# Nightmare-n/GD-MAE

Measured on AMD Instinct MI355X. Metric: MAE pre-train frames/sec (Waymo-shape, 180k pts, 75% mask), higher is better.
Workload: dtype bf16

## Files before the change

### gd-mae_amd/csrc/conv_block.hip

```cpp
#include "../../include/gdmae_hip.h"
#include "common.h"
#include "dw_grouped.h"
#include "gemm.h"
#include <stdlib.h>

bool gd_spconv_supported(int cin, int cout);
int gd_spconv(hipStream_t st, const void* X, int x_f32, const int* nbr, const void* Wp, long long n, int cin, int cout, void* Y, int slot,
              float* part, const float* ride_part = nullptr, int ride_S = 0, int ride_cout = 0, int ride_cin = 0,
              float* ride_dW = nullptr);
int gd_spconv_rows(int cin, int cout, int x_f32);
int gd_bn_fold_from_partials(hipStream_t st, const float* part, int nblk, int C, double count, const float* gamma,
                             const float* beta, double eps, double momentum, float* running_mean, float* running_var,
                             long long* num_batches, double* stats, float* ab, float* mv);

namespace {

__device__ inline unsigned short cb_f2bf(float f) { return gd_to_bf16(f); }

__global__ __launch_bounds__(256) void k_gather_rows_f32_bf16(const float* __restrict__ src, const int* __restrict__ idx,
                                                              long long n_slots, int C, unsigned short* __restrict__ out) {
  const int cv = C >> 3;
  const long long total = n_slots * cv;
  for (long long i = blockIdx.x * (long long)blockDim.x + threadIdx.x; i < total; i += (long long)gridDim.x * blockDim.x) {
    const long long s = i / cv;
    const int c = (int)(i % cv) << 3;
    const int j = idx[s];
    uint4 q = make_uint4(0, 0, 0, 0);
    if (j >= 0) {
      const float4 a = *reinterpret_cast<const float4*>(src + (long long)j * C + c);
      const float4 b = *reinterpret_cast<const float4*>(src + (long long)j * C + c + 4);
      q.x = cb_f2bf(a.x) | ((unsigned)cb_f2bf(a.y) << 16);
      q.y = cb_f2bf(a.z) | ((unsigned)cb_f2bf(a.w) << 16);
      q.z = cb_f2bf(b.x) | ((unsigned)cb_f2bf(b.y) << 16);
      q.w = cb_f2bf(b.z) | ((unsigned)cb_f2bf(b.w) << 16);
    }
    *reinterpret_cast<uint4*>(out + s * C + c) = q;
  }
}

template <typename T>
__global__ __launch_bounds__(256) void k_permute_w(const T* __restrict__ W, int cout, int cin, T* __restrict__ Wt) {
  const int total = cout * 9 * cin;
  for (int e = blockIdx.x * blockDim.x + threadIdx.x; e < total; e += gridDim.x * blockDim.x) {
    const int i = e % cin, ko = e / cin, o = ko % cout, k = ko / cout;
    Wt[e] = W[((long long)o * 9 + k) * cin + i];
  }
}

struct Scratch {
  char *gemm_ws, *cs_ws, *st, *rs_ws, *c01, *dy, *gcols, *wt, *sk_ws, *dw_part;
  size_t bytes;
};
int conv_dw_pick(long long n_out, int tiles, long long* n_pad) {
  static const int wgs = getenv("GDMAE_SPCONV_DW_WGS") ? atoi(getenv("GDMAE_SPCONV_DW_WGS")) : 640;
  return gd_dw_pick(n_out, tiles, wgs, n_pad);
}
Scratch layout(void* base, long long n_in, long long n_out, int cin, int cout, int es, bool implicit) {
  Scratch s;
  size_t off = 0;
  auto take = [&](size_t b) { char* p = (char*)base + off; off += gd_align(b); return p; };
  s.gemm_ws = take(implicit ? 0 : GD_LT_WORKSPACE);
  s.cs_ws = take(gdmae_colstats_workspace_bytes(cout));
  s.st = take((size_t)3 * cout * sizeof(double));
  s.rs_ws = take(gdmae_rows_bwd_stats_workspace_bytes(cout));
  s.c01 = take((size_t)2 * cout * sizeof(float));
  long long n_pad = n_out;
  const int S_dw = implicit ? conv_dw_pick(n_out, 9 * (cout / 128) * (cin / 128), &n_pad) : 0;
  s.dy = take((size_t)n_pad * cout * es);
  s.gcols = take(implicit ? 0 : (size_t)n_in * 9 * cout * es);
  s.wt = take(implicit ? 0 : (size_t)9 * cout * cin * es);
  s.sk_ws = take(implicit ? 0 : gdmae_gemm_tn_splitk_workspace_bytes(n_out, cout, 9 * cin));
  s.dw_part = nullptr;
  if (implicit) {
    s.dw_part = take((size_t)S_dw * 9 * cout * cin * sizeof(float));
  }
  s.bytes = off;
  return s;
}
bool use_implicit(const gdmae_conv_block_args* a) {
  static const int off = getenv("GDMAE_SPCONV") ? atoi(getenv("GDMAE_SPCONV")) == 0 : 0;
  return !off && a->bf16 && a->packed_fwd != nullptr && a->packed_bwd != nullptr && gd_spconv_supported(a->cin, a->cout) &&
         gd_spconv_supported(a->cout, a->cin);
}

__global__ __launch_bounds__(256) void k_spconv_dw_reduce(const float* __restrict__ part, int S, int cout, int cin, float* __restrict__ dW) {
  const long long per_tap = (long long)S * cout * cin, mn4 = (long long)cout * cin / 4;
  for (long long e = blockIdx.x * (long long)blockDim.x + threadIdx.x; e < 9 * mn4; e += (long long)gridDim.x * blockDim.x) {
    const int k = (int)(e / mn4);
    const long long r = e % mn4;
    const float4* p = reinterpret_cast<const float4*>(part + k * per_tap) + r;
    float4 acc = make_float4(0.f, 0.f, 0.f, 0.f);
    int s = 0;
    for (; s + 8 <= S; s += 8) {
      float4 v[8];
#pragma unroll
      for (int j = 0; j < 8; ++j) v[j] = p[(long long)(s + j) * mn4];
#pragma unroll
      for (int j = 0; j < 8; ++j) { acc.x += v[j].x; acc.y += v[j].y; acc.z += v[j].z; acc.w += v[j].w; }
    }
    for (; s < S; ++s) {
      const float4 v = p[(long long)s * mn4];
      acc.x += v.x; acc.y += v.y; acc.z += v.z; acc.w += v.w;
    }
    const long long o = (r * 4) / cin, i = (r * 4) % cin;
    float4* d = reinterpret_cast<float4*>(dW + (o * 9 + k) * cin + i);
    float4 w = *d;
    w.x += acc.x; w.y += acc.y; w.z += acc.z; w.w += acc.w;
    *d = w;
  }
}

#define CB_TRY(x)             \
  do {                        \
    int rc_ = (x);            \
    if (rc_ != 0) return rc_; \
  } while (0)

}

extern "C" size_t gdmae_conv_block_scratch_bytes(long long n_in, long long n_out, int cin, int cout, int bf16) {
  size_t b = layout(nullptr, n_in, n_out, cin, cout, bf16 ? 2 : 4, false).bytes;
  if (bf16 && gd_spconv_supported(cin, cout) && gd_spconv_supported(cout, cin)) {
    const size_t bi = layout(nullptr, n_in, n_out, cin, cout, 2, true).bytes;
    b = bi > b ? bi : b;
  }
  return b;
}

extern "C" int gdmae_conv_block_fwd(const gdmae_conv_block_args* a, void* stream) {
  GD_REQUIRE(a->cin % 8 == 0 && a->cout % 8 == 0 && a->cout <= 256, "conv block: channels must be multiples of 8, cout <= 256");
  if (a->n_out <= 0) return 0;
  hipStream_t st = (hipStream_t)stream;
  const int es = a->bf16 ? 2 : 4;
  const bool implicit = use_implicit(a);
  Scratch s = layout(a->scratch, a->n_in, a->n_out, a->cin, a->cout, es, implicit);
  const long long slots = a->n_out * 9;
  bool stats_fused = false;
  if (implicit) {
    const int rpw = gd_spconv_rows(a->cin, a->cout, a->x_f32);
    const long long nblk = rpw > 0 ? (a->n_out + rpw - 1) / rpw : 0;
    static const bool fuse_ok = !(getenv("GDMAE_SPCONV_STATS") && atoi(getenv("GDMAE_SPCONV_STATS")) == 0);
    stats_fused = fuse_ok && nblk >= 1 && nblk <= 1024;
    CB_TRY(gd_spconv(st, a->x, a->x_f32, a->nbr, a->packed_fwd, a->n_out, a->cin, a->cout, a->y, GD_T_SPCONV_FWD,
                     stats_fused ? (float*)s.cs_ws : nullptr));
    if (stats_fused)
      CB_TRY(gd_bn_fold_from_partials(st, (const float*)s.cs_ws, (int)nblk, a->cout, (double)a->n_out, a->gamma, a->beta, a->eps, a->momentum,
                                      a->running_mean, a->running_var, a->num_batches, a->stats, a->ab, a->mv));
  } else if (a->bf16 && a->x_f32) {
    long long g = (slots * (a->cin / 8) + 255) / 256;
    if (g > 16384) g = 16384;
    hipLaunchKernelGGL(k_gather_rows_f32_bf16, dim3((int)g), dim3(256), 0, st, (const float*)a->x, a->nbr, slots, a->cin,
                       (unsigned short*)a->cols);
    GD_LAUNCH_CHECK();
  } else {
    CB_TRY(gdmae_gather_rows(a->x, a->nbr, slots, a->cin * es, a->cols, stream));
  }
  if (!implicit)
    CB_TRY(gdmae_gemm(a->cols, a->W, a->y, a->n_out, a->cout, 9ll * a->cin, 0, 1, a->bf16, 0, nullptr, s.gemm_ws, stream));
  if (!stats_fused)
    CB_TRY(gdmae_bn_fold(a->y, a->n_out, a->cout, a->bf16, (double)a->n_out, a->gamma, a->beta, a->eps, a->momentum, a->running_mean,
                         a->running_var, a->num_batches, a->stats, a->ab, a->mv, s.cs_ws, stream));
  CB_TRY(gdmae_rows_affine_relu_scatter(a->y, a->bf16, nullptr, a->n_out, a->cout, a->ab, a->ab + a->cout, a->out,
                                        a->out_f32 ? 0 : a->bf16, a->cout, 0, stream));
  return 0;
}

extern "C" int gdmae_conv_block_bwd(const gdmae_conv_block_args* a, void* stream) {
  GD_REQUIRE(a->cin % 8 == 0 && a->cout % 8 == 0 && a->cout <= 256, "conv block: channels must be multiples of 8, cout <= 256");
  if (a->n_out <= 0) return 0;
  hipStream_t st = (hipStream_t)stream;
  const int es = a->bf16 ? 2 : 4;
  const bool implicit = use_implicit(a);
  Scratch s = layout(a->scratch, a->n_in, a->n_out, a->cin, a->cout, es, implicit);
  const int C = a->cout;
  CB_TRY(gdmae_rows_bwd_stats(a->y, a->bf16, nullptr, a->n_out, C, a->ab, a->ab + C, a->g, a->g_f32 ? 0 : a->bf16, C, 0, nullptr,
                              s.rs_ws, stream));
  CB_TRY(gdmae_bn_bwd_coeffs_rows((const float*)s.rs_ws, gdmae_rows_bwd_stats_rows(a->n_out), 3, a->stats, a->ab, a->gamma, C,
                                  (double)a->n_out, nullptr, a->dgamma, a->dbeta, 1, (float*)s.c01, stream));
  CB_TRY(gdmae_rows_bwd(a->y, a->bf16, nullptr, a->n_out, C, a->ab, a->ab + C, (const float*)s.c01, (const float*)s.c01 + C, a->g,
                        a->g_f32 ? 0 : a->bf16, C, 0, s.dy, a->bf16, stream));
  if (implicit) {
    GdDwGroup Gp;
    Gp.n_jobs = 9;
    long long n_pad = 0;
    const int S = conv_dw_pick(a->n_out, 9 * (C / 128) * (a->cin / 128), &n_pad);
    for (int k = 0; k < 9; ++k) {
      Gp.job[k] = GdDwJob{s.dy, a->x, C, a->cin, (float*)s.dw_part + (size_t)k * S * C * a->cin, nullptr, 0, a->nbr + k, 9, a->x_f32};
    }
    {
      GdTimed timed(GD_T_SPCONV_BWD, st, (double)a->n_out * (2.0 * C + 9.0 * a->cin * (a->x_f32 ? 4 : 2) + 36.0) + 36.0 * S * C * a->cin,
                    2.0 * a->n_out * 9.0 * C * a->cin);
      CB_TRY(gd_dw_grouped_s(st, Gp, n_pad, a->n_out, S));
    }
    GD_REQUIRE(Gp.S == S, "conv block: slice count");
    static const bool rides = !(getenv("GDMAE_DW_REDUCE_RIDES") && atoi(getenv("GDMAE_DW_REDUCE_RIDES")) == 0);
    bool reduced = false;
    if (a->dx && rides) {
      const int rc = gd_spconv(st, s.dy, 0, a->nbr_t, a->packed_bwd, a->n_in, C, a->cin, a->dx, GD_T_SPCONV_BWD, nullptr, (const float*)s.dw_part, S,
                               C, a->cin, a->dW);
      if (rc != -2) {
        CB_TRY(rc);
        reduced = true;
      }
    }
    if (!reduced) {
      hipLaunchKernelGGL(k_spconv_dw_reduce, dim3(gd_div_up(9ll * C * a->cin / 4, 256)), dim3(256), 0, st, (const float*)s.dw_part, S, C, a->cin,
                         a->dW);
      GD_LAUNCH_CHECK();
      if (a->dx) CB_TRY(gd_spconv(st, s.dy, 0, a->nbr_t, a->packed_bwd, a->n_in, C, a->cin, a->dx, GD_T_SPCONV_BWD, nullptr));
    }
    return 0;
  }
  CB_TRY(gdmae_gemm_tn_splitk(s.dy, a->cols, a->dW, a->n_out, C, 9 * a->cin, a->bf16, 1, s.sk_ws, stream));
  if (a->dx) {
    CB_TRY(gdmae_gather_rows(s.dy, a->nbr_t, a->n_in * 9, C * es, s.gcols, stream));
    const int total = C * 9 * a->cin;
    if (a->bf16) hipLaunchKernelGGL((k_permute_w<unsigned short>), dim3((total + 255) / 256), dim3(256), 0, st, (const unsigned short*)a->W, C, a->cin, (unsigned short*)s.wt);
    else hipLaunchKernelGGL((k_permute_w<float>), dim3((total + 255) / 256), dim3(256), 0, st, (const float*)a->W, C, a->cin, (float*)s.wt);
    GD_LAUNCH_CHECK();
    CB_TRY(gdmae_gemm(s.gcols, s.wt, a->dx, a->n_in, a->cin, 9ll * C, 0, 0, a->bf16, 0, nullptr, s.gemm_ws, stream));
  }
  return 0;
}
```

### gd-mae_amd/csrc/partition.hip

```cpp
#include "common.h"

struct Dims {
  int B, Y, X;
};

struct VisLoad {
  const float* mask;
  const int* counts;
  __device__ int operator()(long long p) const { return (p < counts[1] && mask[p] == 0.f) ? 1 : 0; }
};
struct VisStore {
  const int* counts;
  const int* pillar_cell;
  int* tok_pillar;
  int* tok_cell;
  int* map;
  __device__ void operator()(long long p, int ex, int v) const {
    if (v) {
      tok_pillar[ex] = (int)p;
      int c = pillar_cell[p];
      tok_cell[ex] = c;
      map[c] = ex;
    }
  }
};

extern "C" int gdmae_visible_tokens(const float* mask, const int* pillar_cell, const int* vox_counts, long long m_cap,
                                    long long n_cells, int* tok_pillar, int* tok_cell, int* map, int* n_tok,
                                    void* scan_ws, void* stream) {
  hipStream_t st = (hipStream_t)stream;
  GD_CHECK(hipMemsetAsync(map, 0xFF, sizeof(int) * n_cells, st));
  return gd_device_scan<int>(m_cap, VisLoad{mask, vox_counts}, VisStore{vox_counts, pillar_cell, tok_pillar, tok_cell, map},
                             n_tok, (int*)scan_ws, st);
}

__global__ __launch_bounds__(256) void k_mark_down(const int* __restrict__ n_in, const int* __restrict__ tok_cell,
                                                   Dims di, Dims dn, int* __restrict__ flag) {
  const int M = *n_in;
  for (int t = blockIdx.x * blockDim.x + threadIdx.x; t < M; t += gridDim.x * blockDim.x) {
    int c = tok_cell[t];
    int x = c % di.X;
    int r = c / di.X;
    int y = r % di.Y;
    int b = r / di.Y;
#pragma unroll
    for (int ky = 0; ky < 3; ++ky) {
      int ty = y + 1 - ky;
      if (ty < 0 || (ty & 1)) continue;
      int oy = ty >> 1;
      if (oy >= dn.Y) continue;
#pragma unroll
      for (int kx = 0; kx < 3; ++kx) {
        int tx = x + 1 - kx;
        if (tx < 0 || (tx & 1)) continue;
        int ox = tx >> 1;
        if (ox >= dn.X) continue;
        flag[(b * dn.Y + oy) * dn.X + ox] = 1;
      }
    }
  }
}

struct FlagLoad {
  const int* flag;
  __device__ int operator()(long long c) const { return flag[c]; }
};
struct FlagStore {
  int* tok_cell;
  int* map;
  __device__ void operator()(long long c, int ex, int v) const {
    if (v) {
      tok_cell[ex] = (int)c;
      map[c] = ex;
    } else {
      map[c] = -1;
    }
  }
};

extern "C" int gdmae_downsample_tokens(const int* n_in, const int* tok_cell_in, long long cap_in, int B, int Yi, int Xi,
                                       int* tok_cell_out, int* map_out, int* n_out, int* flag_ws, void* scan_ws,
                                       void* stream) {
  hipStream_t st = (hipStream_t)stream;
  Dims di{B, Yi, Xi};
  Dims dn{B, (Yi + 2 - 3) / 2 + 1, (Xi + 2 - 3) / 2 + 1};
  const long long cells = (long long)B * dn.Y * dn.X;
  GD_CHECK(hipMemsetAsync(flag_ws, 0, sizeof(int) * cells, st));
  int grid = gd_div_up(cap_in > 0 ? cap_in : 1, 256);
  if (grid > 2048) grid = 2048;
  hipLaunchKernelGGL(k_mark_down, dim3(grid), dim3(256), 0, st, n_in, tok_cell_in, di, dn, flag_ws);
  GD_LAUNCH_CHECK();
  return gd_device_scan<int>(cells, FlagLoad{flag_ws}, FlagStore{tok_cell_out, map_out}, n_out, (int*)scan_ws, st);
}

__global__ __launch_bounds__(256) void k_rulebook(const int* __restrict__ n_tok, const int* __restrict__ tok_cell, Dims dt,
                                                  Dims dm, const int* __restrict__ map, int mode, int* __restrict__ nbr) {
  const long long total = (long long)(*n_tok) * 9;
  for (long long i = blockIdx.x * (long long)blockDim.x + threadIdx.x; i < total; i += (long long)gridDim.x * blockDim.x) {
    const int t = (int)(i / 9), k = (int)(i % 9);
    const int ky = k / 3, kx = k % 3;
    int c = tok_cell[t];
    int x = c % dt.X;
    int r = c / dt.X;
    int y = r % dt.Y;
    int b = r / dt.Y;
    int my, mx;
    bool ok = true;
    if (mode == 0) {
      my = y + ky - 1;
      mx = x + kx - 1;
    } else if (mode == 1) {
      my = 2 * y - 1 + ky;
      mx = 2 * x - 1 + kx;
    } else {
      int ty = y + 1 - ky, tx = x + 1 - kx;
      ok = !(ty & 1) && !(tx & 1) && ty >= 0 && tx >= 0;
      my = ty >> 1;
      mx = tx >> 1;
    }
    ok = ok && my >= 0 && my < dm.Y && mx >= 0 && mx < dm.X;
    nbr[i] = ok ? map[(b * dm.Y + my) * dm.X + mx] : -1;
  }
}

extern "C" int gdmae_rulebook(const int* n_tok, const int* tok_cell, long long cap, int B, int Yt, int Xt, int Ym,
                              int Xm, const int* map, int mode, int* nbr, void* stream) {
  GD_REQUIRE(mode >= 0 && mode <= 2, "rulebook mode");
  int grid = gd_div_up((cap > 0 ? cap : 1) * 9, 256);
  if (grid > 4096) grid = 4096;
  hipLaunchKernelGGL(k_rulebook, dim3(grid), dim3(256), 0, (hipStream_t)stream, n_tok, tok_cell, Dims{B, Yt, Xt},
                     Dims{B, Ym, Xm}, map, mode, nbr);
  GD_LAUNCH_CHECK();
  return 0;
}

struct WinParams {
  int B, Y, X;
  int wx, wy;
  int sx, sy;
  int nwx, nwy, nwz;
  int nlev;
  int lo[3], hi[3], T[3];
};

__device__ inline int win_token(const WinParams& P, const int* map, int w, int lane, int& ref_id) {
  const int wyi = w % P.nwy;
  const int r = w / P.nwy;
  const int wxi = r % P.nwx;
  const int b = r / P.nwx;
  ref_id = b * (P.nwx * P.nwy * P.nwz) + wxi * (P.nwy * P.nwz) + wyi * P.nwz;
  if (lane >= P.wx * P.wy) return -1;
  const int ly = lane / P.wx, lx = lane % P.wx;
  const int x = wxi * P.wx - P.sx + lx;
  const int y = wyi * P.wy - P.sy + ly;
  if (x < 0 || x >= P.X || y < 0 || y >= P.Y) return -1;
  return map[(b * P.Y + y) * P.X + x];
}

__global__ __launch_bounds__(256) void k_win_count(WinParams P, const int* __restrict__ map, int n_win,
                                                   int* __restrict__ win_cnt) {
  const int lane = threadIdx.x & (GD_WAVE - 1);
  const int wib = threadIdx.x / GD_WAVE;
  for (int w = blockIdx.x * 4 + wib; w < n_win; w += gridDim.x * 4) {
    int ref;
    int t = win_token(P, map, w, lane, ref);
    unsigned long long m = __ballot(t >= 0);
    if (lane == 0) win_cnt[w] = __popcll(m);
  }
}

__device__ inline int win_level(const WinParams& P, int cnt) {
  for (int l = 0; l < P.nlev; ++l)
    if (cnt >= P.lo[l] && cnt < P.hi[l]) return l;
  return -1;
}

struct WinLoad {
  WinParams P;
  const int* win_cnt;
  __device__ U128 operator()(long long w) const {
    int c = win_cnt[w];
    if (c <= 0) return U128{0ull, 0ull};
    int l = win_level(P, c);
    if (l < 0) return U128{0ull, 0ull};
    return U128{1ull << (21 * l), (unsigned long long)c << (21 * l)};
  }
};
struct WinStore {
  int* win_dense;
  int* win_tokpre;
  __device__ void operator()(long long w, U128 ex, U128 v) const {
    if (v.a) {
      int l = (v.a >> 21) ? ((v.a >> 42) ? 2 : 1) : 0;
      win_dense[w] = (int)((ex.a >> (21 * l)) & 0x1FFFFFull);
      win_tokpre[w] = (int)((ex.b >> (21 * l)) & 0x1FFFFFull);
    }
  }
};

__global__ void k_win_totals(const U128* total, int* counts) {
  if (threadIdx.x == 0 && blockIdx.x == 0) {
    int nw = 0, nt = 0;
    for (int l = 0; l < 3; ++l) {
      int a = (int)((total->a >> (21 * l)) & 0x1FFFFFull);
      int b = (int)((total->b >> (21 * l)) & 0x1FFFFFull);
      counts[l] = a;
      counts[3 + l] = b;
      nw += a;
      nt += b;
    }
    counts[6] = nw;
    counts[7] = nt;
  }
}

__global__ __launch_bounds__(256) void k_win_fill(WinParams P, const int* __restrict__ map, int n_win,
                                                  const int* __restrict__ win_cnt, const int* __restrict__ win_dense,
                                                  const int* __restrict__ win_tokpre, const int* __restrict__ counts,
                                                  int* __restrict__ tok_win, int* __restrict__ tok_level,
                                                  int* __restrict__ tok_slot, int* __restrict__ tok_pos,
                                                  int* __restrict__ csr_tok, int* __restrict__ win_start,
                                                  int* __restrict__ win_len) {
  const int lane = threadIdx.x & (GD_WAVE - 1);
  const int wib = threadIdx.x / GD_WAVE;
  for (int w = blockIdx.x * 4 + wib; w < n_win; w += gridDim.x * 4) {
    const int cnt = win_cnt[w];
    if (cnt <= 0) continue;
    const int l = win_level(P, cnt);
    if (l < 0) continue;
    int ref;
    const int t = win_token(P, map, w, lane, ref);
    const unsigned long long m = __ballot(t >= 0);
    int wbase = 0, tbase = 0;
    for (int q = 0; q < l; ++q) {
      wbase += counts[q];
      tbase += counts[3 + q];
    }
    const int d = win_dense[w];
    const int start = tbase + win_tokpre[w];
    if (lane == 0) {
      win_start[wbase + d] = start;
      win_len[wbase + d] = cnt;
    }
    if (t >= 0) {
      const int r = __popcll(m & ((1ull << lane) - 1ull));
      csr_tok[start + r] = t;
      tok_win[t] = ref;
      tok_level[t] = l;
      tok_slot[t] = d * P.T[l] + r;
      tok_pos[t] = lane;
    }
  }
}

extern "C" size_t gdmae_window_workspace_bytes(int B, int Y, int X, int wx, int wy) {
  long long nwx = (X + wx - 1) / wx + 1, nwy = (Y + wy - 1) / wy + 1;
  long long n = B * nwx * nwy;
  return gd_align(sizeof(int) * n) * 3 + gd_align(sizeof(U128) * (gd_scan_ws_elems(n) + 2)) + 4096;
}

extern "C" int gdmae_window_partition(const int* map, int B, int Y, int X, int wx, int wy, int shifted, int nlev,
                                      const int* drop_lo, const int* drop_hi, const int* max_tokens, int* tok_win,
                                      int* tok_level, int* tok_slot, int* tok_pos, int* csr_tok, int* win_start,
                                      int* win_len, int* counts, void* workspace, size_t workspace_bytes, void* stream) {
  hipStream_t st = (hipStream_t)stream;
  GD_REQUIRE(wx * wy <= GD_WAVE && wx > 0 && wy > 0, "window must fit one wavefront (wx*wy <= 64)");
  GD_REQUIRE(nlev >= 1 && nlev <= 3, "1..3 drop levels");
  WinParams P;
  P.B = B;
  P.Y = Y;
  P.X = X;
  P.wx = wx;
  P.wy = wy;
  P.sx = shifted ? wx / 2 : wx;
  P.sy = shifted ? wy / 2 : wy;
  P.nwx = (X + wx - 1) / wx + 1;
  P.nwy = (Y + wy - 1) / wy + 1;
  P.nwz = 2;
  P.nlev = nlev;
  for (int l = 0; l < 3; ++l) {
    P.lo[l] = l < nlev ? drop_lo[l] : 0;
    P.hi[l] = l < nlev ? drop_hi[l] : 0;
    P.T[l] = l < nlev ? max_tokens[l] : 0;
  }
  const long long n_win = (long long)B * P.nwx * P.nwy;
  GD_REQUIRE(n_win < (1 << 21), "window grid too large for the packed scan");
  GD_REQUIRE(workspace_bytes >= gdmae_window_workspace_bytes(B, Y, X, wx, wy), "window workspace too small");
  GdArena A(workspace, workspace_bytes);
  int* win_cnt = A.take<int>(n_win);
  int* win_dense = A.take<int>(n_win);
  int* win_tokpre = A.take<int>(n_win);
  U128* scan_ws = A.take<U128>(gd_scan_ws_elems(n_win) + 2);
  U128* total = scan_ws + gd_scan_ws_elems(n_win);
  int grid = gd_div_up(n_win, 4);
  if (grid > 8192) grid = 8192;
  hipLaunchKernelGGL(k_win_count, dim3(grid), dim3(256), 0, st, P, map, (int)n_win, win_cnt);
  GD_LAUNCH_CHECK();
  int rc = gd_device_scan<U128>(n_win, WinLoad{P, win_cnt}, WinStore{win_dense, win_tokpre}, total, scan_ws, st);
  if (rc) return rc;
  hipLaunchKernelGGL(k_win_totals, dim3(1), dim3(64), 0, st, total, counts);
  GD_LAUNCH_CHECK();
  hipLaunchKernelGGL(k_win_fill, dim3(grid), dim3(256), 0, st, P, map, (int)n_win, win_cnt, win_dense, win_tokpre,
                     counts, tok_win, tok_level, tok_slot, tok_pos, csr_tok, win_start, win_len);
  GD_LAUNCH_CHECK();
  return 0;
}



struct VisCellLoad {
  const float* mask;
  const int* cell2pillar;
  __device__ int operator()(long long c) const {
    const int p = cell2pillar[c];
    const float m = mask[p < 0 ? 0 : p];
    return (int)(p >= 0) & (int)(m == 0.f);
  }
};
struct VisCellStore {
  const int* cell2pillar;
  int* tok_pillar;
  int* tok_cell;
  int* map;
  __device__ void operator()(long long c, int ex, int v) const {
    map[c] = v ? ex : -1;
    if (v) {
      tok_pillar[ex] = cell2pillar[c];
      tok_cell[ex] = (int)c;
    }
  }
};
size_t gd_plan_scan_state_bytes(long long n) { return gd_scan_lb_state_bytes<int>(n); }
size_t gd_plan_win_state_bytes(long long n) { return gd_scan_lb_state_bytes<U128>(n); }

int gd_plan_visible_tokens(const float* mask, const int* cell2pillar, long long n_cells, int* tok_pillar, int* tok_cell, int* map,
                           int* n_tok, void* lb_state, hipStream_t st) {
  return gd_device_scan_lb<int>(n_cells, VisCellLoad{mask, cell2pillar}, VisCellStore{cell2pillar, tok_pillar, tok_cell, map}, GdNoTotal{},
                                n_tok, lb_state, st);
}

struct DownLoad {
  const int* map_in;
  Dims di, dn;
  __device__ int operator()(long long c) const {
    const int ci = (int)c;
    const int ox = ci % dn.X;
    const int r = ci / dn.X;
    const int oy = r % dn.Y, b = r / dn.Y;
    const int* m = map_in + (long long)b * di.Y * di.X;
    int any = 0;
#pragma unroll
    for (int ky = 0; ky < 3; ++ky) {
      const int iy = 2 * oy - 1 + ky;
      const int cy = iy < 0 ? 0 : (iy >= di.Y ? di.Y - 1 : iy);
#pragma unroll
      for (int kx = 0; kx < 3; ++kx) {
        const int ix = 2 * ox - 1 + kx;
        const int cx = ix < 0 ? 0 : (ix >= di.X ? di.X - 1 : ix);
        const int v = m[(long long)cy * di.X + cx];
        any |= (int)(v >= 0 && iy == cy && ix == cx);
      }
    }
    return any;
  }
};
int gd_plan_downsample(const int* map_in, int B, int Yi, int Xi, int* tok_cell_out, int* map_out, int* n_out, void* lb_state,
                       hipStream_t st) {
  Dims di{B, Yi, Xi};
  Dims dn{B, (Yi + 2 - 3) / 2 + 1, (Xi + 2 - 3) / 2 + 1};
  const long long cells = (long long)B * dn.Y * dn.X;
  return gd_device_scan_lb<int>(cells, DownLoad{map_in, di, dn}, FlagStore{tok_cell_out, map_out}, GdNoTotal{}, n_out, lb_state, st);
}

struct PlanJob {
  const int* n_tok;
  const int* tok_cell;
  Dims dt, dm;
  const int* map;
  int mode, s;
  int* nbr;
  int* nbr_rev;
};
constexpr int kPlanMaxJobs = 16;
struct PlanJobs {
  PlanJob j[kPlanMaxJobs];
  int count;
};
__global__ __launch_bounds__(256) void k_plan_jobs(PlanJobs J) {
  const PlanJob& q = J.j[blockIdx.y];
  const int n = *q.n_tok;
  if (q.mode == 3) {
    const int ss = q.s * q.s;
    const long long total = (long long)n * ss;
    for (long long i = blockIdx.x * (long long)blockDim.x + threadIdx.x; i < total; i += (long long)gridDim.x * blockDim.x) {
      const int t = (int)(i / ss), e = (int)(i % ss);
      const int c = q.tok_cell[t];
      const int x = c % q.dt.X, r = c / q.dt.X, y = r % q.dt.Y, b = r / q.dt.Y;
      q.nbr[i] = (b * (q.dt.Y * q.s) + y * q.s + e / q.s) * (q.dt.X * q.s) + x * q.s + e % q.s;
    }
    return;
  }
  const long long total = (long long)n * 9;
  for (long long i = blockIdx.x * (long long)blockDim.x + threadIdx.x; i < total; i += (long long)gridDim.x * blockDim.x) {
    const int t = (int)(i / 9), k = (int)(i % 9);
    const int ky = k / 3, kx = k % 3;
    const int c = q.tok_cell[t];
    const int x = c % q.dt.X, r = c / q.dt.X, y = r % q.dt.Y, b = r / q.dt.Y;
    int my, mx;
    bool ok = true;
    if (q.mode == 0) {
      my = y + ky - 1;
      mx = x + kx - 1;
    } else if (q.mode == 1) {
      my = 2 * y - 1 + ky;
      mx = 2 * x - 1 + kx;
    } else {
      const int ty = y + 1 - ky, tx = x + 1 - kx;
      ok = !(ty & 1) && !(tx & 1) && ty >= 0 && tx >= 0;
      my = ty >> 1;
      mx = tx >> 1;
    }
    ok = ok && my >= 0 && my < q.dm.Y && mx >= 0 && mx < q.dm.X;
    const int v = ok ? q.map[(b * q.dm.Y + my) * q.dm.X + mx] : -1;
    q.nbr[i] = v;
    if (q.nbr_rev) q.nbr_rev[(long long)t * 9 + (8 - k)] = v;
  }
}
int gd_plan_jobs(const PlanJobs& J, long long cap_max, hipStream_t st) {
  if (J.count <= 0) return 0;
  int grid = gd_div_up((cap_max > 0 ? cap_max : 1) * 9, 256);
  if (grid > 2048) grid = 2048;
  hipLaunchKernelGGL(k_plan_jobs, dim3(grid, J.count), dim3(256), 0, st, J);
  GD_LAUNCH_CHECK();
  return 0;
}

constexpr int GD_WIN_JOBS = 8;
struct WinSet {
  WinParams P[GD_WIN_JOBS];
  const int* map[GD_WIN_JOBS];
  int n_win[GD_WIN_JOBS];
  int* win_cnt[GD_WIN_JOBS];
  int* win_dense[GD_WIN_JOBS];
  int* win_tokpre[GD_WIN_JOBS];
  int* counts[GD_WIN_JOBS];
  int *tok_win[GD_WIN_JOBS], *tok_level[GD_WIN_JOBS], *tok_slot[GD_WIN_JOBS], *tok_pos[GD_WIN_JOBS], *csr_tok[GD_WIN_JOBS],
      *win_start[GD_WIN_JOBS], *win_len[GD_WIN_JOBS];
};
__global__ __launch_bounds__(256) void k_win_count2(WinSet Q) {
  const int lane = threadIdx.x & (GD_WAVE - 1);
  const int wib = threadIdx.x / GD_WAVE;
  const int sh = blockIdx.y;
  const int n_win = Q.n_win[sh];
  const int* __restrict__ map = Q.map[sh];
  for (int w = blockIdx.x * 4 + wib; w < n_win; w += gridDim.x * 4) {
    int ref;
    const int t = win_token(Q.P[sh], map, w, lane, ref);
    const unsigned long long m = __ballot(t >= 0);
    if (lane == 0) Q.win_cnt[sh][w] = __popcll(m);
  }
}
struct WinTotal {
  int* counts;
  __device__ void operator()(U128 total) const {
    int nw = 0, nt = 0;
    for (int l = 0; l < 3; ++l) {
      const int a = (int)((total.a >> (21 * l)) & 0x1FFFFFull);
      const int b = (int)((total.b >> (21 * l)) & 0x1FFFFFull);
      counts[l] = a;
      counts[3 + l] = b;
      nw += a;
      nt += b;
    }
    counts[6] = nw;
    counts[7] = nt;
  }
};
__global__ __launch_bounds__(256) void k_win_fill2(WinSet Q) {
  const int lane = threadIdx.x & (GD_WAVE - 1);
  const int wib = threadIdx.x / GD_WAVE;
  const int sh = blockIdx.y;
  const int n_win = Q.n_win[sh];
  const int* __restrict__ map = Q.map[sh];
  const WinParams& P = Q.P[sh];
  const int* counts = Q.counts[sh];
  for (int w = blockIdx.x * 4 + wib; w < n_win; w += gridDim.x * 4) {
    const int cnt = Q.win_cnt[sh][w];
    if (cnt <= 0) continue;
    const int l = win_level(P, cnt);
    if (l < 0) continue;
    int ref;
    const int t = win_token(P, map, w, lane, ref);
    const unsigned long long m = __ballot(t >= 0);
    int wbase = 0, tbase = 0;
    for (int q = 0; q < l; ++q) {
      wbase += counts[q];
      tbase += counts[3 + q];
    }
    const int d = Q.win_dense[sh][w];
    const int start = tbase + Q.win_tokpre[sh][w];
    if (lane == 0) {
      Q.win_start[sh][wbase + d] = start;
      Q.win_len[sh][wbase + d] = cnt;
    }
    if (t >= 0) {
      const int r = __popcll(m & ((1ull << lane) - 1ull));
      Q.csr_tok[sh][start + r] = t;
      Q.tok_win[sh][t] = ref;
      Q.tok_level[sh][t] = l;
      Q.tok_slot[sh][t] = d * P.T[l] + r;
      Q.tok_pos[sh][t] = lane;
    }
  }
}
size_t gd_plan_windows_ws_bytes(int B, int Y, int X, int wx, int wy) {
  const long long n = (long long)B * ((X + wx - 1) / wx + 1) * ((Y + wy - 1) / wy + 1);
  return 2 * 3 * gd_align(sizeof(int) * n);
}
long long gd_plan_n_windows(int B, int Y, int X, int wx, int wy) { return (long long)B * ((X + wx - 1) / wx + 1) * ((Y + wy - 1) / wy + 1); }
struct GdWinStage {
  const int* map;
  int B, Y, X, wx, wy, nlev;
  const int *drop_lo, *drop_hi, *max_tokens;
  int* out[2][7];
  int* counts[2];
  void* workspace;
  void* lb_state;
};
int gd_plan_windows_all(const GdWinStage* stages, int n_stages, hipStream_t st) {
  GD_REQUIRE(n_stages >= 1 && 2 * n_stages <= GD_WIN_JOBS, "window partitions: at most four stages per launch");
  WinSet Q;
  GdScanBatch<U128, WinLoad, WinStore, WinTotal, GD_WIN_JOBS> Sc;
  long long n_max = 1;
  for (int i = 0; i < n_stages; ++i) {
    const GdWinStage& g = stages[i];
    GD_REQUIRE(g.wx * g.wy <= GD_WAVE && g.wx > 0 && g.wy > 0, "window must fit one wavefront (wx*wy <= 64)");
    GD_REQUIRE(g.nlev >= 1 && g.nlev <= 3, "1..3 drop levels");
    const long long n_win = gd_plan_n_windows(g.B, g.Y, g.X, g.wx, g.wy);
    GD_REQUIRE(n_win < (1 << 21), "window grid too large for the packed scan");
    n_max = n_win > n_max ? n_win : n_max;
    GdArena A(g.workspace, gd_plan_windows_ws_bytes(g.B, g.Y, g.X, g.wx, g.wy));
    for (int sh = 0; sh < 2; ++sh) {
      const int j = 2 * i + sh;
      WinParams& P = Q.P[j];
      P.B = g.B; P.Y = g.Y; P.X = g.X; P.wx = g.wx; P.wy = g.wy;
      P.sx = sh ? g.wx / 2 : g.wx;
      P.sy = sh ? g.wy / 2 : g.wy;
      P.nwx = (g.X + g.wx - 1) / g.wx + 1;
      P.nwy = (g.Y + g.wy - 1) / g.wy + 1;
      P.nwz = 2;
      P.nlev = g.nlev;
      for (int l = 0; l < 3; ++l) {
        P.lo[l] = l < g.nlev ? g.drop_lo[l] : 0;
        P.hi[l] = l < g.nlev ? g.drop_hi[l] : 0;
        P.T[l] = l < g.nlev ? g.max_tokens[l] : 0;
      }
      Q.map[j] = g.map;
      Q.n_win[j] = (int)n_win;
      Q.win_cnt[j] = A.take<int>(n_win);
      Q.win_dense[j] = A.take<int>(n_win);
      Q.win_tokpre[j] = A.take<int>(n_win);
      Q.counts[j] = g.counts[sh];
      Q.tok_win[j] = g.out[sh][0]; Q.tok_level[j] = g.out[sh][1]; Q.tok_slot[j] = g.out[sh][2]; Q.tok_pos[j] = g.out[sh][3];
      Q.csr_tok[j] = g.out[sh][4]; Q.win_start[j] = g.out[sh][5]; Q.win_len[j] = g.out[sh][6];
      Sc.n[j] = n_win;
      Sc.load[j] = WinLoad{P, Q.win_cnt[j]};
      Sc.store[j] = WinStore{Q.win_dense[j], Q.win_tokpre[j]};
      Sc.on_total[j] = WinTotal{g.counts[sh]};
      Sc.S[j] = gd_scan_lb_state<U128>(n_win, (char*)g.lb_state + sh * gd_plan_win_state_bytes(n_win));
    }
  }
  for (int j = 2 * n_stages; j < GD_WIN_JOBS; ++j) {
    Q.P[j] = Q.P[0]; Q.map[j] = Q.map[0]; Q.n_win[j] = 0;
    Q.win_cnt[j] = Q.win_cnt[0]; Q.win_dense[j] = Q.win_dense[0]; Q.win_tokpre[j] = Q.win_tokpre[0]; Q.counts[j] = Q.counts[0];
    Q.tok_win[j] = Q.tok_win[0]; Q.tok_level[j] = Q.tok_level[0]; Q.tok_slot[j] = Q.tok_slot[0]; Q.tok_pos[j] = Q.tok_pos[0];
    Q.csr_tok[j] = Q.csr_tok[0]; Q.win_start[j] = Q.win_start[0]; Q.win_len[j] = Q.win_len[0];
    Sc.n[j] = 0; Sc.load[j] = Sc.load[0]; Sc.store[j] = Sc.store[0]; Sc.on_total[j] = Sc.on_total[0]; Sc.S[j] = Sc.S[0];
  }
  int grid = gd_div_up(n_max, 4);
  if (grid > 4096) grid = 4096;
  hipLaunchKernelGGL(k_win_count2, dim3(grid, 2 * n_stages), dim3(256), 0, st, Q);
  GD_LAUNCH_CHECK();
  int rc = gd_device_scan_lb_batch(Sc, 2 * n_stages, st);
  if (rc) return rc;
  hipLaunchKernelGGL(k_win_fill2, dim3(grid, 2 * n_stages), dim3(256), 0, st, Q);
  GD_LAUNCH_CHECK();
  return 0;
}
```

### gd-mae_amd/csrc/plan.hip

```cpp
#include "../../include/gdmae_hip.h"
#include "common.h"
#include <string.h>

int gd_voxelize_impl(const float* points, long long n_points, int n_cols, const float* lo, const float* vs, const int* grid_xyz,
                     int batch_size, float* points_out, long long* point_coords, long long* inverse, int* inverse32,
                     long long* voxel_coords, int* pillar_cell, int* pillar_pt_off, int* pillar_pts, int* point_rank,
                     int* sample_pillar_off, float* pillar_mean, int* cell2pillar_out, int* counts, void* workspace, size_t workspace_bytes,
                     void* lb_state, float* points_pm, int* row_pillar, hipStream_t st);
size_t gd_voxelize_lb_state_bytes(long long n_points, long long cells);
size_t gd_plan_scan_state_bytes(long long n);
size_t gd_plan_win_state_bytes(long long n);
int gd_plan_visible_tokens(const float* mask, const int* cell2pillar, long long n_cells, int* tok_pillar, int* tok_cell, int* map,
                           int* n_tok, void* lb_state, hipStream_t st);
int gd_plan_downsample(const int* map_in, int B, int Yi, int Xi, int* tok_cell_out, int* map_out, int* n_out, void* lb_state,
                       hipStream_t st);
struct Dims {
  int B, Y, X;
};
struct PlanJob {
  const int* n_tok;
  const int* tok_cell;
  Dims dt, dm;
  const int* map;
  int mode, s;
  int* nbr;
  int* nbr_rev;
};
constexpr int kPlanMaxJobs = 16;
struct PlanJobs {
  PlanJob j[kPlanMaxJobs];
  int count;
};
int gd_plan_jobs(const PlanJobs& J, long long cap_max, hipStream_t st);
size_t gd_plan_windows_ws_bytes(int B, int Y, int X, int wx, int wy);
long long gd_plan_n_windows(int B, int Y, int X, int wx, int wy);
struct GdWinStage {
  const int* map;
  int B, Y, X, wx, wy, nlev;
  const int *drop_lo, *drop_hi, *max_tokens;
  int* out[2][7];
  int* counts[2];
  void* workspace;
  void* lb_state;
};
int gd_plan_windows_all(const GdWinStage* stages, int n_stages, hipStream_t st);
size_t gd_decoder_tiles_lb_state_bytes(long long nt);
int gd_decoder_tiles_lb(const int* const* maps, const int* strides, int k, int B, int H, int W, int* tile_slot, int* tile_list, int* n_act,
                        int* flag, void* lb_state, hipStream_t st);
int gd_decoder_site_rulebook(const int* site, const int* n_dev, int sites_per_tok, long long cap_sites, const int* tile_slot, int H, int W,
                             int* nbr, hipStream_t st);

namespace {

struct StageGeo {
  int Y, X;
  long long cap;
  long long cap_in;
  int up_s;
  long long n_win;
};

struct Layout {
  gdmae_plan_buffer* table;
  int max_entries, n;
  size_t off;
  bool ok;
  long long add(const char* name, size_t bytes) {
    const size_t o = off;
    if (table) {
      if (n >= max_entries) {
        ok = false;
        return -1;
      }
      strncpy(table[n].name, name, sizeof(table[n].name) - 1);
      table[n].name[sizeof(table[n].name) - 1] = 0;
      table[n].offset = (long long)o;
      table[n].bytes = (long long)bytes;
    }
    ++n;
    off += gd_align(bytes);
    return (long long)o;
  }
};

struct Offsets {
  long long lb_state, counts, points, point_coords, inverse, inverse32, voxel_coords, pillar_cell, pt_off, pillar_pts, point_rank,
      sample_off, pillar_mean, cell2pillar, points_pm, row_pillar, vox_ws, mask, len_keep, tok_pillar;
  long long vis_tok_cell, vis_map;
  struct {
    long long tok_cell, map, nbr_subm, nbr_subm_t, nbr_down, nbr_down_t, up_sites, win_ws;
    long long w[2][7];
  } s[GDMAE_PLAN_MAX_STAGES];
  long long dec_slot, dec_list, dec_flag, dec_nbr[3];
  size_t lb_bytes, vox_ws_bytes;
  int n_counts;
  bool dec;
  StageGeo geo[GDMAE_PLAN_MAX_STAGES];
  long long cap_pts, m_cap, cells;
};

int check(const gdmae_plan_params* p) {
  GD_REQUIRE(p != nullptr, "geometry plan: null parameters");
  GD_REQUIRE(p->n_points >= 0 && p->n_points < (1ll << 31) && p->n_cols >= 4 && p->n_cols <= 65 && p->batch_size >= 1,
             "geometry plan: bad point buffer");
  GD_REQUIRE(p->grid[0] >= 1 && p->grid[1] >= 1 && p->grid[2] == 1, "geometry plan: single-layer pillar grids (spt_backbone_mae.py:94)");
  GD_REQUIRE(p->n_stages >= 1 && p->n_stages <= GDMAE_PLAN_MAX_STAGES, "geometry plan: 1..4 stages");
  for (int i = 0; i < p->n_stages; ++i) {
    GD_REQUIRE(p->stride[i] == 1 || p->stride[i] == 2, "geometry plan: conv_down stride 1 or 2 (k3 s2 p1)");
    GD_REQUIRE(i == 0 || p->stride[i] == 2, "geometry plan: only the first stage may keep the resolution");
    GD_REQUIRE(p->win_x[i] >= 1 && p->win_y[i] >= 1 && p->win_x[i] * p->win_y[i] <= 64, "geometry plan: window must fit one wavefront");
    GD_REQUIRE(p->n_levels[i] >= 1 && p->n_levels[i] <= 3, "geometry plan: 1..3 drop levels");
  }
  GD_REQUIRE(p->n_dec >= 0 && p->n_dec <= 3, "geometry plan: at most 3 decoder source stages");
  for (int g = 0; g < p->n_dec; ++g) GD_REQUIRE(p->dec_sources[g] >= 0 && p->dec_sources[g] < p->n_stages, "geometry plan: decoder source");
  return 0;
}

int layout(const gdmae_plan_params* p, gdmae_plan_buffer* table, int max_entries, Offsets& O, size_t* total, int* n_entries) {
  if (int rc = check(p)) return rc;
  Layout L{table, max_entries, 0, 0, true};
  const int B = p->batch_size, gx = p->grid[0], gy = p->grid[1], F = p->n_cols - 1;
  const long long n0 = p->cap_points > p->n_points ? p->cap_points : p->n_points;
  O.cells = (long long)B * gx * gy;
  GD_REQUIRE(O.cells < (1ll << 31), "geometry plan: B*Y*X must fit int32");
  O.cap_pts = n0 > 0 ? n0 : 1;
  O.m_cap = n0 < O.cells ? n0 : O.cells;
  if (O.m_cap < 1) O.m_cap = 1;
  const long long cap = O.cap_pts;
  int Y = gy, X = gx;
  long long c = O.m_cap;
  for (int i = 0; i < p->n_stages; ++i) {
    StageGeo& g = O.geo[i];
    g.cap_in = c;
    if (p->stride[i] == 2) {
      Y = (Y - 1) / 2 + 1;
      X = (X - 1) / 2 + 1;
      c = 4 * c < (long long)B * Y * X ? 4 * c : (long long)B * Y * X;
    }
    g.Y = Y; g.X = X; g.cap = c;
    const int us = gy / Y;
    g.up_s = (us >= 1 && us * Y == gy && us * X == gx) ? us : 0;
    g.n_win = gd_plan_n_windows(B, Y, X, p->win_x[i], p->win_y[i]);
    GD_REQUIRE(g.n_win < (1 << 21), "geometry plan: window grid too large for the packed scan");
    GD_REQUIRE(g.cap < (1 << 21), "geometry plan: stage token capacity must stay below 2^21 (21-bit fields of the packed window scan)");
  }
  O.dec = p->n_dec > 0;
  for (int g = 0; g < p->n_dec; ++g) {
    const int us = O.geo[p->dec_sources[g]].up_s;
    O.dec = O.dec && (us == 1 || us == 2 || us == 4 || us == 8);
  }
  const long long nt = (long long)B * ((gy + 7) / 8) * ((gx + 7) / 8);
  size_t lb = gd_voxelize_lb_state_bytes(n0, O.cells) + gd_plan_scan_state_bytes(O.cells);
  for (int i = 0; i < p->n_stages; ++i) {
    if (p->stride[i] == 2) lb += gd_plan_scan_state_bytes((long long)B * O.geo[i].Y * O.geo[i].X);
    lb += 2 * gd_plan_win_state_bytes(O.geo[i].n_win);
  }
  if (O.dec) lb += gd_decoder_tiles_lb_state_bytes(nt);
  O.lb_bytes = lb;
  O.lb_state = L.add("lb_state", lb);
  O.n_counts = 2 + p->n_stages + 16 * p->n_stages + 1 + 1;
  O.counts = L.add("counts", sizeof(int) * O.n_counts);
  O.points = L.add("points", sizeof(float) * cap * p->n_cols);
  O.point_coords = L.add("point_coords", sizeof(long long) * cap * 4);
  O.inverse = L.add("inverse", sizeof(long long) * cap);
  O.inverse32 = L.add("inverse32", sizeof(int) * cap);
  O.voxel_coords = L.add("voxel_coords", sizeof(long long) * cap * 4);
  O.pillar_cell = L.add("pillar_cell", sizeof(int) * cap);
  O.pt_off = L.add("pt_off", sizeof(int) * (cap + 1));
  O.pillar_pts = L.add("pillar_pts", sizeof(int) * cap);
  O.point_rank = L.add("point_rank", sizeof(int) * cap);
  O.sample_off = L.add("sample_off", sizeof(int) * (B + 1));
  O.pillar_mean = L.add("pillar_mean", sizeof(float) * cap * F);
  O.cell2pillar = L.add("cell2pillar", sizeof(int) * O.cells);
  O.points_pm = L.add("points_pm", sizeof(float) * cap * p->n_cols);
  O.row_pillar = L.add("row_pillar", sizeof(int) * cap);
  O.vox_ws_bytes = gdmae_voxelize_workspace_bytes(n0, B, gx, gy, 1);
  O.vox_ws = L.add("vox_ws", O.vox_ws_bytes);
  O.mask = L.add("mask", sizeof(float) * O.m_cap);
  O.len_keep = L.add("len_keep", sizeof(int) * B);
  O.tok_pillar = L.add("tok_pillar", sizeof(int) * O.m_cap);
  O.vis_tok_cell = O.vis_map = -1;
  if (p->stride[0] == 2) {
    O.vis_tok_cell = L.add("vis.tok_cell", sizeof(int) * O.m_cap);
    O.vis_map = L.add("vis.map", sizeof(int) * O.cells);
  }
  char nm[40];
  static const char* const kWin[7] = {"tok_win", "tok_level", "tok_slot", "tok_pos", "csr_tok", "win_start", "win_len"};
  for (int i = 0; i < p->n_stages; ++i) {
    const StageGeo& g = O.geo[i];
    auto name = [&](const char* s) { snprintf(nm, sizeof(nm), "s%d.%s", i, s); return (const char*)nm; };
    O.s[i].tok_cell = L.add(name("tok_cell"), sizeof(int) * g.cap);
    O.s[i].map = L.add(name("map"), sizeof(int) * (long long)B * g.Y * g.X);
    O.s[i].nbr_subm = L.add(name("nbr_subm"), sizeof(int) * g.cap * 9);
    O.s[i].nbr_subm_t = L.add(name("nbr_subm_t"), sizeof(int) * g.cap * 9);
    O.s[i].nbr_down = O.s[i].nbr_down_t = O.s[i].up_sites = -1;
    if (p->stride[i] == 2) {
      O.s[i].nbr_down = L.add(name("nbr_down"), sizeof(int) * g.cap * 9);
      O.s[i].nbr_down_t = L.add(name("nbr_down_t"), sizeof(int) * g.cap_in * 9);
    }
    if (g.up_s > 1) O.s[i].up_sites = L.add(name("up_sites"), sizeof(int) * g.cap * g.up_s * g.up_s);
    O.s[i].win_ws = L.add(name("win_ws"), gd_plan_windows_ws_bytes(B, g.Y, g.X, p->win_x[i], p->win_y[i]));
    const long long wcap = g.n_win < g.cap ? g.n_win : g.cap;
    for (int sh = 0; sh < 2; ++sh)
      for (int k = 0; k < 7; ++k) {
        snprintf(nm, sizeof(nm), "s%d.w%d.%s", i, sh, kWin[k]);
        O.s[i].w[sh][k] = L.add(nm, sizeof(int) * (k < 5 ? g.cap : wcap));
      }
  }
  O.dec_slot = O.dec_list = O.dec_flag = -1;
  if (O.dec) {
    O.dec_slot = L.add("dec.tile_slot", sizeof(int) * nt);
    O.dec_list = L.add("dec.tile_list", sizeof(int) * nt);
    O.dec_flag = L.add("dec.flag", sizeof(int) * nt);
    for (int g = 0; g < p->n_dec; ++g) {
      const StageGeo& sg = O.geo[p->dec_sources[g]];
      snprintf(nm, sizeof(nm), "dec.nbr%d", g);
      O.dec_nbr[g] = L.add(nm, sizeof(int) * sg.cap * sg.up_s * sg.up_s * 9);
    }
  }
  GD_REQUIRE(L.ok, "geometry plan: buffer table too small");
  if (total) *total = L.off;
  if (n_entries) *n_entries = L.n;
  return 0;
}

}

extern "C" int gdmae_geometry_plan_layout(const gdmae_plan_params* p, gdmae_plan_buffer* table, int max_entries, int* n_entries,
                                          size_t* total_bytes) {
  Offsets O;
  return layout(p, table, max_entries, O, total_bytes, n_entries);
}

extern "C" int gdmae_geometry_plan(const gdmae_plan_params* p, const float* points, const float* noise, void* arena, size_t arena_bytes,
                                   void* stream) {
  Offsets O;
  size_t total = 0;
  if (int rc = layout(p, nullptr, 0, O, &total, nullptr)) return rc;
  GD_REQUIRE(arena != nullptr && arena_bytes >= total, "geometry plan: arena too small (gdmae_geometry_plan_layout)");
  GD_REQUIRE(!p->masked || noise != nullptr, "geometry plan: masking needs one noise value per pillar (capacity min(points, cells))");
  hipStream_t st = (hipStream_t)stream;
  char* A = (char*)arena;
  auto I = [&](long long off) { return off < 0 ? (int*)nullptr : (int*)(A + off); };
  const int B = p->batch_size, gx = p->grid[0], gy = p->grid[1], ns = p->n_stages;
  int* counts = I(O.counts);
  int* n_tok = counts + 2;
  int* win_counts = counts + 2 + ns;
  int* n_act = counts + 2 + ns + 16 * ns;
  int* n_vis = n_act + 1;
  GD_CHECK(hipMemsetAsync(A + O.lb_state, 0, (size_t)(O.counts - O.lb_state) + gd_align(sizeof(int) * O.n_counts), st));
  char* lb = A + O.lb_state;
  {
    int rc = gd_voxelize_impl(points, p->n_points, p->n_cols, p->lo, p->vs, p->grid, B, (float*)(A + O.points), (long long*)(A + O.point_coords),
                              (long long*)(A + O.inverse), I(O.inverse32), (long long*)(A + O.voxel_coords), I(O.pillar_cell), I(O.pt_off),
                              I(O.pillar_pts), I(O.point_rank), I(O.sample_off), (float*)(A + O.pillar_mean), I(O.cell2pillar), counts,
                              A + O.vox_ws, O.vox_ws_bytes, lb, p->want_pm ? (float*)(A + O.points_pm) : nullptr,
                              p->want_pm ? I(O.row_pillar) : nullptr, st);
    if (rc) return rc;
    lb += gd_voxelize_lb_state_bytes(p->n_points, O.cells);
  }
  float* mask = (float*)(A + O.mask);
  if (p->masked) {
    int rc = gdmae_random_mask(noise, I(O.sample_off), B, p->keep_frac, mask, I(O.len_keep), stream);
    if (rc) return rc;
  } else {
    GD_CHECK(hipMemsetAsync(mask, 0, sizeof(float) * O.m_cap, st));
  }
  const bool first_strided = p->stride[0] == 2;
  int* cur_cell = first_strided ? I(O.vis_tok_cell) : I(O.s[0].tok_cell);
  int* cur_map = first_strided ? I(O.vis_map) : I(O.s[0].map);
  int* cur_n = first_strided ? n_vis : n_tok;
  {
    int rc = gd_plan_visible_tokens(mask, I(O.cell2pillar), O.cells, I(O.tok_pillar), cur_cell, cur_map, cur_n, lb, st);
    if (rc) return rc;
    lb += gd_plan_scan_state_bytes(O.cells);
  }
  int Yp = gy, Xp = gx;
  PlanJobs J;
  J.count = 0;
  long long cap_max = 1;
  GdWinStage W[4];
  GD_REQUIRE(ns <= 4, "geometry plan: at most four stages");
  for (int i = 0; i < ns; ++i) {
    const StageGeo& g = O.geo[i];
    GD_REQUIRE(J.count + 4 <= kPlanMaxJobs, "geometry plan: job table full");
    if (g.cap > cap_max) cap_max = g.cap;
    if (p->stride[i] == 2) {
      int rc = gd_plan_downsample(cur_map, B, Yp, Xp, I(O.s[i].tok_cell), I(O.s[i].map), n_tok + i, lb, st);
      if (rc) return rc;
      lb += gd_plan_scan_state_bytes((long long)B * g.Y * g.X);
      J.j[J.count++] = PlanJob{n_tok + i, I(O.s[i].tok_cell), Dims{B, g.Y, g.X}, Dims{B, Yp, Xp}, cur_map, 1, 0, I(O.s[i].nbr_down), nullptr};
      J.j[J.count++] = PlanJob{cur_n, cur_cell, Dims{B, Yp, Xp}, Dims{B, g.Y, g.X}, I(O.s[i].map), 2, 0, I(O.s[i].nbr_down_t), nullptr};
      if (g.cap_in > cap_max) cap_max = g.cap_in;
      cur_cell = I(O.s[i].tok_cell);
      cur_map = I(O.s[i].map);
      cur_n = n_tok + i;
      Yp = g.Y;
      Xp = g.X;
    }
    J.j[J.count++] = PlanJob{cur_n, cur_cell, Dims{B, g.Y, g.X}, Dims{B, g.Y, g.X}, cur_map, 0, 0, I(O.s[i].nbr_subm), I(O.s[i].nbr_subm_t)};
    if (g.up_s > 1) {
      J.j[J.count++] = PlanJob{cur_n, cur_cell, Dims{B, g.Y, g.X}, Dims{B, g.Y, g.X}, nullptr, 3, g.up_s, I(O.s[i].up_sites), nullptr};
      if (g.cap * g.up_s * g.up_s / 9 + 1 > cap_max) cap_max = g.cap * g.up_s * g.up_s / 9 + 1;
    }
    GdWinStage& w = W[i];
    w.map = cur_map;
    w.B = B; w.Y = g.Y; w.X = g.X; w.wx = p->win_x[i]; w.wy = p->win_y[i]; w.nlev = p->n_levels[i];
    w.drop_lo = p->drop_lo[i]; w.drop_hi = p->drop_hi[i]; w.max_tokens = p->max_tokens[i];
    w.counts[0] = win_counts + 16 * i;
    w.counts[1] = win_counts + 16 * i + 8;
    for (int sh = 0; sh < 2; ++sh)
      for (int k = 0; k < 7; ++k) w.out[sh][k] = I(O.s[i].w[sh][k]);
    w.workspace = A + O.s[i].win_ws;
    w.lb_state = lb;
    lb += 2 * gd_plan_win_state_bytes(g.n_win);
  }
  {
    int rc = gd_plan_jobs(J, cap_max, st);
    if (rc) return rc;
    rc = gd_plan_windows_all(W, ns, st);
    if (rc) return rc;
  }
  if (O.dec) {
    const int* maps[3];
    int ups[3];
    for (int g = 0; g < p->n_dec; ++g) {
      maps[g] = I(O.s[p->dec_sources[g]].map);
      ups[g] = O.geo[p->dec_sources[g]].up_s;
    }
    int rc = gd_decoder_tiles_lb(maps, ups, p->n_dec, B, gy, gx, I(O.dec_slot), I(O.dec_list), n_act, I(O.dec_flag), lb, st);
    if (rc) return rc;
    for (int g = 0; g < p->n_dec; ++g) {
      const int si = p->dec_sources[g];
      const StageGeo& sg = O.geo[si];
      const int* sites = sg.up_s > 1 ? I(O.s[si].up_sites) : I(O.s[si].tok_cell);
      rc = gd_decoder_site_rulebook(sites, n_tok + si, sg.up_s * sg.up_s, sg.cap * sg.up_s * sg.up_s, I(O.dec_slot), gy, gx, I(O.dec_nbr[g]), st);
      if (rc) return rc;
    }
  }
  return 0;
}
```

### gd-mae_amd/csrc/spconv.hip

```cpp
#include "../../include/gdmae_hip.h"
#include "common.h"
#include "dw_grouped.h"
#include <stdlib.h>

typedef float f32x16 __attribute__((ext_vector_type(16)));
typedef __bf16 bf16x8 __attribute__((ext_vector_type(8)));

namespace {

union SpFrag {
  uint4 q;
  bf16x8 v;
};
__device__ inline unsigned short sp_f2bf(float f) { return gd_to_bf16(f); }
__device__ inline unsigned sp_pack2(float lo, float hi) { return gd_pack_bf16(lo, hi); }

struct SpArgs {
  const void* X;
  const int* nbr;
  const uint4* Wp;
  unsigned short* Y;
  long long n;
  float* part;
  const float* ride_part;
  float* ride_dW;
  int ride_S, ride_cout, ride_cin;
  unsigned ride_blocks;
  const float* bias;
};

__device__ __forceinline__ void sp_ride_dw_reduce(const SpArgs& A) {
  const int S = A.ride_S, cout = A.ride_cout, cin = A.ride_cin;
  const long long per_tap = (long long)S * cout * cin, mn4 = (long long)cout * cin / 4;
  for (long long e = blockIdx.x * (long long)blockDim.x + threadIdx.x; e < 9 * mn4; e += (long long)A.ride_blocks * blockDim.x) {
    const int k = (int)(e / mn4);
    const long long r = e % mn4;
    const float4* p = reinterpret_cast<const float4*>(A.ride_part + k * per_tap) + r;
    float4 acc = make_float4(0.f, 0.f, 0.f, 0.f);
    int s = 0;
    for (; s + 8 <= S; s += 8) {
      float4 v[8];
#pragma unroll
      for (int j = 0; j < 8; ++j) v[j] = p[(long long)(s + j) * mn4];
#pragma unroll
      for (int j = 0; j < 8; ++j) { acc.x += v[j].x; acc.y += v[j].y; acc.z += v[j].z; acc.w += v[j].w; }
    }
    for (; s < S; ++s) {
      const float4 v = p[(long long)s * mn4];
      acc.x += v.x; acc.y += v.y; acc.z += v.z; acc.w += v.w;
    }
    const long long o = (r * 4) / cin, i = (r * 4) % cin;
    float4* d = reinterpret_cast<float4*>(A.ride_dW + (o * 9 + k) * cin + i);
    float4 w = *d;
    w.x += acc.x; w.y += acc.y; w.z += acc.z; w.w += acc.w;
    *d = w;
  }
}

constexpr int kWaves = 8;

#ifndef SP_ROWS256
#define SP_ROWS256 64
#endif
template <int CIN, int COUT, bool SRC_F32>
struct SpRows {
#ifndef SP_ROWS128
#define SP_ROWS128 128
#endif
  static constexpr int value = COUT >= 256 ? ((SRC_F32 && CIN >= 256) ? 32 : SP_ROWS256) : ((CIN == 128 && !SRC_F32) ? SP_ROWS128 : 64);
};

template <int CIN, int COUT, bool SRC_F32, bool EPI = false>
__global__ __launch_bounds__(512, 2) void k_spconv(SpArgs A) {
  constexpr int ROWS = SpRows<CIN, COUT, SRC_F32>::value;
  constexpr int KS = CIN / 16;
  constexpr int MB = COUT / 32;
  constexpr int MPW = MB >= kWaves ? MB / kWaves : 1;
  constexpr int WPB = MB >= kWaves ? 1 : kWaves / MB;
  constexpr int NPW = (ROWS / 32) / WPB;
  static_assert(NPW >= 1 && NPW * WPB * 32 == ROWS, "row blocks");
  constexpr int XP = CIN * 2 + 16;
  constexpr int SP = COUT * 2 + 16;
  constexpr int CPR = CIN / 8;
  constexpr int RPP = 512 / CPR;
  constexpr int P = ROWS / RPP;
  static_assert(P >= 1 && ROWS % RPP == 0, "unsupported shape");
  extern __shared__ __align__(16) unsigned char lds[];
  if (blockIdx.x < A.ride_blocks) return sp_ride_dw_reduce(A);
  const unsigned blk = blockIdx.x - A.ride_blocks;
  const int tid = threadIdx.x, lane = tid & 63, wv = tid >> 6;
  const long long row0 = (long long)blk * ROWS;
  const int mb0 = wv / WPB;
  const int nb0 = (wv % WPB) * NPW;
  const uint4* __restrict__ wp = A.Wp + (size_t)mb0 * 64 + lane;

  constexpr int RING = (KS == 16 && (ROWS == 64 || SRC_F32)) ? ((SRC_F32 && ROWS == 64) ? 4 : 8) : ((KS == 8 && ROWS == 128) ? 4 : KS);
  SpFrag wr[RING][MPW];
#pragma unroll
  for (int ks = 0; ks < RING; ++ks)
#pragma unroll
    for (int j = 0; j < MPW; ++j) wr[ks][j].q = wp[((size_t)ks * MB + j * kWaves) * 64];

  constexpr int GD = 1;
  constexpr int RQ = SRC_F32 ? 2 : 1;
  const int gc = tid % CPR;
  long long nrow[P];
  unsigned rvalid = 0u;
#pragma unroll
  for (int p = 0; p < P; ++p) {
    const long long g = row0 + p * RPP + tid / CPR;
    rvalid |= g < A.n ? 1u << p : 0u;
    nrow[p] = (g < A.n ? g : A.n - 1) * 9;
  }
  int idx[P];
  uint4 rq[1][P][RQ];
  unsigned keep[1] = {0u};
  auto load_idx = [&](int tap) {
#pragma unroll
    for (int p = 0; p < P; ++p) idx[p] = A.nbr[nrow[p] + tap];
  };
  auto fetch = [&](int slot) {
    unsigned k = 0u;
#pragma unroll
    for (int p = 0; p < P; ++p) {
      asm volatile("" : "+v"(idx[p]));
      const bool ok = idx[p] >= 0 && ((rvalid >> p) & 1u);
      const long long j = ok ? idx[p] : 0;
      k |= ok ? 1u << p : 0u;
      if (SRC_F32) {
        const float* s = (const float*)A.X + j * CIN + gc * 8;
        rq[slot][p][0] = *reinterpret_cast<const uint4*>(s);
        rq[slot][p][RQ - 1] = *reinterpret_cast<const uint4*>(s + 4);
      } else {
        rq[slot][p][0] = *reinterpret_cast<const uint4*>((const unsigned short*)A.X + j * CIN + gc * 8);
      }
    }
    keep[slot] = k;
  };
  auto stage = [&](unsigned char* b, int slot) {
#pragma unroll
    for (int p = 0; p < P; ++p) {
      uint4 q;
      if (SRC_F32) {
        const uint4 a = rq[slot][p][0], c = rq[slot][p][RQ - 1];
        q.x = sp_pack2(__uint_as_float(a.x), __uint_as_float(a.y)); q.y = sp_pack2(__uint_as_float(a.z), __uint_as_float(a.w));
        q.z = sp_pack2(__uint_as_float(c.x), __uint_as_float(c.y)); q.w = sp_pack2(__uint_as_float(c.z), __uint_as_float(c.w));
      } else {
        q = rq[slot][p][0];
      }
      const unsigned m = ((keep[slot] >> p) & 1u) ? 0xFFFFFFFFu : 0u;
      q.x &= m; q.y &= m; q.z &= m; q.w &= m;
      *reinterpret_cast<uint4*>(b + (p * RPP + tid / CPR) * XP + gc * 16) = q;
    }
  };
  load_idx(0);
  fetch(0);
  load_idx(1);
  stage(lds, 0);
  __syncthreads();

  f32x16 acc[MPW][NPW];
#pragma unroll
  for (int j = 0; j < MPW; ++j)
#pragma unroll
    for (int b = 0; b < NPW; ++b)
#pragma unroll
      for (int i = 0; i < 16; ++i) acc[j][b][i] = 0.f;

#pragma unroll
  for (int tap = 0; tap < 9; ++tap) {
    if (tap + GD < 9) {
      fetch(0);
      if (tap + GD + 1 < 9) load_idx(tap + GD + 1);
    }
    __builtin_amdgcn_sched_barrier(0);
    const unsigned char* lb = lds + (tap & 1) * (ROWS * XP) + ((nb0 * 32) + (lane & 31)) * XP + (lane >> 5) * 16;
    SpFrag sf[2][NPW];
#pragma unroll
    for (int b = 0; b < NPW; ++b) sf[0][b].q = *reinterpret_cast<const uint4*>(lb + b * 32 * XP);
#pragma unroll
    for (int ks = 0; ks < KS; ++ks) {
      if (ks + 1 < KS) {
#pragma unroll
        for (int b = 0; b < NPW; ++b) sf[(ks + 1) & 1][b].q = *reinterpret_cast<const uint4*>(lb + b * 32 * XP + (ks + 1) * 32);
      }
#pragma unroll
      for (int j = 0; j < MPW; ++j)
#pragma unroll
        for (int b = 0; b < NPW; ++b) acc[j][b] = __builtin_amdgcn_mfma_f32_32x32x16_bf16(wr[ks % RING][j].v, sf[ks & 1][b].v, acc[j][b], 0, 0, 0);
      if (tap * KS + ks + RING < 9 * KS) {
#pragma unroll
        for (int j = 0; j < MPW; ++j) wr[ks % RING][j].q = wp[(((size_t)tap * KS + ks + RING) * MB + j * kWaves) * 64];
      }
      __builtin_amdgcn_sched_barrier(0);
    }
    if (tap < 8) stage(lds + ((tap + 1) & 1) * (ROWS * XP), 0);
    __syncthreads();
  }

#pragma unroll
  for (int j = 0; j < MPW; ++j) {
    const int cb = (mb0 + j * kWaves) * 32 + 4 * (lane >> 5);
#pragma unroll
    for (int b = 0; b < NPW; ++b) {
      const int row = (nb0 + b) * 32 + (lane & 31);
#pragma unroll
      for (int q = 0; q < 4; ++q) {
        uint2 o;
        if constexpr (EPI) {
          const float4 bv = *reinterpret_cast<const float4*>(A.bias + cb + 8 * q);
          o.x = sp_pack2(fmaxf(acc[j][b][4 * q] + bv.x, 0.f), fmaxf(acc[j][b][4 * q + 1] + bv.y, 0.f));
          o.y = sp_pack2(fmaxf(acc[j][b][4 * q + 2] + bv.z, 0.f), fmaxf(acc[j][b][4 * q + 3] + bv.w, 0.f));
        } else {
        o.x = sp_pack2(acc[j][b][4 * q], acc[j][b][4 * q + 1]);
        o.y = sp_pack2(acc[j][b][4 * q + 2], acc[j][b][4 * q + 3]);
        }
        *reinterpret_cast<uint2*>(lds + row * SP + (cb + 8 * q) * 2) = o;
      }
    }
  }
  __syncthreads();
  {
    constexpr int OCPR = COUT / 8;
    constexpr int ORPP = 512 / OCPR;
    const int c = tid % OCPR, r = tid / OCPR;
    float s1[8], s2[8];
#pragma unroll
    for (int k = 0; k < 8; ++k) s1[k] = s2[k] = 0.f;
    const bool stats = A.part != nullptr;
#pragma unroll
    for (int p = 0; p < (ROWS + ORPP - 1) / ORPP; ++p) {
      const int rl = p * ORPP + r;
      if (rl < ROWS && row0 + rl < A.n) {
        const uint4 q = *reinterpret_cast<const uint4*>(lds + rl * SP + c * 16);
        *reinterpret_cast<uint4*>(A.Y + (row0 + rl) * COUT + c * 8) = q;
        if (stats) {
          const unsigned w[4] = {q.x, q.y, q.z, q.w};
#pragma unroll
          for (int k = 0; k < 4; ++k) {
            const float lo = __uint_as_float(w[k] << 16), hi = __uint_as_float(w[k] & 0xFFFF0000u);
            s1[2 * k] += lo; s2[2 * k] = fmaf(lo, lo, s2[2 * k]);
            s1[2 * k + 1] += hi; s2[2 * k + 1] = fmaf(hi, hi, s2[2 * k + 1]);
          }
        }
      }
    }
    if (stats) {
      static_assert(ORPP * 2 * COUT * 4 <= 2 * ROWS * XP || ORPP * 2 * COUT * 4 <= ROWS * SP, "statistics scratch fits the tiles");
      __syncthreads();
      float* red = reinterpret_cast<float*>(lds);
#pragma unroll
      for (int k = 0; k < 8; ++k) {
        red[(r * 2 + 0) * COUT + c * 8 + k] = s1[k];
        red[(r * 2 + 1) * COUT + c * 8 + k] = s2[k];
      }
      __syncthreads();
      for (int e = tid; e < 2 * COUT; e += 512) {
        float a = 0.f;
#pragma unroll
        for (int g = 0; g < ORPP; ++g) a += red[g * 2 * COUT + e];
        A.part[(long long)blk * 2 * COUT + e] = a;
      }
    }
  }
}

template <int CIN, int COUT, bool SRC_F32, bool EPI = false>
int sp_launch(const SpArgs& A, hipStream_t st) {
  constexpr int ROWS = SpRows<CIN, COUT, SRC_F32>::value;
  constexpr int tile = ROWS * (CIN * 2 + 16), stg = ROWS * (COUT * 2 + 16);
  constexpr int lds = 2 * tile > stg ? 2 * tile : stg;
  static bool once = false;
  if (!once) {
    GD_CHECK(hipFuncSetAttribute((const void*)k_spconv<CIN, COUT, SRC_F32, EPI>, hipFuncAttributeMaxDynamicSharedMemorySize, lds));
    once = true;
  }
  hipLaunchKernelGGL((k_spconv<CIN, COUT, SRC_F32, EPI>), dim3((unsigned)gd_div_up(A.n, ROWS) + A.ride_blocks), dim3(512), lds, st, A);
  GD_LAUNCH_CHECK();
  return 0;
}

}

bool gd_spconv_supported(int cin, int cout) { return (cin == 128 || cin == 256) && (cout == 128 || cout == 256); }
size_t gd_spconv_packed_bytes(int cin, int cout) { return (size_t)9 * cin * cout * 2; }

int gd_spconv_rows(int cin, int cout, int x_f32) {
#define SP_CASE(ci, co) \
  if (cin == ci && cout == co) return x_f32 ? SpRows<ci, co, true>::value : SpRows<ci, co, false>::value;
  SP_CASE(128, 128);
  SP_CASE(128, 256);
  SP_CASE(256, 128);
  SP_CASE(256, 256);
#undef SP_CASE
  return 0;
}
int gd_spconv(hipStream_t st, const void* X, int x_f32, const int* nbr, const void* Wp, long long n, int cin, int cout, void* Y, int slot,
              float* part, const float* ride_part, int ride_S, int ride_cout, int ride_cin, float* ride_dW) {
  if (n <= 0) return ride_part ? -2 : 0;
  GD_REQUIRE(gd_spconv_supported(cin, cout), "spconv: channels must be 128 or 256");
  SpArgs A{X, nbr, (const uint4*)Wp, (unsigned short*)Y, n, part, nullptr, nullptr, 0, 0, 0, 0u, nullptr};
  if (ride_part) {
    A.ride_part = ride_part; A.ride_dW = ride_dW; A.ride_S = ride_S; A.ride_cout = ride_cout; A.ride_cin = ride_cin;
    A.ride_blocks = (unsigned)gd_div_up(9ll * ride_cout * ride_cin / 4, 512);
  }
  GdTimed timed(slot, st, (double)n * (9.0 * cin * (x_f32 ? 4 : 2) + 2.0 * cout + 36.0) + 18.0 * cin * cout, 2.0 * n * 9.0 * cin * cout);
#define SP_CASE(ci, co)                                                    \
  if (cin == ci && cout == co) return x_f32 ? sp_launch<ci, co, true>(A, st) : sp_launch<ci, co, false>(A, st);
  SP_CASE(128, 128);
  SP_CASE(128, 256);
  SP_CASE(256, 128);
  SP_CASE(256, 256);
#undef SP_CASE
  return -1;
}

extern "C" size_t gdmae_spconv_packed_bytes(int cin, int cout) { return gd_spconv_packed_bytes(cin, cout); }

extern "C" int gdmae_spconv_pack_jobs(const float* W, int cin, int cout, int transposed, void* packed, long long* jobs) {
  GD_REQUIRE(gd_spconv_supported(cin, cout), "spconv_pack_jobs: channels must be 128 or 256");
  for (int t = 0; t < 9; ++t) {
    long long* J = jobs + 6 * t;
    J[0] = (long long)(W + (size_t)t * cin);
    J[1] = (long long)((char*)packed + (size_t)t * cin * cout * 2);
    J[2] = transposed ? cin : cout;
    J[3] = transposed ? cout : cin;
    J[4] = 9ll * cin;
    J[5] = transposed;
  }
  return 0;
}

extern "C" int gdmae_spconv(const void* X, int x_f32, const int* nbr, const void* packed, long long n, int cin, int cout, void* Y,
                            int timing_slot, void* stream) {
  return gd_spconv((hipStream_t)stream, X, x_f32, nbr, packed, n, cin, cout, Y, timing_slot > 0 ? timing_slot : GD_T_SPCONV_FWD, nullptr, nullptr, 0, 0, 0, nullptr);
}
extern "C" int gdmae_spconv_bias_relu(const void* X, int x_f32, const int* nbr, const void* packed, const float* bias, long long n, int cin,
                                      int cout, void* Y, void* stream) {
  if (n <= 0) return 0;
  GD_REQUIRE(gd_spconv_supported(cin, cout), "spconv_bias_relu: channels must be 128 or 256");
  GD_REQUIRE(bias != nullptr, "spconv_bias_relu: bias");
  hipStream_t st = (hipStream_t)stream;
  SpArgs A{X, nbr, (const uint4*)packed, (unsigned short*)Y, n, nullptr, nullptr, nullptr, 0, 0, 0, 0u, bias};
  GdTimed timed(GD_T_SPCONV_FWD, st, (double)n * (9.0 * cin * (x_f32 ? 4 : 2) + 2.0 * cout + 36.0) + 18.0 * cin * cout, 2.0 * n * 9.0 * cin * cout);
#define SP_CASE(ci, co) \
  if (cin == ci && cout == co) return x_f32 ? sp_launch<ci, co, true, true>(A, st) : sp_launch<ci, co, false, true>(A, st);
  SP_CASE(128, 128);
  SP_CASE(128, 256);
  SP_CASE(256, 128);
  SP_CASE(256, 256);
#undef SP_CASE
  return -1;
}
extern "C" int gdmae_spconv_stat_rows(int cin, int cout, int x_f32) { return gd_spconv_rows(cin, cout, x_f32); }
extern "C" int gdmae_spconv_stats(const void* X, int x_f32, const int* nbr, const void* packed, long long n, int cin, int cout, void* Y,
                                  float* part, void* stream) {
  GD_REQUIRE(part != nullptr, "spconv_stats: partial rows");
  return gd_spconv((hipStream_t)stream, X, x_f32, nbr, packed, n, cin, cout, Y, GD_T_SPCONV_FWD, part, nullptr, 0, 0, 0, nullptr);
}


namespace {
__global__ __launch_bounds__(256) void k_tap_dw_reduce(const float* __restrict__ part, int S, int M, int N, float* __restrict__ out, int ld_out,
                                                       int m_off) {
  const long long per_tap = (long long)S * M * N;
  const long long total = 9ll * N * M;
  for (long long e = blockIdx.x * (long long)blockDim.x + threadIdx.x; e < total; e += (long long)gridDim.x * blockDim.x) {
    const int n = (int)(e % N);
    const long long km = e / N;
    const int m = (int)(km % M), k = (int)(km / M);
    const float* p = part + k * per_tap + (long long)m * N + n;
    const long long st = (long long)M * N;
    float acc = 0.f;
    int s = 0;
    for (; s + 8 <= S; s += 8) {
      float v[8];
#pragma unroll
      for (int j = 0; j < 8; ++j) v[j] = p[(long long)(s + j) * st];
#pragma unroll
      for (int j = 0; j < 8; ++j) acc += v[j];
    }
    for (; s < S; ++s) acc += p[(long long)s * st];
    out[((long long)k * N + n) * ld_out + m_off + m] += acc;
  }
}
int tap_dw_pick(long long n, int tiles, long long* n_pad) {
  static const int wgs = getenv("GDMAE_SPCONV_DW_WGS") ? atoi(getenv("GDMAE_SPCONV_DW_WGS")) : 640;
  return gd_dw_pick(n, tiles, wgs, n_pad);
}
}

extern "C" long long gdmae_tap_dw_rows(long long n, int M, int N) {
  long long n_pad = 0;
  tap_dw_pick(n, 9 * (M / 128) * (N / 128), &n_pad);
  return n_pad;
}
extern "C" size_t gdmae_tap_dw_workspace_bytes(long long n, int M, int N) {
  long long n_pad = 0;
  return gd_align((size_t)tap_dw_pick(n, 9 * (M / 128) * (N / 128), &n_pad) * 9 * M * N * sizeof(float));
}
extern "C" int gdmae_tap_dw(const void* G, long long n, long long n_pad, int M, const void* X, const int* nbr, int N, float* out, int ld_out,
                            int m_off, void* workspace, void* stream) {
  GD_REQUIRE(M % 128 == 0 && N % 128 == 0 && n >= 0, "tap_dw: M, N multiples of 128");
  if (n == 0) return 0;
  hipStream_t st = (hipStream_t)stream;
  GdDwGroup Gp;
  Gp.n_jobs = 9;
  long long want = 0;
  const int S = tap_dw_pick(n, 9 * (M / 128) * (N / 128), &want);
  GD_REQUIRE(n_pad == want, "tap_dw: G must be allocated for gdmae_tap_dw_rows(n, M, N) rows");
  for (int k = 0; k < 9; ++k) Gp.job[k] = GdDwJob{G, X, M, N, (float*)workspace + (size_t)k * S * M * N, nullptr, 0, nbr + k, 9, 0};
  {
    GdTimed timed(GD_T_DEC_CONV_BWD, st, (double)n * (2.0 * M + 9.0 * 2.0 * N + 36.0) + 36.0 * S * M * N, 2.0 * n * 9.0 * M * N);
    int rc = gd_dw_grouped_s(st, Gp, n_pad, n, S);
    if (rc) return rc;
  }
  hipLaunchKernelGGL(k_tap_dw_reduce, dim3(gd_div_up(9ll * M * N, 256)), dim3(256), 0, st, (const float*)workspace, S, M, N, out, ld_out, m_off);
  GD_LAUNCH_CHECK();
  return 0;
}
```

### gd-mae_amd/gdmae_hip/convblock.py

```python
from __future__ import annotations

import ctypes as C

import torch

from . import lib as L
from . import ops, packing


import os

IMPLICIT = os.environ.get("GDMAE_SPCONV", "1") != "0"


class ConvBNReLUFn(torch.autograd.Function):
    @staticmethod
    def forward(ctx, x, info):
        weight, bn, nbr, nbr_t, direct, out_f32 = info
        cout, _, _, cin = weight.shape
        n_in, n_out = x.shape[0], nbr.shape[0]
        dev = x.device
        cdt = torch.bfloat16 if torch.is_autocast_enabled() else torch.float32
        assert x.dtype in (torch.float32, cdt)
        x = x.contiguous()
        wc = ops.shadow(weight, cdt).contiguous()
        a = L.ConvBlockArgs()
        a.n_in, a.n_out, a.cin, a.cout = n_in, n_out, cin, cout
        a.bf16, a.x_f32 = int(cdt == torch.bfloat16), int(x.dtype == torch.float32 and cdt != torch.float32)
        a.eps = float(bn.eps)
        a.x, a.nbr, a.nbr_t, a.W = L.ptr(x), L.ptr(nbr), L.ptr(nbr_t), L.ptr(wc)
        a.gamma, a.beta = L.ptr(bn.weight), L.ptr(bn.bias)
        if bn.training and bn.running_mean is not None:
            a.momentum = float(bn.momentum)
            a.running_mean, a.running_var, a.num_batches = L.ptr(bn.running_mean), L.ptr(bn.running_var), L.ptr(bn.num_batches_tracked)
        packed = None
        if cdt == torch.bfloat16 and IMPLICIT and packing.conv_supported(weight):
            packed = packing.conv_registered(weight)
            a.packed_fwd, a.packed_bwd = L.ptr(packed[0]), L.ptr(packed[1])
        cols = torch.empty(n_out, 9 * cin, dtype=cdt, device=dev) if packed is None else torch.empty(0, dtype=cdt, device=dev)
        y = torch.empty(n_out, cout, dtype=cdt, device=dev)
        out = torch.empty(n_out, cout, dtype=torch.float32 if out_f32 else cdt, device=dev)
        a.out_f32 = int(out_f32 and cdt != torch.float32)
        stats = torch.empty(2 * cout, dtype=torch.float64, device=dev)
        abmv = torch.empty(4 * cout, dtype=torch.float32, device=dev)
        nb = L.load().gdmae_conv_block_scratch_bytes(n_in, n_out, cin, cout, a.bf16)
        scratch = torch.empty(nb, dtype=torch.uint8, device=dev)
        a.cols, a.y, a.out, a.stats, a.ab, a.mv = (L.ptr(cols) if packed is None else None, L.ptr(y), L.ptr(out), L.ptr(stats),
                                                   L.ptr(abmv), L.ptr(abmv[2 * cout:]))
        a.scratch = L.ptr(scratch)
        L.call("gdmae_conv_block_fwd", C.byref(a), L.stream())
        ctx.save_for_backward(x, cols, y, stats, abmv, wc, nbr, nbr_t, bn.weight.detach())
        ctx.meta = (a, nb, direct, x.dtype)
        ctx.packed = packed
        return out

    @staticmethod
    def backward(ctx, g):
        x, cols, y, stats, abmv, wc, nbr, nbr_t, gamma = ctx.saved_tensors
        a0, nb, direct, x_dtype = ctx.meta
        a = L.ConvBlockArgs.from_buffer_copy(a0)
        g = g.contiguous()
        assert g.dtype in (torch.float32, y.dtype)
        a.g, a.g_f32 = L.ptr(g), int(g.dtype == torch.float32 and y.dtype != torch.float32)
        dx = torch.empty(x.shape[0], a.cin, dtype=y.dtype, device=x.device) if ctx.needs_input_grad[0] else None
        a.dx = L.ptr(dx) if dx is not None else None
        a.dW, a.dgamma, a.dbeta = (L.ptr(t) for t in direct)
        scratch = torch.empty(nb, dtype=torch.uint8, device=x.device)
        a.scratch = L.ptr(scratch)
        L.call("gdmae_conv_block_bwd", C.byref(a), L.stream())
        return dx, None


def conv_bn_relu(x, conv, bn, nbr, nbr_t, out_f32=False):
    direct = [ops.direct_grad(p) for p in (conv.weight, bn.weight, bn.bias)]
    if any(t is None for t in direct) or not x.is_cuda:
        return None
    return ConvBNReLUFn.apply(x, (conv.weight, bn, nbr, nbr_t, direct, out_f32))
```

### gd-mae_amd/gdmae_hip/lib.py

```python
from __future__ import annotations

import ctypes as C
import os

import torch

_HERE = os.path.dirname(os.path.abspath(__file__))
LIB_PATH = os.path.abspath(os.path.join(_HERE, "..", "csrc", "libgdmae_hip.so"))
if os.environ.get("GDMAE_LIB"):
    LIB_PATH = os.path.abspath(os.environ["GDMAE_LIB"])


class GdmaeHipError(RuntimeError):
    pass


_P, _I, _L, _F, _D, _Z = C.c_void_p, C.c_int, C.c_longlong, C.c_float, C.c_double, C.c_size_t

SIGNATURES = {
    "gdmae_abi_version": (_I, []),
    "gdmae_target_arch": (C.c_char_p, []),
    "gdmae_last_error": (C.c_char_p, []),
    "gdmae_voxelize_workspace_bytes": (_Z, [_L, _I, _I, _I, _I]),
    "gdmae_voxelize": (_I, [_P, _L, _I, _P, _P, _P, _I, _P, _P, _P, _P, _P, _P, _P, _P, _P, _P, _P, _P, _P, _P, _Z, _P]),
    "gdmae_decorate_points": (_I, [_P, _P, _P, _P, _L, _I, _P, _P, _P, _P]),
    "gdmae_vfe_infer": (_I, [_P, _P, _P, _P, _L, _L, _I, _P, _P, _P, _P, _I, _P, _P, _I, _P, _P]),
    "gdmae_vfe_point_layer_workspace_bytes": (_Z, [_I]),
    "gdmae_pillar_major_rows": (_I, [_P, _I, _P, _P, _P, _L, _P, _P, _P]),
    "gdmae_vfe_point_layer_fwd": (_I, [_P, _P, _P, _P, _I, _L, _I, _P, _P, _P, _I, _P, _P, _D, _D, _P, _P, _P, _P, _P, _P, _P, _I, _P, _P]),
    "gdmae_vfe_point_layer_bwd": (_I, [_P, _P, _P, _P, _I, _L, _I, _P, _P, _P, _I, _P, _P, _P, _P, _I, _P, _P, _P, _I, _P, _P]),
    "gdmae_vfe_max_layer_workspace_bytes": (_Z, []),
    "gdmae_vfe_max_layer_fwd": (_I, [_P, _L, _P, _P, _P, _I, _P, _P, _D, _D, _P, _P, _P, _P, _P, _P, _P, _P, _P, _P]),
    "gdmae_vfe_max_layer_bwd": (_I, [_P, _L, _P, _P, _I, _P, _P, _P, _P, _P, _P, _P, _P, _P, _P, _P, _I, _P, _P]),
    "gdmae_vfe_max_layer_fwd_f16": (_I, [_P, _L, _P, _P, _P, _I, _P, _P, _D, _D, _P, _P, _P, _P, _P, _P, _P, _P, _P, _P]),
    "gdmae_vfe_max_layer_bwd_f16": (_I, [_P, _L, _P, _P, _I, _P, _P, _P, _P, _P, _P, _P, _P, _P, _P, _P, _I, _P, _P]),
    "gdmae_fill_rows": (_I, [_P, _L, _I, _I, _P, _P]),
    "gdmae_weighted_mean_finish": (_I, [_P, _P, _L, _P, _P]),
    "gdmae_decoder_region_workspace_bytes": (_Z, [_I, _I]),
    "gdmae_decoder_region_algebra": (_I, [_P, _P, _P, _P, _P, _P, _P, _D, _I, _I, _P, _P, _I, _P, _P, _P, _P, _P, _P]),
    "gdmae_segment_max": (_I, [_P, _P, _P, _I, _I, _P, _P, _P]),
    "gdmae_segment_max_bwd": (_I, [_P, _P, _P, _L, _I, _P, _P]),
    "gdmae_random_mask": (_I, [_P, _P, _I, _D, _P, _P, _P]),
    "gdmae_visible_tokens": (_I, [_P, _P, _P, _L, _L, _P, _P, _P, _P, _P, _P]),
    "gdmae_downsample_tokens": (_I, [_P, _P, _L, _I, _I, _I, _P, _P, _P, _P, _P, _P]),
    "gdmae_rulebook": (_I, [_P, _P, _L, _I, _I, _I, _I, _I, _P, _I, _P, _P]),
    "gdmae_window_workspace_bytes": (_Z, [_I, _I, _I, _I, _I]),
    "gdmae_window_partition": (_I, [_P, _I, _I, _I, _I, _I, _I, _I, _P, _P, _P, _P, _P, _P, _P, _P, _P, _P, _P, _P, _Z, _P]),
    "gdmae_gather_rows": (_I, [_P, _P, _L, _I, _P, _P]),
    "gdmae_scatter_rows": (_I, [_P, _P, _L, _I, _P, _P]),
    "gdmae_gather_rows_strided": (_I, [_P, _P, _L, _I, _I, _I, _P, _P]),
    "gdmae_scatter_rows_strided": (_I, [_P, _P, _L, _I, _I, _I, _P, _P]),
    "gdmae_colstats_workspace_bytes": (_Z, [_I]),
    "gdmae_colstats": (_I, [_P, _L, _I, _I, _P, _P, _P]),
    "gdmae_rows_affine_relu_scatter": (_I, [_P, _I, _P, _L, _I, _P, _P, _P, _I, _I, _I, _P]),
    "gdmae_rows_affine_relu_sub": (_I, [_P, _I, _P, _L, _I, _P, _P, _P, _P, _I, _I, _I, _P]),
    "gdmae_rows_affine_relu_add": (_I, [_P, _I, _L, _I, _P, _P, _P, _P, _I, _P]),
    "gdmae_rows_bwd_stats_workspace_bytes": (_Z, [_I]),
    "gdmae_rows_bwd_stats": (_I, [_P, _I, _P, _L, _I, _P, _P, _P, _I, _I, _I, _P, _P, _P]),
    "gdmae_bn_fold": (_I, [_P, _L, _I, _I, _D, _P, _P, _D, _D, _P, _P, _P, _P, _P, _P, _P, _P]),
    "gdmae_bn_bwd_coeffs": (_I, [_P, _I, _P, _P, _P, _I, _D, _P, _P, _P, _I, _P, _P]),
    "gdmae_rows_bwd_stats_rows": (_I, [_L]),
    "gdmae_bn_bwd_coeffs_rows": (_I, [_P, _I, _I, _P, _P, _P, _I, _D, _P, _P, _P, _I, _P, _P]),
    "gdmae_border_sums_workspace_bytes": (_Z, [_I, _I]),
    "gdmae_border_sums": (_I, [_P, _I, _P, _P, _P, _P, _I, _I, _I, _I, _I, _P, _P, _P]),
    "gdmae_conv3x3_grad_taps": (_I, [_P, _I, _P, _P, _P, _P, _P, _P, _P, _L, _I, _I, _I, _P, _P]),
    "gdmae_decoder_tiles_workspace_bytes": (_Z, [_I, _I, _I]),
    "gdmae_decoder_tiles": (_I, [_P, _P, _I, _I, _I, _I, _P, _P, _P, _P, _P]),
    "gdmae_conv3x3_tiles_packed_bytes": (_Z, [_I]),
    "gdmae_conv3x3_tiles_pack": (_I, [_P, _I, _I, _P, _I, _P, _P, _P, _P]),
    "gdmae_conv3x3_tiles_workspace_bytes": (_Z, [_I]),
    "gdmae_conv3x3_tiles_fwd": (_I, [_P, _P, _P, _P, _P, _I, _P, _P, _P, _I, _I, _I, _I, _P, _P, _P, _D, _D, _P, _P, _P, _P, _P, _P,
                                     _P, _P]),
    "gdmae_tiles_gather_rows": (_I, [_P, _P, _P, _P, _L, _I, _I, _I, _I, _P, _P]),
    "gdmae_tiles_to_dense": (_I, [_P, _P, _P, _I, _I, _I, _I, _I, _P, _P]),
    "gdmae_tiles_to_dense_affine_relu": (_I, [_P, _P, _P, _I, _I, _I, _I, _P, _P, _P, _P]),
    "gdmae_rows_bwd": (_I, [_P, _I, _P, _L, _I, _P, _P, _P, _P, _P, _I, _I, _I, _P, _I, _P]),
    "gdmae_segment_max_affine": (_I, [_P, _I, _P, _P, _I, _I, _P, _P, _P, _P, _P]),
    "gdmae_segmax_bwd_stats": (_I, [_P, _I, _P, _P, _P, _L, _I, _P, _P, _P, _P, _P]),
    "gdmae_segmax_bn_bwd": (_I, [_P, _I, _P, _P, _P, _P, _L, _I, _P, _P, _P, _P, _I, _P]),
    "gdmae_window_attention_fwd": (_I, [_P, _P, _P, _I, _P, _P, _P, _I, _I, _I, _I, _P, _F, _P]),
    "gdmae_window_attention_bwd": (_I, [_P, _P, _P, _P, _P, _I, _P, _P, _P, _P, _I, _I, _I, _I, _P, _F, _P]),
    "gdmae_window_attention_levels_writes_lse": (_I, [_I, _I, _P, _I, _I]),
    "gdmae_window_attention_levels_fwd": (_I, [_P, _P, _P, _I, _P, _P, _P, _I, _P, _P, _I, _I, _P, _F, _P, _P]),
    "gdmae_window_attention_levels_bwd": (_I, [_P, _P, _P, _P, _P, _I, _P, _P, _P, _P, _I, _P, _P, _I, _I, _P, _F, _P, _P, _P]),
    "gdmae_conv3x3_dense_packed_bytes": (_Z, [_I, _I]),
    "gdmae_conv3x3_dense_pack": (_I, [_P, _I, _I, _I, _I, _P, _P]),
    "gdmae_conv3x3_dense": (_I, [_P, _I, _I, _I, _I, _I, _I, _P, _P, _P, _P]),
    "gdmae_conv3x3_dense_add": (_I, [_P, _I, _I, _I, _I, _I, _I, _P, _P, _P, _P, _P]),
    "gdmae_conv3x3_dense_relu": (_I, [_P, _I, _I, _I, _I, _I, _I, _P, _P, _P, _P, _P]),
    "gdmae_conv3x3_dense_stats_workspace_bytes": (_Z, [_I, _I, _I, _I]),
    "gdmae_conv3x3_dense_stat_rows": (_I, []),
    "gdmae_conv3x3_dense_stats": (_I, [_P, _I, _I, _I, _I, _I, _I, _P, _P, _P, _P, _P, _P]),
    "gdmae_bn_fold_partials": (_I, [_P, _I, _I, _D, _P, _P, _D, _D, _P, _P, _P, _P, _P, _P, _P]),
    "gdmae_conv3x3_dense_f32out": (_I, [_P, _I, _I, _I, _I, _I, _I, _P, _P, _P, _I, _P]),
    "gdmae_conv3x3_dense_dw_workspace_bytes": (_Z, [_I, _I, _I, _I, _I]),
    "gdmae_conv3x3_dense_bwd_weight": (_I, [_P, _P, _I, _I, _I, _I, _I, _I, _I, _I, _P, _P, _P]),
    "gdmae_attention_timing": (_I, [_I]),
    "gdmae_attention_timing_read": (_I, [_I, _P, _P]),
    "gdmae_kernel_timing": (_I, [_I]),
    "gdmae_kernel_timing_slots": (_I, []),
    "gdmae_kernel_timing_name": (C.c_char_p, [_I]),
    "gdmae_kernel_timing_read": (_I, [_I, _P, _P, _P, _P]),
    "gdmae_kernel_timing_read_side": (_I, [_I, _P]),
    "gdmae_add_layernorm_workspace_bytes": (_Z, [_I]),
    "gdmae_add_layernorm_fwd": (_I, [_P, _P, _I, _P, _P, _L, _I, _F, _P, _P, _P, _P]),
    "gdmae_add_layernorm_bwd": (_I, [_P, _P, _I, _P, _P, _P, _P, _I, _L, _I, _P, _P, _P, _P, _P]),
    "gdmae_prep_tokens": (_I, [_P, _P, _P, _L, _I, _P, _P, _I, _P]),
    "gdmae_sum_bf16": (_I, [_P, _I, _L, _P, _P]),
    "gdmae_add3": (_I, [_P, _P, _I, _P, _I, _L, _P, _P]),
    "gdmae_add3_to": (_I, [_P, _P, _I, _P, _I, _L, _P, _I, _P]),
    "gdmae_set_attention_impl": (_I, [_I]),
    "gdmae_sum_partials": (_I, [_P, _L, _F, _P, _I, _P]),
    "gdmae_sum_partials_gated": (_I, [_P, _L, _F, _P, _P, _F, _P]),
    "gdmae_gemm_workspace_bytes": (_Z, []),
    "gdmae_gemm_stats": (_I, [_P]),
    "gdmae_gemm_tuning": (_I, [_I]),
    "gdmae_gemm": (_I, [_P, _P, _P, _L, _L, _L, _I, _I, _I, _I, _P, _P, _P]),
    "gdmae_gemm_tn_splitk_workspace_bytes": (_Z, [_L, _I, _I]),
    "gdmae_gemm_tn_splitk": (_I, [_P, _P, _P, _L, _I, _I, _I, _I, _P, _P]),
    "gdmae_conv_block_scratch_bytes": (_Z, [_L, _L, _I, _I, _I]),
    "gdmae_spconv_packed_bytes": (_Z, [_I, _I]),
    "gdmae_spconv_pack_jobs": (_I, [_P, _I, _I, _I, _P, _P]),
    "gdmae_spconv": (_I, [_P, _I, _P, _P, _L, _I, _I, _P, _I, _P]),
    "gdmae_spconv_bias_relu": (_I, [_P, _I, _P, _P, _P, _L, _I, _I, _P, _P]),
    "gdmae_spconv_stat_rows": (_I, [_I, _I, _I]),
    "gdmae_spconv_stats": (_I, [_P, _I, _P, _P, _L, _I, _I, _P, _P, _P]),
    "gdmae_decoder_dy": (_I, [_P, _P, _I, _P, _P, _P, _P, _I, _I, _I, _P, _P]),
    "gdmae_decoder_site_rulebook": (_I, [_P, _P, _I, _L, _P, _I, _I, _P, _P]),
    "gdmae_tap_dw_rows": (_L, [_L, _I, _I]),
    "gdmae_tap_dw_workspace_bytes": (_Z, [_L, _I, _I]),
    "gdmae_tap_dw": (_I, [_P, _L, _L, _I, _P, _P, _I, _P, _I, _I, _P, _P]),
    "gdmae_decoder_block_dw_workspace_bytes": (_Z, [_L, _I]),
    "gdmae_decoder_block_dw": (_I, [_P, _P, _P, _P, _P, _L, _I, _P, _P, _I, _I, _P, _I, _I, _P, _P]),
    "gdmae_conv_block_fwd": (_I, [_P, _P]),
    "gdmae_conv_block_bwd": (_I, [_P, _P]),
    "gdmae_encoder_layer_bytes": (_I, [_L, _I, _I, _I, _I, _P, _P, _P]),
    "gdmae_dw_gemm_workspace_bytes": (_Z, [_L, _I, _I]),
    "gdmae_dw_gemm": (_I, [_P, _P, _L, _I, _I, _P, _P, _P, _P]),
    "gdmae_layer_packed_bytes": (_Z, [_I, _I]),
    "gdmae_layer_pack_jobs": (_I, [_P, _P, _P, _P, _I, _I, _P, _P]),
    "gdmae_layer_pack_job_count": (_I, [_I, _I]),
    "gdmae_tok_gemm_pack": (_I, [_P, _I, _P]),
    "gdmae_tok_gemm": (_I, [_P, _P, _P, _L, _L, _I, _I, _I, _P, _P, _P, _P, _P, _P, _F, _P, _P, _P, _P, _P, _P, _P]),
    "gdmae_tok_gemm_qkv": (_I, [_P, _P, _P, _P, _P, _L, _I, _P, _P, _P]),
    "gdmae_tok_gemm_ffn": (_I, [_P, _P, _P, _P, _P, _L, _L, _I, _P, _P, _P, _P, _F, _P, _P, _P, _P, _P, _P, _P, _P]),
    "gdmae_tok_gemm_ln_bwd_rows": (_I, [_I]),
    "gdmae_tok_gemm_ln_bwd": (_I, [_P, _P, _L, _L, _I, _I, _P, _P, _P, _P, _P, _P, _P, _P, _P, _P]),
    "gdmae_encoder_layer_fwd": (_I, [_P, _P]),
    "gdmae_encoder_layer_bwd": (_I, [_P, _P]),
    "gdmae_encoder_stage_fwd": (_I, [_P, _I, _P]),
    "gdmae_encoder_stage_bwd": (_I, [_P, _I, _P]),
    "gdmae_deconv_rows_packed_bytes": (_Z, [_I, _I, _I]),
    "gdmae_deconv_rows_pack": (_I, [_P, _I, _I, _I, _P, _P, _P]),
    "gdmae_deconv_rows_fwd": (_I, [_P, _L, _I, _I, _I, _P, _P, _P]),
    "gdmae_deconv_rows_bwd_input": (_I, [_P, _L, _I, _I, _I, _P, _P, _P]),
    "gdmae_deconv_rows_dw_workspace_bytes": (_Z, [_L, _I, _I, _I]),
    "gdmae_deconv_rows_bwd_weight": (_I, [_P, _P, _L, _I, _I, _I, _P, _P, _P]),
    "gdmae_pred_head_packed_bytes": (_Z, []),
    "gdmae_pred_head_pack": (_I, [_P, _P, _I, _I, _P, _P]),
    "gdmae_pred_head_fwd": (_I, [_P, _L, _I, _P, _P, _P, _P, _P]),
    "gdmae_pred_head_bwd_workspace_bytes": (_Z, [_L]),
    "gdmae_pred_head_bwd": (_I, [_P, _I, _P, _P, _P, _P, _L, _I, _P, _P, _P, _P, _P, _P]),
    "gdmae_encoder_set_layer_path": (_I, [_I]),
    "gdmae_encoder_stage_fused": (_I, [_P, _I]),
    "gdmae_group_gt_points": (_I, [_P, _I, _P, _P, _P, _I, _I, _P, _P, _P, _P, _P]),
    "gdmae_chamfer": (_I, [_P, _P, _P, _I, _I, _I, _P, _P, _P]),
    "gdmae_augment_collate_workspace_bytes": (_Z, [_L]),
    "gdmae_augment_collate": (_I, [_P, _L, _I, _P, _I, _P, _P, _P, _P, _P, _P]),
    "gdmae_gt_sample_workspace_bytes": (_Z, [_L]),
    "gdmae_gt_sample_select": (_I, [_P, _P, _P, _P, _I, _I, _P, _P, _P, _I, _I, _P, _P, _P, _P, _P, _P]),
    "gdmae_gt_sample_collate": (_I, [_P, _P, _I, _P, _I, _L, _I, _P, _P, _P, _P, _P, _P, _P, _P, _P, _P]),
    "gdmae_group_workspace_bytes": (_Z, [_L, _L]),
    "gdmae_ingroup_inds": (_I, [_P, _L, _L, _P, _P, _Z, _P]),
    "gdmae_group_inner_inds": (_I, [_P, _L, _L, _I, _P, _P, _Z, _P]),
    "gdmae_center_head_targets_workspace_bytes": (_Z, [_I, _I]),
    "gdmae_center_head_targets": (_I, [_P, _I, _I, _I, _P, _I, _I, _P, _P, _F, _I, _I, _I, _D, _I, _P, _P, _P, _P, _P, _P]),
    "gdmae_center_head_targets_iou": (_I, [_P, _I, _I, _I, _P, _I, _I, _P, _P, _F, _I, _I, _I, _D, _I, _P, _P, _P, _P, _P, _P, _P]),
    "gdmae_focal_loss_rows": (_I, []),
    "gdmae_focal_loss_fwd": (_I, [_P, _I, _P, _P, _I, _I, _I, _I, _P, _P, _P, _P]),
    "gdmae_focal_loss_bwd": (_I, [_P, _I, _P, _P, _I, _I, _I, _I, _P, _P, _P, _I, _P]),
    "gdmae_center_head_decode": (_I, [_P, _P, _P, _P, _P, _P, _P, _P, _I, _I, _I, _I, _P, _P, _F, _P, _F, _I, _P, _P, _P, _P, _P]),
    "gdmae_center_head_detect_workspace_bytes": (_Z, [_I, _I, _I]),
    "gdmae_center_head_detect": (_I, [_P] * 8 + [_I] * 4 + [_P, _P, _F, _P, _F, _I, _I, _P, _P, _P, _P, _P, _I, _I] + [_P] * 6),
    "gdmae_anchor_targets_workspace_bytes": (_Z, [_I, _I, _I]),
    "gdmae_anchor_targets": (_I, [_P, _I, _I, _I, _I, _I, _I, _I, _I, _P, _P, _P, _P, _P, _P, _P, _P, _P, _F, _I, _P, _P, _P, _P, _P, _P, _P]),
    "gdmae_anchor_loss_rows": (_I, []),
    "gdmae_anchor_loss_fwd": (_I, [_P, _I, _I, _I, _I, _I, _I, _I, _P, _P, _P, _P, _P, _P, _P, _P, _P]),
    "gdmae_anchor_loss_bwd": (_I, [_P, _I, _I, _I, _I, _I, _I, _I, _P, _P, _P, _P, _P, _P, _P, _P, _P]),
    "gdmae_anchor_decode": (_I, [_P, _I, _I, _I, _I, _I, _I, _I, _I, _P, _P, _P, _F, _F, _P, _P, _P]),
    "gdmae_anchor_select": (_I, [_P, _I, _I, _I, _I, _F, _P, _P, _P, _P, _P]),
    "gdmae_anchor_head_infer_packed_bytes": (_Z, [_I]),
    "gdmae_anchor_head_infer_pack": (_I, [_P, _P, _P, _P, _P, _P, _I, _I, _I, _I, _P, _P]),
    "gdmae_anchor_head_infer_workspace_bytes": (_Z, [_I, _I, _I, _I]),
    "gdmae_anchor_head_infer": (_I, [_P, _I, _I, _I, _I, _I, _I, _I, _P, _P, _P, _P, _F, _F, _F, _P, _P, _P, _P, _P, _P, _P, _P]),
    "gdmae_boxes_bev_pairs": (_I, [_P, _I, _P, _I, _I, _P, _P]),
    "gdmae_nms_workspace_bytes": (_Z, [_I]),
    "gdmae_nms_bev": (_I, [_P, _I, _F, _I, _P, _P, _P, _P]),
    "gdmae_geometry_plan_layout": (_I, [_P, _P, _I, _P, _P]),
    "gdmae_geometry_plan": (_I, [_P, _P, _P, _P, _Z, _P]),
    "gdmae_grad_sq_norm": (_I, [_P, _L, _P, _P, _P]),
    "gdmae_adam_step": (_I, [_P, _P, _P, _P, _P, _I, _F, _F, _F, _F, _F, _I, _F, _F, _P, _P]),
    "gdmae_adam_step_shadow": (_I, [_P, _P, _P, _P, _P, _I, _F, _F, _F, _F, _F, _I, _F, _F, _P, _P, _P]),
    "gdmae_roi_dfvs_pool_workspace_bytes": (_Z, [_L, _I, _I, _I, _I]),
    "gdmae_roi_dfvs_pool": (_I, [_P, _L, _I, _P, _I, _I, _I, _P, _P, _I, _I, _P, _I, _I, _I, _F, _F, _I, _I, _P, _P, _P, _P, _P, _Z, _P]),
    "gdmae_roi_graph_folded_floats": (_Z, []),
    "gdmae_roi_graph_packed_bytes": (_Z, []),
    "gdmae_roi_graph_workspace_bytes": (_Z, [_L]),
    "gdmae_roi_graph_pack": (_I, [_P, _P, _P]),
    "gdmae_roi_graph_forward": (_I, [_P, _P, _P, _I, _P, _I, _I, _I, _P, _P, _P, _P, _P, _P, _P, _Z, _P]),
}

class LayerArgs(C.Structure):
    _fields_ = ([("n", _L), ("d", _I), ("ff", _I), ("nhead", _I), ("bf16", _I), ("eps", _F), ("tau_min", _F), ("n_levels", _I),
                 ("n_win", _I * 4), ("max_tokens", _I * 4)]
                + [(k, _P) for k in ("tok_pos", "csr_tok", "win_start", "win_len", "pos_table", "Win", "bin", "Wo", "bo", "W1", "b1",
                                     "W2", "b2", "g1", "be1", "g2", "be2", "tau", "x", "y", "dy", "dx", "dWin", "dbin", "dtau", "dWo",
                                     "dbo", "dW1", "db1", "dW2", "db2", "dg1", "dbe1", "dg2", "dbe2", "saved", "scratch", "packed")]
                + [("x_bf16", _I), ("res_out", _P), ("dres", _P), ("dx_bf16", _P), ("path", _I)])


class PlanParams(C.Structure):
    _fields_ = [("n_points", _L), ("n_cols", _I), ("batch_size", _I), ("lo", _F * 3), ("vs", _F * 3), ("grid", _I * 3), ("n_stages", _I),
                ("stride", _I * 4), ("win_x", _I * 4), ("win_y", _I * 4), ("n_levels", _I * 4), ("drop_lo", (_I * 3) * 4),
                ("drop_hi", (_I * 3) * 4), ("max_tokens", (_I * 3) * 4), ("masked", _I), ("keep_frac", _D), ("n_dec", _I),
                ("dec_sources", _I * 4), ("want_pm", _I), ("cap_points", _L)]


class PlanBuffer(C.Structure):
    _fields_ = [("name", C.c_char * 40), ("offset", _L), ("bytes", _L)]


class ConvBlockArgs(C.Structure):
    _fields_ = ([("n_in", _L), ("n_out", _L), ("cin", _I), ("cout", _I), ("bf16", _I), ("x_f32", _I), ("g_f32", _I),
                 ("eps", _F), ("momentum", _F)]
                + [(k, _P) for k in ("x", "nbr", "nbr_t", "W", "gamma", "beta", "running_mean", "running_var", "num_batches", "cols",
                                     "y", "stats", "ab", "mv", "out", "g", "dx", "dW", "dgamma", "dbeta", "scratch", "packed_fwd", "packed_bwd")]
                + [("out_f32", _I)])


_lib = None


def load():
    global _lib
    if _lib is not None:
        return _lib
    if not os.path.exists(LIB_PATH):
        raise GdmaeHipError(f"{LIB_PATH} not found - build it with `python -m gdmae_hip.build` "
                            "(__graft_entry__.build()); there is no CPU fallback for the product path")
    lib = C.CDLL(LIB_PATH)
    for name, (res, args) in SIGNATURES.items():
        fn = getattr(lib, name)
        fn.restype = res
        fn.argtypes = args
    _lib = lib
    return lib


def ptr(t):
    if t is None:
        return None
    assert t.is_cuda and t.is_contiguous(), "HIP entry points need contiguous device tensors"
    return t.data_ptr()


_raw_stream = getattr(torch._C, "_cuda_getCurrentRawStream", None)


def stream():
    if _raw_stream is not None:
        return _raw_stream(torch.cuda.current_device())
    return torch.cuda.current_stream().cuda_stream


def call(name, *args):
    lib = load()
    rc = getattr(lib, name)(*args)
    if rc != 0:
        raise GdmaeHipError(f"{name} failed ({rc}): {lib.gdmae_last_error().decode()}")


def host_f32(vals):
    return (C.c_float * len(vals))(*[float(v) for v in vals])


def host_i32(vals):
    return (C.c_int * len(vals))(*[int(v) for v in vals])


def host_i64(vals):
    return (C.c_longlong * len(vals))(*[int(v) for v in vals])


def ptr_any(t):
    assert t.is_cuda
    return t.data_ptr()


def host_ptrs(tensors):
    return (C.c_void_p * len(tensors))(*[ptr(t) for t in tensors])


def host_ptrs_any(tensors):
    return (C.c_void_p * len(tensors))(*[ptr_any(t) for t in tensors])
```

### gd-mae_amd/gdmae_hip/plan.py

```python
from __future__ import annotations

from dataclasses import dataclass, field
from typing import List, Optional

import torch

from . import lib as L

I32 = torch.int32


def _empty(n, dtype, dev):
    return torch.empty(int(n), dtype=dtype, device=dev)


@dataclass
class VoxelPlan:
    batch_size: int
    grid: tuple
    lo: tuple
    vs: tuple
    n_cols: int
    N: int
    M: int
    points: torch.Tensor
    point_coords: torch.Tensor
    inverse: torch.Tensor
    inverse32: torch.Tensor
    voxel_coords: torch.Tensor
    pillar_cell: torch.Tensor
    pt_off: torch.Tensor
    pillar_pts: torch.Tensor
    point_rank: torch.Tensor
    sample_off: torch.Tensor
    pillar_mean: torch.Tensor
    cell2pillar: torch.Tensor
    counts: torch.Tensor
    points_pm: torch.Tensor = None
    row_pillar: torch.Tensor = None


def _voxelize_launch(points: torch.Tensor, point_cloud_range, voxel_size, grid_size, batch_size: int) -> dict:
    assert points.is_cuda and points.dtype == torch.float32 and points.dim() == 2
    points = points.contiguous()
    dev = points.device
    n0, ncols = points.shape
    gx, gy, gz = (int(g) for g in grid_size)
    cells = batch_size * gx * gy * gz
    lo = tuple(float(v) for v in point_cloud_range[:3])
    vs = tuple(float(v) for v in voxel_size)
    F = ncols - 1
    cap = max(n0, 1)
    r = dict(batch_size=batch_size, grid=(gx, gy, gz), lo=lo, vs=vs, ncols=ncols, n0=n0, src=points,
             pts_out=_empty(cap * ncols, torch.float32, dev), pcoords=_empty(cap * 4, torch.int64, dev),
             inverse=_empty(cap, torch.int64, dev), inverse32=_empty(cap, I32, dev), vcoords=_empty(cap * 4, torch.int64, dev),
             pillar_cell=_empty(cap, I32, dev), pt_off=_empty(cap + 1, I32, dev), pillar_pts=_empty(cap, I32, dev),
             prank=_empty(cap, I32, dev), sample_off=_empty(batch_size + 1, I32, dev), mean=_empty(cap * F, torch.float32, dev),
             cell2pillar=_empty(cells, I32, dev), counts=_empty(2, I32, dev))
    wsb = L.load().gdmae_voxelize_workspace_bytes(n0, batch_size, gx, gy, gz)
    r["ws"] = _empty(wsb, torch.uint8, dev)
    L.call("gdmae_voxelize", L.ptr(points), n0, ncols, L.host_f32(lo), L.host_f32(vs), L.host_i32((gx, gy, gz)),
           batch_size, L.ptr(r["pts_out"]), L.ptr(r["pcoords"]), L.ptr(r["inverse"]), L.ptr(r["inverse32"]), L.ptr(r["vcoords"]),
           L.ptr(r["pillar_cell"]), L.ptr(r["pt_off"]), L.ptr(r["pillar_pts"]), L.ptr(r["prank"]), L.ptr(r["sample_off"]),
           L.ptr(r["mean"]), L.ptr(r["cell2pillar"]), L.ptr(r["counts"]), L.ptr(r["ws"]), wsb, L.stream())
    r["pts_pm"] = _empty(cap * ncols, torch.float32, dev)
    r["row_pillar"] = _empty(cap, I32, dev)
    L.call("gdmae_pillar_major_rows", L.ptr(r["pts_out"]), ncols, L.ptr(r["pillar_pts"]), L.ptr(r["inverse32"]), L.ptr(r["counts"]),
           cap, L.ptr(r["pts_pm"]), L.ptr(r["row_pillar"]), L.stream())
    return r


def _voxelize_finalize(r: dict, N: int, M: int) -> VoxelPlan:
    ncols = r["ncols"]
    F = ncols - 1
    return VoxelPlan(r["batch_size"], r["grid"], r["lo"], r["vs"], ncols, N, M,
                     r["pts_out"][:N * ncols].view(N, ncols), r["pcoords"][:N * 4].view(N, 4), r["inverse"][:N],
                     r["inverse32"][:N], r["vcoords"][:M * 4].view(M, 4), r["pillar_cell"][:M], r["pt_off"][:M + 1],
                     r["pillar_pts"][:N], r["prank"][:N], r["sample_off"], r["mean"][:M * F].view(M, F), r["cell2pillar"],
                     r["counts"], r["pts_pm"][:N * ncols].view(N, ncols), r["row_pillar"][:N])


def voxelize(points: torch.Tensor, point_cloud_range, voxel_size, grid_size, batch_size: int) -> VoxelPlan:
    r = _voxelize_launch(points, point_cloud_range, voxel_size, grid_size, batch_size)
    N, M = (int(v) for v in r["counts"].tolist())
    return _voxelize_finalize(r, N, M)


@dataclass
class WindowPlan:
    tok_win: torch.Tensor
    tok_level: torch.Tensor
    tok_slot: torch.Tensor
    tok_pos: torch.Tensor
    csr_tok: torch.Tensor
    win_start: torch.Tensor
    win_len: torch.Tensor
    n_win: List[int] = field(default_factory=list)
    n_tok: List[int] = field(default_factory=list)
    max_tokens: List[int] = field(default_factory=list)


@dataclass
class StagePlan:
    B: int
    Y: int
    X: int
    n_tok: int
    tok_cell: torch.Tensor
    map: torch.Tensor
    nbr_subm: torch.Tensor
    nbr_down: Optional[torch.Tensor]
    nbr_down_t: Optional[torch.Tensor]
    windows: List[WindowPlan] = field(default_factory=list)

    def indices_byx(self) -> torch.Tensor:
        c = self.tok_cell.long()
        x = c % self.X
        r = c // self.X
        return torch.stack([r // self.Y, r % self.Y, x], dim=-1).int()


@dataclass
class DecoderTiles:
    sources: tuple
    B: int
    H: int
    W: int
    n_act: int
    tile_slot: torch.Tensor
    tile_list: torch.Tensor
    nbr: Optional[list] = None


@dataclass
class EncoderPlan:
    mask: Optional[torch.Tensor]
    tok_pillar: torch.Tensor
    stages: List[StagePlan]
    dec_tiles: Optional[DecoderTiles] = None


def upsample_cells(c: torch.Tensor, Ys: int, Xs: int, s: int) -> torch.Tensor:
    x = c % Xs
    r = torch.div(c, Xs, rounding_mode='floor')
    y = r % Ys
    b = torch.div(r, Ys, rounding_mode='floor')
    d = torch.arange(s, device=c.device, dtype=c.dtype)
    yy = (y * s).view(-1, 1, 1) + d.view(1, s, 1)
    xx = (x * s).view(-1, 1, 1) + d.view(1, 1, s)
    return ((b.view(-1, 1, 1) * (Ys * s) + yy) * (Xs * s) + xx).reshape(c.numel(), s * s)


def _drop_arrays(drop_info):
    d = {int(k): v for k, v in drop_info.items()}
    keys = sorted(d)
    assert keys == list(range(len(keys))) and len(keys) <= 3
    lo = [int(d[k]["drop_range"][0]) for k in keys]
    hi = [int(d[k]["drop_range"][1]) for k in keys]
    T = [int(d[k]["max_tokens"]) for k in keys]
    return lo, hi, T


def _decoder_tiles_launch(maps, ups, B, H, W, dev) -> dict:
    nt = B * ((H + 7) // 8) * ((W + 7) // 8)
    r = dict(tile_slot=_empty(nt, I32, dev), tile_list=_empty(nt, I32, dev), n_act=_empty(1, I32, dev), B=B, H=H, W=W)
    ws = _empty(L.load().gdmae_decoder_tiles_workspace_bytes(B, H, W), torch.uint8, dev)
    L.call("gdmae_decoder_tiles", L.host_ptrs(maps), L.host_i32(ups), len(maps), B, H, W, L.ptr(r["tile_slot"]),
           L.ptr(r["tile_list"]), L.ptr(r["n_act"]), L.ptr(ws), L.stream())
    r["_ws"] = ws
    return r


def decoder_tiles(ep: "EncoderPlan", sources, H: int, W: int) -> DecoderTiles:
    sources = tuple(int(v) for v in sources)
    dt = ep.dec_tiles
    if dt is not None and dt.sources == sources and dt.H == H and dt.W == W:
        return dt
    st = [ep.stages[i] for i in sources]
    B = st[0].B
    ups = [H // sp.Y for sp in st]
    assert all(sp.Y * u == H and sp.X * u == W for sp, u in zip(st, ups))
    r = _decoder_tiles_launch([sp.map for sp in st], ups, B, H, W, st[0].map.device)
    n = int(r["n_act"].item())
    ep.dec_tiles = DecoderTiles(sources, B, H, W, n, r["tile_slot"], r["tile_list"][:n])
    ep.dec_tiles.nbr = _site_rulebooks(ep.dec_tiles, st, ups)
    return ep.dec_tiles


def decoder_site_rulebooks(dt: "DecoderTiles", sites, ups, n_tok=None):
    out = []
    for g, (st, u) in enumerate(zip(sites, ups)):
        n_dev = torch.tensor([st.numel() // (u * u) if n_tok is None else n_tok[g]], dtype=I32, device=st.device)
        nbr = _empty(st.numel() * 9, I32, st.device)
        L.call("gdmae_decoder_site_rulebook", L.ptr(st.contiguous()), L.ptr(n_dev), u * u, st.numel(), L.ptr(dt.tile_slot), dt.H, dt.W,
               L.ptr(nbr), L.stream())
        out.append(nbr.view(-1, 9))
    return out


def _site_rulebooks(dt: "DecoderTiles", stages, ups):
    sites = (sp.tok_cell if u == 1 else (sp._up_sites[1] if getattr(sp, "_up_sites", None) is not None and sp._up_sites[0] == u
                                         else upsample_cells(sp.tok_cell, sp.Y, sp.X, u).reshape(-1).contiguous())
             for sp, u in zip(stages, ups))
    return decoder_site_rulebooks(dt, sites, ups, [sp.n_tok for sp in stages])


def _encoder_launch(vox, m_cap: int, strides, window_shapes, drop_infos, keep_frac, noise, dec_sources=None) -> dict:
    if isinstance(vox, dict):
        dev, grid, B = vox["src"].device, vox["grid"], vox["batch_size"]
        sample_off, pillar_cell, vcounts = vox["sample_off"], vox["pillar_cell"], vox["counts"]
    else:
        dev, grid, B = vox.points.device, vox.grid, vox.batch_size
        sample_off, pillar_cell, vcounts = vox.sample_off, vox.pillar_cell, vox.counts
    gx, gy, gz = grid
    assert gz == 1, "the SST backbone works on single-layer pillar grids (spt_backbone_mae.py:94)"
    lib = L.load()
    st = L.stream()
    M = m_cap
    scan_ws = _empty(8 * (max(B * gx * gy, M) // 4096 + 4), torch.int64, dev)

    if keep_frac is not None:
        if noise is None:
            noise = torch.rand(max(M, 1), device=dev, dtype=torch.float32)
        assert noise.numel() >= 1 and noise.dtype == torch.float32
        mask = _empty(max(M, 1), torch.float32, dev)
        len_keep = _empty(B, I32, dev)
        L.call("gdmae_random_mask", L.ptr(noise.contiguous()), L.ptr(sample_off), B, float(keep_frac), L.ptr(mask),
               L.ptr(len_keep), st)
    else:
        mask = torch.zeros(max(M, 1), dtype=torch.float32, device=dev)

    cap = max(M, 1)
    Y, X = gy, gx
    tok_pillar = _empty(cap, I32, dev)
    tok_cell = _empty(cap, I32, dev)
    smap = _empty(B * Y * X, I32, dev)
    n_tok = _empty(1, I32, dev)
    L.call("gdmae_visible_tokens", L.ptr(mask), L.ptr(pillar_cell), L.ptr(vcounts), M, B * Y * X,
           L.ptr(tok_pillar), L.ptr(tok_cell), L.ptr(smap), L.ptr(n_tok), L.ptr(scan_ws), st)

    raw = []
    for si, stride in enumerate(strides):
        if stride > 1:
            assert stride == 2, "only the k3 s2 p1 strided sparse conv of the shipped configs is implemented"
            Yi, Xi = Y, X
            Y, X = (Yi - 1) // 2 + 1, (Xi - 1) // 2 + 1
            cap_in = cap
            cap = min(4 * cap_in, B * Y * X)
            tok_cell_n = _empty(cap, I32, dev)
            smap_n = _empty(B * Y * X, I32, dev)
            n_tok_n = _empty(1, I32, dev)
            flag = _empty(B * Y * X, I32, dev)
            L.call("gdmae_downsample_tokens", L.ptr(n_tok), L.ptr(tok_cell), cap_in, B, Yi, Xi, L.ptr(tok_cell_n),
                   L.ptr(smap_n), L.ptr(n_tok_n), L.ptr(flag), L.ptr(scan_ws), st)
            nbr_down = _empty(cap * 9, I32, dev)
            L.call("gdmae_rulebook", L.ptr(n_tok_n), L.ptr(tok_cell_n), cap, B, Y, X, Yi, Xi, L.ptr(smap), 1,
                   L.ptr(nbr_down), st)
            nbr_down_t = _empty(cap_in * 9, I32, dev)
            L.call("gdmae_rulebook", L.ptr(n_tok), L.ptr(tok_cell), cap_in, B, Yi, Xi, Y, X, L.ptr(smap_n), 2,
                   L.ptr(nbr_down_t), st)
            tok_cell, smap, n_tok = tok_cell_n, smap_n, n_tok_n
        else:
            nbr_down = nbr_down_t = None
        nbr_subm = _empty(cap * 9, I32, dev)
        L.call("gdmae_rulebook", L.ptr(n_tok), L.ptr(tok_cell), cap, B, Y, X, Y, X, L.ptr(smap), 0, L.ptr(nbr_subm), st)
        wx, wy, wz = (int(v) for v in window_shapes[si])
        assert wz == 1
        dlo, dhi, dT = _drop_arrays(drop_infos[si])
        assert wx * wy <= max(dT), "token drop would not be the identity: unsupported (SURVEY header item 5)"
        wsb = lib.gdmae_window_workspace_bytes(B, Y, X, wx, wy)
        wins = []
        for shifted in (0, 1):
            nwin_cap = B * ((X + wx - 1) // wx + 1) * ((Y + wy - 1) // wy + 1)
            w = dict(tok_win=_empty(cap, I32, dev), tok_level=_empty(cap, I32, dev), tok_slot=_empty(cap, I32, dev),
                     tok_pos=_empty(cap, I32, dev), csr_tok=_empty(cap, I32, dev),
                     win_start=_empty(min(nwin_cap, cap), I32, dev), win_len=_empty(min(nwin_cap, cap), I32, dev),
                     counts=_empty(8, I32, dev), T=dT)
            ws = _empty(wsb, torch.uint8, dev)
            L.call("gdmae_window_partition", L.ptr(smap), B, Y, X, wx, wy, shifted, len(dT), L.host_i32(dlo),
                   L.host_i32(dhi), L.host_i32(dT), L.ptr(w["tok_win"]), L.ptr(w["tok_level"]), L.ptr(w["tok_slot"]),
                   L.ptr(w["tok_pos"]), L.ptr(w["csr_tok"]), L.ptr(w["win_start"]), L.ptr(w["win_len"]),
                   L.ptr(w["counts"]), L.ptr(ws), wsb, st)
            w["_ws"] = ws
            wins.append(w)
        nbr_subm_t = torch.flip(nbr_subm.view(cap, 9), dims=[1]).contiguous().view(-1)
        up_s = gy // Y
        up_sites = upsample_cells(tok_cell, Y, X, up_s) if (up_s > 1 and up_s * Y == gy and up_s * X == gx) else None
        raw.append(dict(B=B, Y=Y, X=X, cap=cap, tok_cell=tok_cell, map=smap, n_tok=n_tok, nbr_subm=nbr_subm,
                        nbr_subm_t=nbr_subm_t, up_s=up_s, up_sites=up_sites, nbr_down=nbr_down, nbr_down_t=nbr_down_t, wins=wins))
    dec = None
    if dec_sources is not None:
        srcs = [raw[int(i)] for i in dec_sources]
        if all(r["up_s"] * r["Y"] == gy and r["up_s"] * r["X"] == gx and r["up_s"] in (1, 2, 4, 8) for r in srcs):
            dec = _decoder_tiles_launch([r["map"] for r in srcs], [r["up_s"] for r in srcs], B, gy, gx, dev)
            dec["sources"] = tuple(int(i) for i in dec_sources)
    counts = torch.cat([r["n_tok"] for r in raw] + [w["counts"] for r in raw for w in r["wins"]]
                       + ([dec["n_act"]] if dec is not None else []))
    return dict(stages=raw, mask=mask, tok_pillar=tok_pillar, masked=keep_frac is not None, counts=counts,
                keep=(noise, scan_ws), dec=dec)


def _encoder_finalize(e: dict, allc, M: int) -> EncoderPlan:
    raw = e["stages"]
    ns = len(raw)
    stages = []
    for si, r in enumerate(raw):
        n = int(allc[si])
        wps = []
        for k, w in enumerate(r["wins"]):
            c = allc[ns + 8 * (2 * si + k): ns + 8 * (2 * si + k) + 8]
            assert c[7] == n, (c, n)
            nw = int(c[6])
            wps.append(WindowPlan(w["tok_win"][:n], w["tok_level"][:n], w["tok_slot"][:n], w["tok_pos"][:n],
                                  w["csr_tok"][:n], w["win_start"][:nw], w["win_len"][:nw],
                                  [int(v) for v in c[0:3]], [int(v) for v in c[3:6]], list(w["T"])))
        n_prev = int(allc[si - 1]) if r["nbr_down"] is not None else 0
        stages.append(StagePlan(r["B"], r["Y"], r["X"], n, r["tok_cell"][:n], r["map"],
                                r["nbr_subm"][:n * 9].view(n, 9),
                                None if r["nbr_down"] is None else r["nbr_down"][:n * 9].view(n, 9),
                                None if r["nbr_down_t"] is None else r["nbr_down_t"][:n_prev * 9].view(n_prev, 9),
                                wps))
        stages[-1]._nbr_subm_t = r["nbr_subm_t"][:n * 9].view(n, 9)
        stages[-1]._up_sites = None if r["up_sites"] is None else (r["up_s"], r["up_sites"][:n].reshape(-1))
    dec = e.get("dec", None)
    dt = None
    if dec is not None:
        n_act = int(allc[ns + 16 * ns])
        dt = DecoderTiles(dec["sources"], dec["B"], dec["H"], dec["W"], n_act, dec["tile_slot"], dec["tile_list"][:n_act])
    return EncoderPlan(e["mask"][:M] if e["masked"] else None, e["tok_pillar"][:stages[0].n_tok], stages, dt)


def encoder_plan(vox: VoxelPlan, strides, window_shapes, drop_infos, keep_frac: Optional[float] = None,
                 noise: Optional[torch.Tensor] = None, dec_sources=None) -> EncoderPlan:
    if noise is not None:
        assert noise.shape == (vox.M,)
    e = _encoder_launch(vox, vox.M, strides, window_shapes, drop_infos, keep_frac, noise, dec_sources)
    return _encoder_finalize(e, e["counts"].tolist(), vox.M)


import collections
import time as _time

EVENT_WAIT_S = 0.0

_PLAN_SHAPES = collections.OrderedDict()
_PLAN_SHAPES_MAX = 32
_PLAN_GRANULE = 16384
_PINNED = {}


def _plan_shape(n0, ncols, B, pcr, voxel_size, grid_size, strides, window_shapes, drop_infos, keep_frac, dec_sources):
    gx, gy, gz = (int(g) for g in grid_size)
    lo = tuple(float(v) for v in pcr[:3])
    vs = tuple(float(v) for v in voxel_size)
    drops = tuple(tuple(map(tuple, _drop_arrays(d))) for d in drop_infos)
    n_exact = n0
    n0 = max(1, (n0 + _PLAN_GRANULE - 1) // _PLAN_GRANULE) * _PLAN_GRANULE
    key = (n0, ncols, B, lo, vs, (gx, gy, gz), tuple(int(s) for s in strides), tuple(tuple(int(v) for v in w) for w in window_shapes),
           drops, None if keep_frac is None else float(keep_frac), None if dec_sources is None else tuple(int(i) for i in dec_sources))
    hit = _PLAN_SHAPES.get(key)
    if hit is not None:
        _PLAN_SHAPES.move_to_end(key)
        return hit
    del n_exact
    import ctypes as C
    ns = len(strides)
    assert gz == 1, "the SST backbone works on single-layer pillar grids (spt_backbone_mae.py:94)"
    assert 1 <= ns <= 4
    P = L.PlanParams()
    P.n_points, P.cap_points, P.n_cols, P.batch_size = n0, n0, ncols, B
    for i in range(3):
        P.lo[i], P.vs[i] = lo[i], vs[i]
        P.grid[i] = (gx, gy, gz)[i]
    P.n_stages = ns
    geo = []
    Y, X = gy, gx
    cap = max(1, min(n0, B * gx * gy))
    m_cap = cap
    for i in range(ns):
        wx, wy, wz = (int(v) for v in window_shapes[i])
        assert wz == 1
        dlo, dhi, dT = drops[i]
        assert wx * wy <= max(dT), "token drop would not be the identity: unsupported (SURVEY header item 5)"
        P.stride[i], P.win_x[i], P.win_y[i], P.n_levels[i] = int(strides[i]), wx, wy, len(dT)
        for l in range(len(dT)):
            P.drop_lo[i][l], P.drop_hi[i][l], P.max_tokens[i][l] = dlo[l], dhi[l], dT[l]
        cap_in = cap
        if int(strides[i]) > 1:
            assert int(strides[i]) == 2, "only the k3 s2 p1 strided sparse conv of the shipped configs is implemented"
            Y, X = (Y - 1) // 2 + 1, (X - 1) // 2 + 1
            cap = min(4 * cap, B * Y * X)
        us = gy // Y
        up_s = us if (us >= 1 and us * Y == gy and us * X == gx) else 0
        geo.append(dict(Y=Y, X=X, cap=cap, cap_in=cap_in, up_s=up_s, strided=int(strides[i]) > 1, T=list(dT)))
    P.masked = int(keep_frac is not None)
    P.keep_frac = float(keep_frac) if keep_frac is not None else 1.0
    P.n_dec = 0 if dec_sources is None else len(dec_sources)
    for g in range(P.n_dec):
        P.dec_sources[g] = int(dec_sources[g])
    P.want_pm = 1
    table = (L.PlanBuffer * 160)()
    n_ent, total = C.c_int(0), C.c_size_t(0)
    L.call("gdmae_geometry_plan_layout", C.byref(P), table, 160, C.byref(n_ent), C.byref(total))
    names = {table[i].name.decode(): (int(table[i].offset), int(table[i].bytes)) for i in range(n_ent.value)}
    hit = _PLAN_SHAPES[key] = (P, names, int(total.value), geo, m_cap, (lo, vs, (gx, gy, gz)))
    while len(_PLAN_SHAPES) > _PLAN_SHAPES_MAX:
        _PLAN_SHAPES.popitem(last=False)
    return hit


class _Arena:

    def __init__(self, raw, names):
        self.raw, self.names = raw, names
        self.base = {torch.int32: raw.view(torch.int32), torch.float32: raw.view(torch.float32), torch.int64: raw.view(torch.int64)}

    def has(self, name):
        return name in self.names

    def view(self, name, dtype, *shape):
        off, _ = self.names[name]
        es = 8 if dtype == torch.int64 else 4
        strides, acc = [], 1
        for d in reversed(shape):
            strides.append(acc)
            acc *= int(d)
        return self.base[dtype].as_strided(tuple(int(d) for d in shape), tuple(reversed(strides)), off // es)


class PlanPrefetch:

    _side = {}
    _arena_bytes = {}

    def __init__(self, points, point_cloud_range, voxel_size, grid_size, batch_size, strides, window_shapes, drop_infos,
                 keep_frac=None, noise=None, ready=None, dec_sources=None):
        import ctypes as C
        assert points.is_cuda and points.dtype == torch.float32 and points.dim() == 2
        points = points.contiguous()
        dev = points.device
        main = torch.cuda.current_stream(dev)
        side = PlanPrefetch._side.setdefault(dev.index, torch.cuda.Stream(device=dev))
        side.wait_stream(main)
        if ready is not None:
            side.wait_event(ready)
        points.record_stream(side)
        if noise is not None:
            noise.record_stream(side)
        n0, ncols = points.shape
        P, names, total, geo, m_cap, _ = self.shape = _plan_shape(n0, ncols, int(batch_size), point_cloud_range, voxel_size, grid_size,
                                                                    strides, window_shapes, drop_infos, keep_frac, dec_sources)
        self.masked, self.dec_sources, self.batch_size, self.ncols = keep_frac is not None, dec_sources, int(batch_size), ncols
        with torch.cuda.stream(side):
            cap = PlanPrefetch._arena_bytes.get(dev.index, 0)
            if total > cap:
                cap = PlanPrefetch._arena_bytes[dev.index] = -(-total // (64 << 20)) * (64 << 20)
            raw = torch.empty(cap, dtype=torch.uint8, device=dev)
            if self.masked and noise is None:
                noise = torch.rand(m_cap, device=dev, dtype=torch.float32)
            if noise is not None:
                assert noise.dtype == torch.float32 and noise.numel() >= 1
                noise = noise.contiguous()
            Pc = L.PlanParams.from_buffer_copy(P)
            Pc.n_points = n0
            L.call("gdmae_geometry_plan", C.byref(Pc), L.ptr(points), None if noise is None else L.ptr(noise), L.ptr(raw), total, L.stream())
            self.arena = _Arena(raw, names)
            nc = names["counts"][1] // 4
            assert nc <= 256
            free = _PINNED.setdefault(dev.index, [])
            self._pinned = free.pop() if free else torch.empty(256, dtype=torch.int32).pin_memory()
            self.host = self._pinned[:nc]
            self.host.copy_(self.arena.view("counts", torch.int32, nc), non_blocking=True)
            self.event = torch.cuda.Event()
            self.event.record(side)
        self.side, self.keep, self.points = side, noise, points
        self.serial = side == main

    def finish(self):
        assert self.serial or torch.cuda.current_stream() != self.side, "plan tensors must not be consumed on the plan stream"
        global EVENT_WAIT_S
        t_w = _time.perf_counter()
        self.event.synchronize()
        EVENT_WAIT_S += _time.perf_counter() - t_w
        torch.cuda.current_stream().wait_event(self.event)
        c = self.host.tolist()
        self.points_device = self.points.device
        self.host = None
        if self._pinned is not None:
            _PINNED.setdefault(self.points_device.index, []).append(self._pinned)
            self._pinned = None
        P, names, total, geo, m_cap, (lo, vs, grid) = self.shape
        A, V = self.arena, self.arena.view
        i32, f32, i64 = torch.int32, torch.float32, torch.int64
        B, ncols = self.batch_size, self.ncols
        F = ncols - 1
        N, M = int(c[0]), int(c[1])
        gx, gy, gz = grid
        vox = VoxelPlan(B, grid, lo, vs, ncols, N, M, V("points", f32, N, ncols), V("point_coords", i64, N, 4), V("inverse", i64, N),
                        V("inverse32", i32, N), V("voxel_coords", i64, M, 4), V("pillar_cell", i32, M), V("pt_off", i32, M + 1),
                        V("pillar_pts", i32, N), V("point_rank", i32, N), V("sample_off", i32, B + 1), V("pillar_mean", f32, M, F),
                        V("cell2pillar", i32, B * gx * gy * gz), V("counts", i32, 2), V("points_pm", f32, N, ncols), V("row_pillar", i32, N))
        vox._arena = A
        ns = len(geo)
        n_vis = int(c[2 + ns + 16 * ns + 1])
        stages = []
        for i, g in enumerate(geo):
            n = int(c[2 + i])
            pre = f"s{i}."
            wps = []
            for k in range(2):
                wc = c[2 + ns + 16 * i + 8 * k: 2 + ns + 16 * i + 8 * k + 8]
                assert wc[7] == n, (wc, n)
                nw = int(wc[6])
                wpre = f"{pre}w{k}."
                wps.append(WindowPlan(V(wpre + "tok_win", i32, n), V(wpre + "tok_level", i32, n), V(wpre + "tok_slot", i32, n),
                                      V(wpre + "tok_pos", i32, n), V(wpre + "csr_tok", i32, n), V(wpre + "win_start", i32, nw),
                                      V(wpre + "win_len", i32, nw), [int(v) for v in wc[0:3]], [int(v) for v in wc[3:6]], list(g["T"])))
            n_prev = (int(c[2 + i - 1]) if i > 0 else n_vis) if g["strided"] else 0
            sp = StagePlan(B, g["Y"], g["X"], n, V(pre + "tok_cell", i32, n), V(pre + "map", i32, B * g["Y"] * g["X"]),
                           V(pre + "nbr_subm", i32, n, 9), V(pre + "nbr_down", i32, n, 9) if g["strided"] else None,
                           V(pre + "nbr_down_t", i32, n_prev, 9) if g["strided"] else None, wps)
            sp._nbr_subm_t = V(pre + "nbr_subm_t", i32, n, 9)
            sp._up_sites = (g["up_s"], V(pre + "up_sites", i32, n * g["up_s"] * g["up_s"])) if g["up_s"] > 1 else None
            stages.append(sp)
        dt = None
        if A.has("dec.tile_slot"):
            n_act = int(c[2 + ns + 16 * ns])
            nt = B * ((gy + 7) // 8) * ((gx + 7) // 8)
            nbrs = [V(f"dec.nbr{g}", i32, stages[int(si)].n_tok * geo[int(si)]["up_s"] ** 2, 9) for g, si in enumerate(self.dec_sources)]
            dt = DecoderTiles(tuple(int(i) for i in self.dec_sources), B, gy, gx, n_act, V("dec.tile_slot", i32, nt), V("dec.tile_list", i32, n_act),
                              nbrs)
        ep = EncoderPlan(V("mask", f32, M) if self.masked else None, V("tok_pillar", i32, stages[0].n_tok if not geo[0]["strided"] else n_vis),
                         stages, dt)
        self.arena = self.points = self.keep = None
        return vox, ep


def _tensors_of(obj):
    out = []
    if isinstance(obj, torch.Tensor):
        if obj.is_cuda:
            out.append(obj)
    elif isinstance(obj, dict):
        for v in obj.values():
            out += _tensors_of(v)
    elif isinstance(obj, (list, tuple)):
        for v in obj:
            out += _tensors_of(v)
    return out
```

### gd-mae_amd/pcdet/utils/spconv_utils.py

```python
from __future__ import annotations

import math
import os
import types
from typing import Set

import torch
import torch.nn as nn

from gdmae_hip import ops


class SparseConvTensor:
    def __init__(self, features, plan, stage: int):
        self.features = features
        self._plan = plan
        self._stage = stage

    @property
    def stage_plan(self):
        return self._plan.stages[self._stage]

    @property
    def indices(self):
        return self.stage_plan.indices_byx()

    @property
    def spatial_shape(self):
        sp = self.stage_plan
        return [sp.Y, sp.X]

    @property
    def batch_size(self):
        return self.stage_plan.B

    def replace_feature(self, f):
        return SparseConvTensor(f, self._plan, self._stage)

    def dense(self, channels_last: bool = True):
        sp = self.stage_plan
        flat = ops.ScatterToDense.apply(self.features, sp.tok_cell, sp.B * sp.Y * sp.X)
        return flat.view(sp.B, sp.Y, sp.X, -1).permute(0, 3, 1, 2)


class SparseModule(nn.Module):
    pass


class SparseConvolution(SparseModule):
    def __init__(self, in_channels, out_channels, kernel_size, stride=1, padding=0, bias=False, indice_key=None, subm=False):
        super().__init__()
        if bias or kernel_size != 3 or (not subm and (stride != 2 or padding != 1)):
            raise NotImplementedError("hot path uses SubMConv2d(k3) and SparseConv2d(k3, s2, p1) without bias only")
        self.in_channels, self.out_channels, self.subm, self.indice_key = in_channels, out_channels, subm, indice_key
        self.weight = nn.Parameter(torch.empty(out_channels, 3, 3, in_channels))
        nn.init.kaiming_uniform_(self.weight, a=math.sqrt(5))

    def rulebooks(self, x: SparseConvTensor):
        if self.subm:
            sp = x.stage_plan
            if getattr(sp, "_nbr_subm_t", None) is None:
                sp._nbr_subm_t = torch.flip(sp.nbr_subm, dims=[1]).contiguous()
            return sp.nbr_subm, sp._nbr_subm_t, x._stage
        nxt = x._plan.stages[x._stage + 1]
        return nxt.nbr_down, nxt.nbr_down_t, x._stage + 1

    def forward(self, x: SparseConvTensor) -> SparseConvTensor:
        nbr, nbr_t, stage = self.rulebooks(x)
        f = ops.SparseConv3x3.apply(x.features, self.weight, nbr, nbr_t)
        return x.replace_feature(f) if stage == x._stage else SparseConvTensor(f, x._plan, stage)


class SubMConv2d(SparseConvolution):
    def __init__(self, in_channels, out_channels, kernel_size, bias=False, indice_key=None, **kw):
        super().__init__(in_channels, out_channels, kernel_size, 1, kernel_size // 2, bias, indice_key, subm=True)


class SparseConv2d(SparseConvolution):
    def __init__(self, in_channels, out_channels, kernel_size, stride=1, padding=0, bias=False, indice_key=None, **kw):
        super().__init__(in_channels, out_channels, kernel_size, stride, padding, bias, indice_key, subm=False)


class SparseSequential(SparseModule):
    fused_bn_relu = True
    native_block = os.environ.get("GDMAE_CONV_BLOCK", "1") != "0"
    out_fp32 = False

    def __init__(self, *mods):
        super().__init__()
        for i, m in enumerate(mods):
            self.add_module(str(i), m)

    def forward(self, x):
        mods = list(self._modules.values())
        if (self.fused_bn_relu and self.training and len(mods) == 3 and isinstance(mods[1], nn.BatchNorm1d)
                and isinstance(mods[2], nn.ReLU) and mods[1].affine):
            from gdmae_hip import convblock, vfe as gvfe
            conv, bn = mods[0], mods[1]
            if self.native_block and isinstance(conv, SparseConvolution):
                nbr, nbr_t, stage = conv.rulebooks(x)
                f = convblock.conv_bn_relu(x.features, conv, bn, nbr, nbr_t, self.out_fp32)
                if f is not None:
                    return x.replace_feature(f) if stage == x._stage else SparseConvTensor(f, x._plan, stage)
            x = conv(x)
            f, _, _ = gvfe.BNReLURows.apply(x.features, bn.weight, bn.bias, bn.eps, bn)
            return x.replace_feature(f)
        for m in mods:
            x = m(x) if isinstance(m, SparseModule) else x.replace_feature(m(x.features))
        return x


spconv = types.SimpleNamespace(SparseConvTensor=SparseConvTensor, SparseModule=SparseModule, SubMConv2d=SubMConv2d,
                               SparseConv2d=SparseConv2d, SparseSequential=SparseSequential,
                               conv=types.SimpleNamespace(SparseConvolution=SparseConvolution))


def find_all_spconv_keys(model: nn.Module, prefix="") -> Set[str]:
    found: Set[str] = set()
    for name, child in model.named_children():
        p = f"{prefix}.{name}" if prefix else name
        if isinstance(child, SparseConvolution):
            found.add(f"{p}.weight")
        found.update(find_all_spconv_keys(child, prefix=p))
    return found


def replace_feature(out, new_features):
    return out.replace_feature(new_features)


def post_act_block(in_channels, out_channels, kernel_size, indice_key=None, stride=1, padding=0, conv_type='subm',
                   norm_fn=None, dim=2):
    if dim != 2:
        raise NotImplementedError("only 2-D sparse convolutions are on the GD-MAE hot path")
    if conv_type == 'subm':
        conv = SubMConv2d(in_channels, out_channels, kernel_size, bias=False, indice_key=indice_key)
    elif conv_type == 'spconv':
        conv = SparseConv2d(in_channels, out_channels, kernel_size, stride=stride, padding=padding, bias=False,
                            indice_key=indice_key)
    else:
        raise NotImplementedError(conv_type)
    return SparseSequential(conv, norm_fn(out_channels), nn.ReLU())
```

### include/gdmae_hip.h

```cpp
#ifndef GDMAE_HIP_H
#define GDMAE_HIP_H

#include <stddef.h>
#include <stdint.h>

#ifdef __cplusplus
extern "C" {
#endif

int gdmae_abi_version(void);
const char* gdmae_target_arch(void);
const char* gdmae_last_error(void);

size_t gdmae_voxelize_workspace_bytes(long long n_points, int batch_size, int gx, int gy, int gz);
int gdmae_voxelize(const float* points, long long n_points, int n_cols, const float* lo, const float* vs,
                   const int* grid_xyz, int batch_size, float* points_out, long long* point_coords,
                   long long* inverse, int* inverse32, long long* voxel_coords, int* pillar_cell,
                   int* pillar_pt_off, int* pillar_pts, int* point_rank, int* sample_pillar_off,
                   float* pillar_mean, int* cell2pillar, int* counts, void* workspace, size_t workspace_bytes,
                   void* stream);

int gdmae_decorate_points(const float* points, const long long* point_coords, const int* inverse32,
                          const float* pillar_mean, long long N, int n_cols, const float* lo, const float* vs,
                          float* out, void* stream);
int gdmae_pillar_major_rows(const float* points, int n_cols, const int* pillar_pts, const int* inverse32, const int* n_dev,
                            long long capacity, float* points_pm, int* row_pillar, void* stream);
int gdmae_vfe_infer(const float* points_pm, const long long* voxel_coords, const int* row_pillar, const float* pillar_mean,
                    long long N, long long M, int n_cols, const float* lo, const float* vs, const float* W1, const float* b1,
                    int c1, const float* W2, const float* b2, int c2, float* out, void* stream);
size_t gdmae_vfe_point_layer_workspace_bytes(int n_cols);
int gdmae_vfe_point_layer_fwd(const float* points, const long long* point_coords, const int* inverse32,
                              const float* pillar_mean, int coords_per_pillar, long long N, int n_cols, const float* lo,
                              const float* vs,
                              const float* W, int C, const float* gamma, const float* beta, double eps, double momentum,
                              float* running_mean, float* running_var, long long* num_batches, double* stats, float* ab,
                              float* mv, void* out, int out_bf16, void* workspace, void* stream);
int gdmae_vfe_point_layer_bwd(const float* points, const long long* point_coords, const int* inverse32,
                              const float* pillar_mean, int coords_per_pillar, long long N, int n_cols, const float* lo,
                              const float* vs,
                              const float* W, int C, const float* gamma, const double* stats, const float* ab,
                              const void* g, int g_bf16, float* dgamma, float* dbeta, float* dW, int accumulate,
                              void* workspace, void* stream);
size_t gdmae_vfe_max_layer_workspace_bytes(void);
int gdmae_vfe_max_layer_fwd(const void* y1, long long N, const void* W, const int* pillar_pt_off, const int* row_pillar,
                            int M, const float* gamma, const float* beta, double eps, double momentum,
                            float* running_mean, float* running_var, long long* num_batches, double* stats, float* ab,
                            float* mv, float* out, int* arg, void* workspace, void* stream);
int gdmae_vfe_max_layer_bwd(const void* y1, long long N, const void* W, const int* row_pillar, int M, const float* gamma,
                            const double* stats, const float* ab, const float* out, const int* arg, const float* g, void* gm,
                            void* dy1, float* dgamma, float* dbeta, float* dW, int accumulate,
                            void* workspace, void* stream);
int gdmae_vfe_max_layer_fwd_f16(const void* y1, long long N, const float* W, const int* pillar_pt_off, const int* row_pillar,
                                int M, const float* gamma, const float* beta, double eps, double momentum,
                                float* running_mean, float* running_var, long long* num_batches, double* stats, float* ab,
                                float* mv, float* out, int* arg, void* workspace, void* stream);
int gdmae_vfe_max_layer_bwd_f16(const void* y1, long long N, const float* W, const int* row_pillar, int M, const float* gamma,
                                const double* stats, const float* ab, const float* out, const int* arg, const float* g, void* gm,
                                void* dy1, float* dgamma, float* dbeta, float* dW, int accumulate,
                                void* workspace, void* stream);
int gdmae_segment_max(const float* x, const int* pillar_pt_off, const int* pillar_pts, int M, int C, float* out,
                      int* arg, void* stream);
int gdmae_segment_max_bwd(const float* dout, const int* arg, const int* inverse32, long long N, int C, float* dx,
                          void* stream);

int gdmae_random_mask(const float* noise, const int* sample_pillar_off, int batch_size, double keep_frac,
                      float* mask_out, int* len_keep_out, void* stream);

int gdmae_visible_tokens(const float* mask, const int* pillar_cell, const int* vox_counts, long long m_cap,
                         long long n_cells, int* tok_pillar, int* tok_cell, int* map, int* n_tok, void* scan_ws,
                         void* stream);
int gdmae_downsample_tokens(const int* n_in, const int* tok_cell_in, long long cap_in, int B, int Yi, int Xi,
                            int* tok_cell_out, int* map_out, int* n_out, int* flag_ws, void* scan_ws, void* stream);
int gdmae_rulebook(const int* n_tok, const int* tok_cell, long long cap, int B, int Yt, int Xt, int Ym, int Xm,
                   const int* map, int mode, int* nbr, void* stream);

size_t gdmae_window_workspace_bytes(int B, int Y, int X, int wx, int wy);
int gdmae_window_partition(const int* map, int B, int Y, int X, int wx, int wy, int shifted, int nlev,
                           const int* drop_lo, const int* drop_hi, const int* max_tokens, int* tok_win,
                           int* tok_level, int* tok_slot, int* tok_pos, int* csr_tok, int* win_start, int* win_len,
                           int* counts, void* workspace, size_t workspace_bytes, void* stream);

int gdmae_gather_rows(const void* src, const int* idx, long long n_slots, int row_bytes, void* out, void* stream);
int gdmae_scatter_rows(const void* src, const int* idx, long long n_rows, int row_bytes, void* dst, void* stream);

int gdmae_gather_rows_strided(const void* src, const int* idx, long long n_slots, int row_bytes, int table_row_bytes,
                              int table_col_bytes, void* out, void* stream);
int gdmae_scatter_rows_strided(const void* src, const int* idx, long long n_rows, int row_bytes, int table_row_bytes,
                               int table_col_bytes, void* dst, void* stream);
size_t gdmae_colstats_workspace_bytes(int C);
int gdmae_colstats(const void* x, long long R, int C, int is_bf16, double* out, void* workspace, void* stream);

size_t gdmae_decoder_region_workspace_bytes(int C2, int Cin);
int gdmae_decoder_region_algebra(const double* stats2, const float* ab2, const double* st2, const float* k01,
                                 const double* reg, const double* tap_region, const double* cnt, double R, int C2, int Cin,
                                 const float* conv_w, const void* bgz, int cdt_bf16, double* S, double* tot, float* dWk,
                                 void* Wd, void* workspace, void* stream);
int gdmae_fill_rows(const void* v, long long R, int C, int elem_bytes, void* Z, void* stream);
int gdmae_rows_affine_relu_scatter(const void* P, int p_bf16, const int* site, long long n, int C, const float* a,
                                   const float* b, void* Z, int z_bf16, int z_row_elems, int col0, void* stream);
int gdmae_rows_affine_relu_sub(const void* P, int p_bf16, const int* site, long long n, int C, const float* a, const float* b,
                               const void* sub, void* Z, int z_bf16, int z_row_elems, int col0, void* stream);
int gdmae_rows_affine_relu_add(const void* P, int p_bf16, long long n, int C, const float* a, const float* b, const void* R, void* Z,
                               int z_bf16, void* stream);
size_t gdmae_rows_bwd_stats_workspace_bytes(int C);
int gdmae_rows_bwd_stats(const void* P, int p_bf16, const int* site, long long n, int C, const float* a, const float* b,
                         const void* dZ, int z_bf16, int z_row_elems, int col0, double* out, void* workspace, void* stream);
int gdmae_rows_bwd(const void* P, int p_bf16, const int* site, long long n, int C, const float* a, const float* b,
                   const float* c0, const float* c1, const void* dZ, int z_bf16, int z_row_elems, int col0, void* dP,
                   int dp_bf16, void* stream);

int gdmae_bn_fold(const void* x, long long R, int C, int is_bf16, double count, const float* gamma, const float* beta,
                  double eps, double momentum, float* running_mean, float* running_var, long long* num_batches,
                  double* stats, float* ab, float* mv, void* workspace, void* stream);
int gdmae_bn_fold_partials(const float* part, int nblk, int C, double count, const float* gamma, const float* beta, double eps,
                           double momentum, float* running_mean, float* running_var, long long* num_batches, double* stats, float* ab,
                           float* mv, void* stream);
int gdmae_bn_bwd_coeffs(const double* st, int n_st, const double* stats, const float* ab, const float* gamma, int C,
                        double count, const double* tot, float* dgamma, float* dbeta, int accumulate, float* c01,
                        void* stream);
int gdmae_rows_bwd_stats_rows(long long n);
int gdmae_bn_bwd_coeffs_rows(const float* part, int nblk, int n_st, const double* stats, const float* ab, const float* gamma, int C,
                             double count, const double* tot, float* dgamma, float* dbeta, int accumulate, float* c01,
                             void* stream);

int gdmae_conv3x3_grad_taps(const void* Y, int y_bf16, const int* tile_slot, const void* ybg, const float* k0,
                            const float* k1, const float* rows, const int* cell2pillar, const int* site, long long n, int H,
                            int W, int C, void* out, void* stream);

size_t gdmae_border_sums_workspace_bytes(int B, int C);
int gdmae_border_sums(const void* Y, int y_bf16, const int* tile_slot, const void* ybg, const float* rows,
                      const int* pillar_cell, int M, int B, int H, int W, int C, double* out, void* workspace, void* stream);

size_t gdmae_decoder_tiles_workspace_bytes(int B, int H, int W);
int gdmae_decoder_tiles(const int* const* maps, const int* strides, int k, int B, int H, int W, int* tile_slot, int* tile_list,
                        int* n_act, void* workspace, void* stream);
size_t gdmae_conv3x3_tiles_packed_bytes(int k);
int gdmae_conv3x3_tiles_pack(const float* conv_w, int C2, int Cin, const float* const* b, int k, void* Wp, void* bgz, void* ybg,
                             void* stream);
size_t gdmae_conv3x3_tiles_workspace_bytes(int n_act);
int gdmae_conv3x3_tiles_fwd(const void* const* P, const int* const* maps, const float* const* a, const float* const* b,
                            const int* strides, int k, const void* Wp, const void* ybg, const int* tile_list, int n_act, int B,
                            int H, int W, void* Yc, const float* gamma, const float* beta, double eps, double momentum,
                            float* running_mean, float* running_var, long long* num_batches, double* stats, float* ab,
                            float* mv, void* workspace, void* stream);
int gdmae_tiles_gather_rows(const void* Yc, const int* tile_slot, const void* ybg, const int* cell, long long n, int H, int W,
                            int C, int elem_bytes, void* out, void* stream);
int gdmae_tiles_to_dense(const void* Yc, const int* tile_slot, const void* ybg, int B, int H, int W, int C, int elem_bytes,
                         void* out, void* stream);
int gdmae_tiles_to_dense_affine_relu(const void* Yc, const int* tile_slot, const void* ybg, int B, int H, int W, int C, const float* a,
                                     const float* b, float* out, void* stream);

int gdmae_segment_max_affine(const void* x, int x_bf16, const int* pillar_pt_off, const int* pillar_pts, int M, int C,
                             const float* a, const float* b, float* out, int* arg, void* stream);
int gdmae_segmax_bwd_stats(const void* x, int x_bf16, const float* out, const int* arg, const float* dout, long long M,
                           int C, const float* a ,
                           const float* b, double* sums, void* workspace, void* stream);
int gdmae_segmax_bn_bwd(const void* x, int x_bf16, const float* out, const int* arg, const float* dout,
                        const int* inverse32, long long N, int C, const float* a, const float* c0, const float* c1,
                        void* dx, int dx_bf16, void* stream);

int gdmae_set_attention_impl(int impl);
int gdmae_window_attention_fwd(const void* qk, const void* v, void* out, int io_bf16, const int* csr_tok,
                               const int* win_start, const int* win_len, int n_win, int T, int d, int H,
                               const float* tau, float tau_min, void* stream);
int gdmae_window_attention_bwd(const void* qk, const void* v, const void* dout, void* dqk, void* dv, int io_bf16,
                               float* dtau_part, const int* csr_tok, const int* win_start, const int* win_len,
                               int n_win, int T, int d, int H, const float* tau, float tau_min, void* stream);
int gdmae_window_attention_levels_writes_lse(int io_bf16, int n_levels, const int* max_tokens, int d, int H);
int gdmae_window_attention_levels_fwd(const void* qk, const void* v, void* out, int io_bf16, const int* csr_tok,
                                      const int* win_start, const int* win_len, int n_levels, const int* n_win,
                                      const int* max_tokens, int d, int H, const float* tau, float tau_min, float* lse, void* stream);
int gdmae_window_attention_levels_bwd(const void* qk, const void* v, const void* dout, void* dqk, void* dv, int io_bf16,
                                      float* dtau_part, const int* csr_tok, const int* win_start, const int* win_len,
                                      int n_levels, const int* n_win, const int* max_tokens, int d, int H, const float* tau,
                                      float tau_min, const void* out, const float* lse, void* stream);
int gdmae_attention_timing(int on);
int gdmae_attention_timing_read(int which, double* total_ms, long long* calls);
int gdmae_kernel_timing(int on);
int gdmae_kernel_timing_slots(void);
const char* gdmae_kernel_timing_name(int slot);
int gdmae_kernel_timing_read(int slot, double* total_ms, long long* calls, double* bytes, double* flops);
int gdmae_kernel_timing_read_side(int slot, double* side_bytes);
int gdmae_weighted_mean_finish(const float* term, const float* weights, long long n, float* out, void* stream);
int gdmae_sum_partials(const float* part, long long n, float scale, float* out, int accumulate, void* stream);
int gdmae_sum_partials_gated(const float* part, long long n, float scale, float* out, const float* gate, float gate_min,
                             void* stream);

size_t gdmae_add_layernorm_workspace_bytes(int d);
int gdmae_add_layernorm_fwd(const float* a, const void* b, int b_is_bf16, const float* gamma, const float* beta,
                            long long n, int d, float eps, float* y, float* stats, void* y_bf16 ,
                            void* stream);
int gdmae_add_layernorm_bwd(const float* a, const void* b, int b_is_bf16, const float* gamma, const float* stats,
                            const float* dy, const void* dy2, int dy2_bf16, long long n, int d, float* dx, void* dx_bf16,
                            float* sums, void* workspace, void* stream);
int gdmae_prep_tokens(const float* x, const float* pos_table, const int* tok_pos, long long n, int d, void* x_out,
                      void* xpos_out, int out_bf16, void* stream);
int gdmae_sum_bf16(const void* const* src, int k, long long total, void* out, void* stream);
int gdmae_add3(const float* a, const void* b, int b_bf16, const void* c, int c_bf16, long long total, float* out, void* stream);
int gdmae_add3_to(const float* a, const void* b, int b_bf16, const void* c, int c_bf16, long long total, void* out, int out_bf16,
                  void* stream);

int gdmae_gemm_stats(long long* calls);
int gdmae_gemm_tuning(int mode);
size_t gdmae_gemm_workspace_bytes(void);
int gdmae_gemm(const void* A, const void* B, void* C, long long M, long long N, long long K, int trans_a, int trans_b,
               int ab_bf16, int c_f32, const void* bias, void* workspace, void* stream);
size_t gdmae_gemm_tn_splitk_workspace_bytes(long long K, int m, int n);
int gdmae_gemm_tn_splitk(const void* A, const void* B, float* C, long long K, int m, int n, int ab_bf16, int accumulate,
                         void* workspace, void* stream);

size_t gdmae_dw_gemm_workspace_bytes(long long rows, int M, int N);
int gdmae_dw_gemm(const void* G, const void* X, long long rows, int M, int N, float* dW, float* dbias, void* workspace,
                  void* stream);

typedef struct gdmae_conv_block_args {
  long long n_in, n_out;
  int cin, cout, bf16, x_f32, g_f32;
  float eps, momentum;
  const void* x;
  const int* nbr;
  const int* nbr_t;
  const void* W;
  const float *gamma, *beta;
  float *running_mean, *running_var;
  long long* num_batches;
  void* cols;
  void* y;
  double* stats;
  float* ab;
  float* mv;
  void* out;
  const void* g;
  void* dx;
  float *dW, *dgamma, *dbeta;
  void* scratch;
  const void* packed_fwd;
  const void* packed_bwd;
  int out_f32;
} gdmae_conv_block_args;
size_t gdmae_conv_block_scratch_bytes(long long n_in, long long n_out, int cin, int cout, int bf16);
size_t gdmae_spconv_packed_bytes(int cin, int cout);
int gdmae_spconv_pack_jobs(const float* W , int cin, int cout, int transposed, void* packed, long long* jobs);
int gdmae_spconv(const void* X, int x_f32, const int* nbr, const void* packed, long long n, int cin, int cout, void* Y,
                 int timing_slot , void* stream);
int gdmae_spconv_bias_relu(const void* X, int x_f32, const int* nbr, const void* packed, const float* bias, long long n, int cin, int cout,
                           void* Y, void* stream);
int gdmae_spconv_stat_rows(int cin, int cout, int x_f32);
int gdmae_spconv_stats(const void* X, int x_f32, const int* nbr, const void* packed, long long n, int cin, int cout, void* Y, float* part,
                       void* stream);
int gdmae_decoder_dy(const void* Yc, const int* tile_list, int n_act, const float* k0, const float* k1, const float* rows,
                     const int* cell2pillar, int H, int W, int C, void* dYc, void* stream);
int gdmae_decoder_site_rulebook(const int* site, const int* n_dev, int sites_per_tok, long long cap_sites, const int* tile_slot,
                                int H, int W, int* nbr, void* stream);
long long gdmae_tap_dw_rows(long long n, int M, int N);
size_t gdmae_tap_dw_workspace_bytes(long long n, int M, int N);
int gdmae_tap_dw(const void* G, long long n, long long n_pad, int M, const void* X, const int* nbr, int N, float* out, int ld_out,
                 int m_off, void* workspace, void* stream);
size_t gdmae_decoder_block_dw_workspace_bytes(long long n, int u);
int gdmae_decoder_block_dw(const void* P, const float* a, const float* b, const void* bg, const int* site, long long n, int u,
                           const void* dYc, const int* tile_slot, int H, int W, float* out, int ld_out, int m_off, void* workspace,
                           void* stream);
int gdmae_conv_block_fwd(const gdmae_conv_block_args* args , void* stream);
int gdmae_conv_block_bwd(const gdmae_conv_block_args* args , void* stream);

typedef struct gdmae_layer_args {
  long long n;
  int d, ff, nhead, bf16;
  float eps, tau_min;
  int n_levels;
  int n_win[4], max_tokens[4];
  const int* tok_pos;
  const int* csr_tok;
  const int* win_start;
  const int* win_len;
  const float* pos_table;
  const void *Win, *bin, *Wo, *bo, *W1, *b1, *W2, *b2;
  const float *g1, *be1, *g2, *be2, *tau;
  const float* x;
  float* y;
  const float* dy;
  float* dx;
  float *dWin, *dbin, *dtau, *dWo, *dbo, *dW1, *db1, *dW2, *db2, *dg1, *dbe1, *dg2, *dbe2;
  void* saved;
  void* scratch;
  const void* packed;
  int x_bf16;
  void* res_out;
  const void* dres;
  void* dx_bf16;
  int path;
} gdmae_layer_args;
size_t gdmae_layer_packed_bytes(int d, int ff);
int gdmae_layer_pack_jobs(const float* Win, const float* Wo, const float* W1, const float* W2, int d, int ff, void* packed,
                          long long* jobs_host );
int gdmae_layer_pack_job_count(int d, int ff);
int gdmae_tok_gemm_pack(const long long* jobs_dev, int n_jobs, void* stream);
int gdmae_tok_gemm(const void* X, const void* Wp, const void* bias, long long n, long long n_pad, int K, int N, int epilogue,
                   void* out0, void* out1, const void* aux, const float* res, const float* gamma, const float* beta, float eps,
                   float* y, float* stats, void* y_bf16, const float* pos_table, const int* tok_pos, void* ypos_bf16,
                   void* stream);

int gdmae_tok_gemm_qkv(const void* Xpos, const void* X, const void* Wp_qk, const void* Wp_v, const void* bias3, long long n_pad,
                       int d, void* qk, void* v, void* stream);

int gdmae_tok_gemm_ffn(const void* X, const void* W1p, const void* b1, const void* W2p, const void* b2, long long n, long long n_pad,
                       int d, void* h, const float* res, const float* gamma, const float* beta, float eps, float* y, float* stats,
                       void* y_bf16, const float* pos_table, const int* tok_pos, void* ypos_bf16, void* f_out, void* stream);

int gdmae_tok_gemm_ln_bwd_rows(int N);
int gdmae_tok_gemm_ln_bwd(const void* X, const void* Wp, long long n, long long n_pad, int K, int N, const float* dy,
                          const void* dy2_bf16, const float* ln_a, const void* ln_b_bf16, const float* stats,
                          const float* gamma, float* dx, void* dx_bf16, float* part, void* stream);
int gdmae_encoder_layer_bytes(long long n, int d, int ff, int nhead, int bf16, size_t* saved_bytes,
                              size_t* fwd_scratch_bytes, size_t* bwd_scratch_bytes);
int gdmae_encoder_layer_fwd(const gdmae_layer_args* args , void* stream);
int gdmae_encoder_layer_bwd(const gdmae_layer_args* args , void* stream);
int gdmae_encoder_stage_fwd(const gdmae_layer_args* layers , int n_layers, void* stream);
int gdmae_encoder_stage_bwd(const gdmae_layer_args* layers , int n_layers, void* stream);
int gdmae_encoder_set_layer_path(int path);
int gdmae_encoder_stage_fused(const gdmae_layer_args* layers , int n_layers);

size_t gdmae_deconv_rows_packed_bytes(int cin, int cout, int s);
int gdmae_deconv_rows_pack(const float* weight, int cin, int cout, int s, void* packed_fwd, void* packed_bwd, void* stream);
int gdmae_deconv_rows_fwd(const void* X, long long n, int cin, int cout, int s, const void* packed_fwd, void* P, void* stream);
int gdmae_deconv_rows_bwd_input(const void* dP, long long n, int cin, int cout, int s, const void* packed_bwd, void* dX, void* stream);
size_t gdmae_deconv_rows_dw_workspace_bytes(long long n, int cin, int cout, int s);
int gdmae_deconv_rows_bwd_weight(const void* X, const void* dP, long long n, int cin, int cout, int s, float* dW, void* workspace,
                                 void* stream);

size_t gdmae_pred_head_packed_bytes(void);
int gdmae_pred_head_pack(const float* weight, const float* bias, int n_in, int n_out, void* packed, void* stream);
int gdmae_pred_head_fwd(const float* X, long long n, int n_out, const void* packed, void* Y, void* X_bf16 , float* Y_f32 ,
                        void* stream);
size_t gdmae_pred_head_bwd_workspace_bytes(long long n);
int gdmae_pred_head_bwd(const void* dY, int dy_f32 ,
                        void* dY_bf16 ,
                        const float* scale_a, const float* scale_b ,
                        const void* X_bf16, long long n, int n_out,
                        const void* packed, float* dX, float* dW, float* db, void* workspace, void* stream);

size_t gdmae_conv3x3_dense_packed_bytes(int cin, int cout);
int gdmae_conv3x3_dense_pack(const float* weight, int cin, int cout, int dil, int transposed, void* packed, void* stream);
int gdmae_conv3x3_dense(const void* X, int B, int H, int W, int cin_l, int cout_l, int dil, const void* packed, const float* bias,
                        void* Y, void* stream);
int gdmae_conv3x3_dense_add(const void* X, int B, int H, int W, int cin_l, int cout_l, int dil, const void* packed, const float* bias,
                            const void* addend, void* Y, void* stream);
int gdmae_conv3x3_dense_relu(const void* X, int B, int H, int W, int cin_l, int cout_l, int dil, const void* packed, const float* bias,
                             const void* shortcut, void* Y, void* stream);
size_t gdmae_conv3x3_dense_stats_workspace_bytes(int B, int H, int W, int cout_l);
int gdmae_conv3x3_dense_stat_rows(void);
int gdmae_conv3x3_dense_stats(const void* X, int B, int H, int W, int cin_l, int cout_l, int dil, const void* packed, const float* bias,
                              void* Y, float* stat_rows, void* workspace, void* stream);
int gdmae_conv3x3_dense_f32out(const void* X, int B, int H, int W, int cin_l, int cout_l, int dil, const void* packed, const float* bias,
                               float* Y, int accumulate, void* stream);
size_t gdmae_conv3x3_dense_dw_workspace_bytes(int B, int H, int W, int cin_l, int cout_l);
int gdmae_conv3x3_dense_bwd_weight(const void* X, const void* dY, int B, int H, int W, int cin_l, int cout_l, int cin, int cout, int dil,
                                   float* dW, void* workspace, void* stream);

int gdmae_group_gt_points(const float* points, int n_cols, const int* pillar_pt_off, const int* pillar_pts,
                          const long long* voxel_coords, int M, int K, const float* lo, const float* vs,
                          float* gt_points, int* gt_index, void* stream);
int gdmae_chamfer(const float* pred, const float* gt, const float* weights, int M, int P1, int P2, float* term,
                  float* dpred, void* stream);

size_t gdmae_augment_collate_workspace_bytes(long long n_raw);
int gdmae_augment_collate(const float* raw, long long n_raw, int F, const int* frame_off, int B, const float* frame_params,
                          const float* xy_range , float* out, int* kept_off, void* workspace, void* stream);

size_t gdmae_gt_sample_workspace_bytes(long long n_rows);
int gdmae_gt_sample_select(const float* boxes, const int* frame_desc_host, const int* frame_desc, const int* cand_group, int B,
                           int n_groups, const float* frame_params, const float* range ,
                           const float* extra_width , int min_corners, int cap, int* valid, float* rm_boxes,
                           int* n_valid, float* gt_boxes, int* num_gt, void* stream);
int gdmae_gt_sample_collate(const float* raw, const float* db, int F, const int* seg, int S, long long n_rows, int B,
                            const float* frame_params, const float* boxes, const int* valid, const float* rm_boxes,
                            const int* n_valid, const float* xy_range , float* out, int* kept_off, void* workspace,
                            void* stream);

size_t gdmae_group_workspace_bytes(long long n, long long n_groups);
int gdmae_ingroup_inds(const long long* group_inds, long long n, long long n_groups, long long* out_inds,
                       void* workspace, size_t workspace_bytes, void* stream);
int gdmae_group_inner_inds(const long long* inverse_inds, long long n, long long M, int K, long long* group_inds,
                           void* workspace, size_t workspace_bytes, void* stream);

#define GDMAE_PLAN_MAX_STAGES 4
typedef struct gdmae_plan_params {
  long long n_points;
  int n_cols, batch_size;
  float lo[3], vs[3];
  int grid[3];
  int n_stages;
  int stride[GDMAE_PLAN_MAX_STAGES];
  int win_x[GDMAE_PLAN_MAX_STAGES], win_y[GDMAE_PLAN_MAX_STAGES];
  int n_levels[GDMAE_PLAN_MAX_STAGES];
  int drop_lo[GDMAE_PLAN_MAX_STAGES][3], drop_hi[GDMAE_PLAN_MAX_STAGES][3], max_tokens[GDMAE_PLAN_MAX_STAGES][3];
  int masked;
  double keep_frac;
  int n_dec;
  int dec_sources[GDMAE_PLAN_MAX_STAGES];
  int want_pm;
  long long cap_points;
} gdmae_plan_params;
typedef struct gdmae_plan_buffer {
  char name[40];
  long long offset, bytes;
} gdmae_plan_buffer;
int gdmae_geometry_plan_layout(const gdmae_plan_params* p, gdmae_plan_buffer* table, int max_entries, int* n_entries,
                               size_t* total_bytes);
int gdmae_geometry_plan(const gdmae_plan_params* p, const float* points, const float* noise, void* arena, size_t arena_bytes,
                        void* stream);

size_t gdmae_center_head_targets_workspace_bytes(int B, int num_max_objs);
int gdmae_center_head_targets(const float* gt_boxes, int B, int n_max, int box_dim, const int* class_map, int n_class_total,
                              int n_cls, const float* pc_range , const float* voxel_size ,
                              float feature_map_stride, int fw, int fh, int num_max_objs, double gaussian_overlap, int min_radius,
                              float* heatmap, float* ret_boxes, long long* inds, long long* mask, void* workspace, void* stream);
int gdmae_focal_loss_rows(void);
int gdmae_focal_loss_fwd(const void* logits, int logits_bf16, const long long* strides_byxc, const float* gt, int B, int C, int H, int W,
                         float* prob, float* partials, float* out4, void* stream);
int gdmae_focal_loss_bwd(const void* logits, int logits_bf16, const long long* strides_byxc, const float* gt, int B, int C, int H, int W,
                         const float* out4, const float* grad_out, void* dlogits, int dlogits_bf16, void* stream);
int gdmae_center_head_targets_iou(const float* gt_boxes, int B, int n_max, int box_dim, const int* class_map, int n_class_total,
                                  int n_cls, const float* pc_range, const float* voxel_size, float feature_map_stride, int fw, int fh,
                                  int num_max_objs, double gaussian_overlap, int min_radius, float* heatmap, float* ret_boxes,
                                  float* iou_boxes, long long* inds, long long* mask, void* workspace, void* stream);
int gdmae_center_head_decode(const long long* cell, const float* score, const float* center, const float* center_z,
                             const float* dim, const float* rot, const float* vel, const float* iou, int B, int K, int H, int W,
                             const float* pc_range , const float* voxel_size ,
                             float feature_map_stride, const float* post_center_limit_range , float score_thresh,
                             int use_score_thresh, float* boxes, int* labels, float* ious, unsigned char* valid, void* stream);
size_t gdmae_center_head_detect_workspace_bytes(int B, int K, int box_dim);
int gdmae_center_head_detect(const long long* cell, const float* score, const float* center, const float* center_z, const float* dim,
                             const float* rot, const float* vel, const float* iou, int B, int K, int H, int W, const float* pc_range,
                             const float* voxel_size, float feature_map_stride, const float* post_center_limit_range, float score_thresh,
                             int use_score_thresh, int C, const float* thresh, const int* pre_max, const int* post_max,
                             const float* rectifier, const int* to_global, int class_aware, int n_out, float* boxes, float* scores,
                             long long* labels, int* count, void* workspace, void* stream);

int gdmae_boxes_bev_pairs(const float* boxes_a, int n, const float* boxes_b, int m, int mode, float* out, void* stream);
size_t gdmae_nms_workspace_bytes(int n);
int gdmae_nms_bev(const float* boxes, int n, float thresh, int rotated, long long* keep, int* n_keep, void* workspace,
                  void* stream);

size_t gdmae_anchor_targets_workspace_bytes(int B, int n_cls, int n_max);
int gdmae_anchor_targets(const float* gt_boxes, int B, int n_max, int box_dim, int H, int W, int K, int n_cls, int n_names,
                         const int* name_idx, const int* slot_cls, const float* xr, const float* yr, const float* xc, const float* yc,
                         const float* slot, const float* matched, const float* unmatched, float dir_offset, int num_bins,
                         int* labels, int* gt_ids, float* reg_targets, int* dir_bins, int* num_pos, void* workspace, void* stream);
int gdmae_anchor_loss_rows(void);
int gdmae_anchor_loss_fwd(const void* rows, int rows_bf16, int ld, int B, int n_loc, int K, int C, int nb, const int* labels,
                          const float* reg_targets, const int* dir_bins, const int* num_pos, const float* code_weights,
                          const float* scale, float* partials, float* out4, void* stream);
int gdmae_anchor_loss_bwd(const void* rows, int rows_bf16, int ld, int B, int n_loc, int K, int C, int nb, const int* labels,
                          const float* reg_targets, const int* dir_bins, const int* num_pos, const float* code_weights,
                          const float* scale, const float* grad3, void* drows, void* stream);
int gdmae_anchor_decode(const void* rows, int rows_bf16, int ld, int B, int H, int W, int K, int C, int nb, const float* xc,
                        const float* yc, const float* slot, float dir_offset, float dir_limit_offset, float* cls_out, float* boxes,
                        void* stream);
int gdmae_anchor_select(const float* cls, int B, int n, int C, int normalized, float thresh, int* idx, float* score, int* label,
                        int* count, void* stream);

size_t gdmae_anchor_head_infer_packed_bytes(int cin);
int gdmae_anchor_head_infer_pack(const float* w_cls, const float* b_cls, const float* w_box, const float* b_box, const float* w_dir,
                                 const float* b_dir, int cin, int K, int C, int nb, void* packed, void* stream);
size_t gdmae_anchor_head_infer_workspace_bytes(int B, int H, int W, int K);
int gdmae_anchor_head_infer(const void* X, int B, int H, int W, int cin, int K, int C, int nb, const void* packed, const float* xc,
                            const float* yc, const float* slot, float dir_offset, float dir_limit_offset, float thresh,
                            float* rows_out, int* count, int* idx, float* score, int* label, float* box, void* workspace,
                            void* stream);

int gdmae_grad_sq_norm(const float* grad, long long n, float* partials , float* sq_norm_out, void* stream);
int gdmae_adam_step(float* param, const float* grad, float* exp_avg, float* exp_avg_sq, const long long* segments,
                    int n_segments, float lr, float beta1, float beta2, float eps, float weight_decay, int step,
                    float max_norm, float grad_scale, const float* sq_norm, void* stream);
int gdmae_adam_step_shadow(float* param, const float* grad, float* exp_avg, float* exp_avg_sq, const long long* segments,
                           int n_segments, float lr, float beta1, float beta2, float eps, float weight_decay, int step,
                           float max_norm, float grad_scale, const float* sq_norm, void* param_bf16, void* stream);

size_t gdmae_roi_dfvs_pool_workspace_bytes(long long n_points, int batch, int n_rois, int patches_x, int patches_y);
int gdmae_roi_dfvs_pool(const float* points, long long n_points, int n_cols, const float* rois, int batch, int n_rois,
                        int roi_cols, const float* range_xy, const float* patch_lo, int patches_x, int patches_y,
                        const float* extra_width, int num_dvs_points, int num_fps_points, int hash_size, float lambda,
                        float delta, int boxes_per_patch, int phases, int* pooled_idx, int* pooled_num, float* feats_local,
                        float* xyz_global, void* workspace, size_t workspace_bytes, void* stream);

size_t gdmae_roi_graph_folded_floats(void);
size_t gdmae_roi_graph_packed_bytes(void);
size_t gdmae_roi_graph_workspace_bytes(long long n_rois_total);
int gdmae_roi_graph_pack(const float* folded, void* packed, void* stream);
int gdmae_roi_graph_forward(const float* feats_local, const int* pooled_num, const float* rois, int roi_cols,
                            const float* roi_scores, int batch, int n_rois, int scores_normalized, const void* packed,
                            float* rcnn_cls, float* rcnn_reg, float* batch_box_preds, float* batch_cls_preds, int* nbr_debug,
                            void* workspace, size_t workspace_bytes, void* stream);

#ifdef __cplusplus
}
#endif
#endif
```

Before: 1078.

## Sort sparse-conv rows by active-tap mask and skip empty taps per block

Adds a planning pass that computes, for each rulebook, a 9-bit mask of which neighbour taps are present per output row and counting-sorts rows by that mask. The implicit sparse-conv kernel gets a TAPS variant that processes rows in that sorted order, ORs the masks over the block, and only loads weights and runs MFMAs for taps that some row in the block actually uses. The goal is to avoid the many zero-neighbour taps that dominate at 75% masking. In exchange it adds histogram and scatter kernels to the plan, extra buffers, indirect row indexing with scattered output writes, and a smaller weight ring for some shapes.

```diff
diff --git a/gd-mae_amd/csrc/conv_block.hip b/gd-mae_amd/csrc/conv_block.hip
--- a/gd-mae_amd/csrc/conv_block.hip
+++ b/gd-mae_amd/csrc/conv_block.hip
@@ -7,7 +7,7 @@
 bool gd_spconv_supported(int cin, int cout);
 int gd_spconv(hipStream_t st, const void* X, int x_f32, const int* nbr, const void* Wp, long long n, int cin, int cout, void* Y, int slot,
               float* part, const float* ride_part = nullptr, int ride_S = 0, int ride_cout = 0, int ride_cin = 0,
-              float* ride_dW = nullptr);
+              float* ride_dW = nullptr, const int* order = nullptr, const int* omask = nullptr);
 int gd_spconv_rows(int cin, int cout, int x_f32);
 int gd_bn_fold_from_partials(hipStream_t st, const float* part, int nblk, int C, double count, const float* gamma,
                              const float* beta, double eps, double momentum, float* running_mean, float* running_var,
@@ -82,6 +82,10 @@
   return !off && a->bf16 && a->packed_fwd != nullptr && a->packed_bwd != nullptr && gd_spconv_supported(a->cin, a->cout) &&
          gd_spconv_supported(a->cout, a->cin);
 }
+bool use_taps(const int* order, const int* omask) {
+  static const bool on = !(getenv("GDMAE_SPCONV_TAPS") && atoi(getenv("GDMAE_SPCONV_TAPS")) == 0);
+  return on && order != nullptr && omask != nullptr;
+}
 
 __global__ __launch_bounds__(256) void k_spconv_dw_reduce(const float* __restrict__ part, int S, int cout, int cin, float* __restrict__ dW) {
   const long long per_tap = (long long)S * cout * cin, mn4 = (long long)cout * cin / 4;
@@ -142,7 +146,8 @@
     static const bool fuse_ok = !(getenv("GDMAE_SPCONV_STATS") && atoi(getenv("GDMAE_SPCONV_STATS")) == 0);
     stats_fused = fuse_ok && nblk >= 1 && nblk <= 1024;
     CB_TRY(gd_spconv(st, a->x, a->x_f32, a->nbr, a->packed_fwd, a->n_out, a->cin, a->cout, a->y, GD_T_SPCONV_FWD,
-                     stats_fused ? (float*)s.cs_ws : nullptr));
+                     stats_fused ? (float*)s.cs_ws : nullptr, nullptr, 0, 0, 0, nullptr, use_taps(a->order, a->omask) ? a->order : nullptr,
+                     use_taps(a->order, a->omask) ? a->omask : nullptr));
     if (stats_fused)
       CB_TRY(gd_bn_fold_from_partials(st, (const float*)s.cs_ws, (int)nblk, a->cout, (double)a->n_out, a->gamma, a->beta, a->eps, a->momentum,
                                       a->running_mean, a->running_var, a->num_batches, a->stats, a->ab, a->mv));
@@ -195,9 +200,11 @@
     GD_REQUIRE(Gp.S == S, "conv block: slice count");
     static const bool rides = !(getenv("GDMAE_DW_REDUCE_RIDES") && atoi(getenv("GDMAE_DW_REDUCE_RIDES")) == 0);
     bool reduced = false;
+    const bool taps_t = use_taps(a->order_t, a->omask_t);
+    const int *ord_t = taps_t ? a->order_t : nullptr, *om_t = taps_t ? a->omask_t : nullptr;
     if (a->dx && rides) {
       const int rc = gd_spconv(st, s.dy, 0, a->nbr_t, a->packed_bwd, a->n_in, C, a->cin, a->dx, GD_T_SPCONV_BWD, nullptr, (const float*)s.dw_part, S,
-                               C, a->cin, a->dW);
+                               C, a->cin, a->dW, ord_t, om_t);
       if (rc != -2) {
         CB_TRY(rc);
         reduced = true;
@@ -207,7 +214,8 @@
       hipLaunchKernelGGL(k_spconv_dw_reduce, dim3(gd_div_up(9ll * C * a->cin / 4, 256)), dim3(256), 0, st, (const float*)s.dw_part, S, C, a->cin,
                          a->dW);
       GD_LAUNCH_CHECK();
-      if (a->dx) CB_TRY(gd_spconv(st, s.dy, 0, a->nbr_t, a->packed_bwd, a->n_in, C, a->cin, a->dx, GD_T_SPCONV_BWD, nullptr));
+      if (a->dx) CB_TRY(gd_spconv(st, s.dy, 0, a->nbr_t, a->packed_bwd, a->n_in, C, a->cin, a->dx, GD_T_SPCONV_BWD, nullptr, nullptr, 0, 0, 0, nullptr,
+                                  ord_t, om_t));
     }
     return 0;
   }
diff --git a/gd-mae_amd/csrc/partition.hip b/gd-mae_amd/csrc/partition.hip
--- a/gd-mae_amd/csrc/partition.hip
+++ b/gd-mae_amd/csrc/partition.hip
@@ -587,3 +587,124 @@
   GD_LAUNCH_CHECK();
   return 0;
 }
+
+constexpr int kTapBlock = 512;
+constexpr int kTapChunks = 4;
+constexpr int kTapRows = kTapBlock * kTapChunks;
+constexpr int kTapMaxJobs = 16;
+struct TapJob {
+  const int* n_dev;
+  const int* nbr;
+  int* order;
+  int* omask;
+  int* hist;
+};
+struct TapJobs {
+  TapJob j[kTapMaxJobs];
+  int count;
+};
+__device__ __forceinline__ int tap_mask_of(const int* __restrict__ nbr, long long r) {
+  int m = 0;
+#pragma unroll
+  for (int k = 0; k < 9; ++k) m |= (nbr[r * 9 + k] >= 0 ? 1 : 0) << k;
+  return m;
+}
+__global__ __launch_bounds__(kTapBlock) void k_tap_hist(TapJobs J) {
+  const TapJob& q = J.j[blockIdx.y];
+  const long long n = *q.n_dev, base = (long long)blockIdx.x * kTapRows;
+  if (base >= n) return;
+  __shared__ int h[512];
+  const int tid = threadIdx.x;
+  h[tid] = 0;
+  __syncthreads();
+#pragma unroll
+  for (int c = 0; c < kTapChunks; ++c) {
+    const long long r = base + c * kTapBlock + tid;
+    if (r < n) atomicAdd(&h[tap_mask_of(q.nbr, r)], 1);
+  }
+  __syncthreads();
+  q.hist[(long long)blockIdx.x * 512 + tid] = h[tid];
+}
+__global__ __launch_bounds__(kTapBlock) void k_tap_scatter(TapJobs J) {
+  const TapJob& q = J.j[blockIdx.y];
+  const long long n = *q.n_dev, base = (long long)blockIdx.x * kTapRows;
+  if (base >= n) return;
+  __shared__ int sbase[512];
+  __shared__ int scan[2][512];
+  __shared__ int wh[kTapBlock / 64][512];
+  const int tid = threadIdx.x, lane = tid & 63, wv = tid >> 6;
+  const int nb = (int)((n + kTapRows - 1) / kTapRows);
+  int tot = 0, mine = 0;
+  for (int b = 0; b < nb; ++b) {
+    const int v = q.hist[(long long)b * 512 + tid];
+    tot += v;
+    mine += b < (int)blockIdx.x ? v : 0;
+  }
+  scan[0][tid] = tot;
+  __syncthreads();
+  int cur = 0;
+  for (int d = 1; d < 512; d <<= 1) {
+    scan[cur ^ 1][tid] = scan[cur][tid] + (tid >= d ? scan[cur][tid - d] : 0);
+    cur ^= 1;
+    __syncthreads();
+  }
+  sbase[tid] = scan[cur][tid] - tot + mine;
+#pragma unroll
+  for (int w = 0; w < kTapBlock / 64; ++w) wh[w][tid] = 0;
+  __syncthreads();
+  for (int c = 0; c < kTapChunks; ++c) {
+    const long long r = base + c * kTapBlock + tid;
+    const bool valid = r < n;
+    const int key = valid ? tap_mask_of(q.nbr, r) : 512;
+    unsigned long long peers = ~0ull;
+#pragma unroll
+    for (int b = 0; b < 10; ++b) {
+      const bool bit = (key >> b) & 1;
+      const unsigned long long m = __ballot(bit);
+      peers &= bit ? m : ~m;
+    }
+    const int rank = __popcll(peers & ((1ull << lane) - 1ull));
+    if (valid && rank == 0) wh[wv][key] = __popcll(peers);
+    __syncthreads();
+    int run = 0;
+#pragma unroll
+    for (int w = 0; w < kTapBlock / 64; ++w) {
+      const int v = wh[w][tid];
+      wh[w][tid] = run;
+      run += v;
+    }
+    __syncthreads();
+    if (valid) {
+      const int pos = sbase[key] + wh[wv][key] + rank;
+      q.order[pos] = (int)r;
+      q.omask[pos] = key;
+    }
+    __syncthreads();
+    sbase[tid] += run;
+#pragma unroll
+    for (int w = 0; w < kTapBlock / 64; ++w) wh[w][tid] = 0;
+    __syncthreads();
+  }
+}
+size_t gd_tap_order_ws_bytes(long long cap) { return gd_align((size_t)gd_div_up(cap > 0 ? cap : 1, kTapRows) * 512 * sizeof(int)); }
+int gd_plan_tap_orders(const void* jobs, int count, long long cap_max, hipStream_t st) {
+  if (count <= 0) return 0;
+  GD_REQUIRE(count <= kTapMaxJobs, "tap order: at most 16 rulebooks per launch");
+  GD_REQUIRE(cap_max < (1ll << 31) / 9, "tap order: rulebook too large");
+  TapJobs J;
+  const TapJob* src = (const TapJob*)jobs;
+  for (int i = 0; i < kTapMaxJobs; ++i) J.j[i] = src[i < count ? i : 0];
+  J.count = count;
+  const int grid = gd_div_up(cap_max > 0 ? cap_max : 1, kTapRows);
+  hipLaunchKernelGGL(k_tap_hist, dim3(grid, count), dim3(kTapBlock), 0, st, J);
+  GD_LAUNCH_CHECK();
+  hipLaunchKernelGGL(k_tap_scatter, dim3(grid, count), dim3(kTapBlock), 0, st, J);
+  GD_LAUNCH_CHECK();
+  return 0;
+}
+extern "C" size_t gdmae_tap_order_workspace_bytes(long long cap) { return gd_tap_order_ws_bytes(cap); }
+extern "C" int gdmae_tap_order(const int* nbr, const int* n_dev, long long cap, int* order, int* omask, void* workspace, void* stream) {
+  GD_REQUIRE(nbr && n_dev && order && omask && workspace && cap >= 1, "tap_order: null argument");
+  TapJob j{n_dev, nbr, order, omask, (int*)workspace};
+  return gd_plan_tap_orders(&j, 1, cap, (hipStream_t)stream);
+}
diff --git a/gd-mae_amd/csrc/plan.hip b/gd-mae_amd/csrc/plan.hip
--- a/gd-mae_amd/csrc/plan.hip
+++ b/gd-mae_amd/csrc/plan.hip
@@ -49,6 +49,15 @@
                         int* flag, void* lb_state, hipStream_t st);
 int gd_decoder_site_rulebook(const int* site, const int* n_dev, int sites_per_tok, long long cap_sites, const int* tile_slot, int H, int W,
                              int* nbr, hipStream_t st);
+struct TapJob {
+  const int* n_dev;
+  const int* nbr;
+  int* order;
+  int* omask;
+  int* hist;
+};
+size_t gd_tap_order_ws_bytes(long long cap);
+int gd_plan_tap_orders(const void* jobs, int count, long long cap_max, hipStream_t st);
 
 namespace {
 
@@ -89,6 +98,7 @@
   long long vis_tok_cell, vis_map;
   struct {
     long long tok_cell, map, nbr_subm, nbr_subm_t, nbr_down, nbr_down_t, up_sites, win_ws;
+    long long tap[4][2], tap_ws[4];
     long long w[2][7];
   } s[GDMAE_PLAN_MAX_STAGES];
   long long dec_slot, dec_list, dec_flag, dec_nbr[3];
@@ -199,6 +209,18 @@
       O.s[i].nbr_down_t = L.add(name("nbr_down_t"), sizeof(int) * g.cap_in * 9);
     }
     if (g.up_s > 1) O.s[i].up_sites = L.add(name("up_sites"), sizeof(int) * g.cap * g.up_s * g.up_s);
+    static const char* const kTap[4] = {"subm", "subm_t", "down", "down_t"};
+    for (int r = 0; r < 4; ++r) {
+      O.s[i].tap[r][0] = O.s[i].tap[r][1] = O.s[i].tap_ws[r] = -1;
+      if (!p->want_taps || (r >= 2 && p->stride[i] != 2)) continue;
+      const long long rows = r == 3 ? g.cap_in : g.cap;
+      snprintf(nm, sizeof(nm), "s%d.ord_%s", i, kTap[r]);
+      O.s[i].tap[r][0] = L.add(nm, sizeof(int) * rows);
+      snprintf(nm, sizeof(nm), "s%d.om_%s", i, kTap[r]);
+      O.s[i].tap[r][1] = L.add(nm, sizeof(int) * rows);
+      snprintf(nm, sizeof(nm), "s%d.tapws_%s", i, kTap[r]);
+      O.s[i].tap_ws[r] = L.add(nm, gd_tap_order_ws_bytes(rows));
+    }
     O.s[i].win_ws = L.add(name("win_ws"), gd_plan_windows_ws_bytes(B, g.Y, g.X, p->win_x[i], p->win_y[i]));
     const long long wcap = g.n_win < g.cap ? g.n_win : g.cap;
     for (int sh = 0; sh < 2; ++sh)
@@ -281,6 +303,9 @@
   long long cap_max = 1;
   GdWinStage W[4];
   GD_REQUIRE(ns <= 4, "geometry plan: at most four stages");
+  TapJob T[16];
+  int n_tap = 0;
+  long long tap_cap = 1;
   for (int i = 0; i < ns; ++i) {
     const StageGeo& g = O.geo[i];
     GD_REQUIRE(J.count + 4 <= kPlanMaxJobs, "geometry plan: job table full");
@@ -292,6 +317,11 @@
       J.j[J.count++] = PlanJob{n_tok + i, I(O.s[i].tok_cell), Dims{B, g.Y, g.X}, Dims{B, Yp, Xp}, cur_map, 1, 0, I(O.s[i].nbr_down), nullptr};
       J.j[J.count++] = PlanJob{cur_n, cur_cell, Dims{B, Yp, Xp}, Dims{B, g.Y, g.X}, I(O.s[i].map), 2, 0, I(O.s[i].nbr_down_t), nullptr};
       if (g.cap_in > cap_max) cap_max = g.cap_in;
+      if (p->want_taps) {
+        T[n_tap++] = TapJob{n_tok + i, I(O.s[i].nbr_down), I(O.s[i].tap[2][0]), I(O.s[i].tap[2][1]), I(O.s[i].tap_ws[2])};
+        T[n_tap++] = TapJob{cur_n, I(O.s[i].nbr_down_t), I(O.s[i].tap[3][0]), I(O.s[i].tap[3][1]), I(O.s[i].tap_ws[3])};
+        if (g.cap_in > tap_cap) tap_cap = g.cap_in;
+      }
       cur_cell = I(O.s[i].tok_cell);
       cur_map = I(O.s[i].map);
       cur_n = n_tok + i;
@@ -299,6 +329,11 @@
       Xp = g.X;
     }
     J.j[J.count++] = PlanJob{cur_n, cur_cell, Dims{B, g.Y, g.X}, Dims{B, g.Y, g.X}, cur_map, 0, 0, I(O.s[i].nbr_subm), I(O.s[i].nbr_subm_t)};
+    if (p->want_taps) {
+      T[n_tap++] = TapJob{cur_n, I(O.s[i].nbr_subm), I(O.s[i].tap[0][0]), I(O.s[i].tap[0][1]), I(O.s[i].tap_ws[0])};
+      T[n_tap++] = TapJob{cur_n, I(O.s[i].nbr_subm_t), I(O.s[i].tap[1][0]), I(O.s[i].tap[1][1]), I(O.s[i].tap_ws[1])};
+      if (g.cap > tap_cap) tap_cap = g.cap;
+    }
     if (g.up_s > 1) {
       J.j[J.count++] = PlanJob{cur_n, cur_cell, Dims{B, g.Y, g.X}, Dims{B, g.Y, g.X}, nullptr, 3, g.up_s, I(O.s[i].up_sites), nullptr};
       if (g.cap * g.up_s * g.up_s / 9 + 1 > cap_max) cap_max = g.cap * g.up_s * g.up_s / 9 + 1;
@@ -320,6 +355,8 @@
     if (rc) return rc;
     rc = gd_plan_windows_all(W, ns, st);
     if (rc) return rc;
+    rc = gd_plan_tap_orders(T, n_tap, tap_cap, st);
+    if (rc) return rc;
   }
   if (O.dec) {
     const int* maps[3];
diff --git a/gd-mae_amd/csrc/spconv.hip b/gd-mae_amd/csrc/spconv.hip
--- a/gd-mae_amd/csrc/spconv.hip
+++ b/gd-mae_amd/csrc/spconv.hip
@@ -2,6 +2,7 @@
 #include "common.h"
 #include "dw_grouped.h"
 #include <stdlib.h>
+#include <type_traits>
 
 typedef float f32x16 __attribute__((ext_vector_type(16)));
 typedef __bf16 bf16x8 __attribute__((ext_vector_type(8)));
@@ -27,6 +28,8 @@
   int ride_S, ride_cout, ride_cin;
   unsigned ride_blocks;
   const float* bias;
+  const int* order;
+  const int* omask;
 };
 
 __device__ __forceinline__ void sp_ride_dw_reduce(const SpArgs& A) {
@@ -70,7 +73,7 @@
   static constexpr int value = COUT >= 256 ? ((SRC_F32 && CIN >= 256) ? 32 : SP_ROWS256) : ((CIN == 128 && !SRC_F32) ? SP_ROWS128 : 64);
 };
 
-template <int CIN, int COUT, bool SRC_F32, bool EPI = false>
+template <int CIN, int COUT, bool SRC_F32, bool EPI = false, bool TAPS = false>
 __global__ __launch_bounds__(512, 2) void k_spconv(SpArgs A) {
   constexpr int ROWS = SpRows<CIN, COUT, SRC_F32>::value;
   constexpr int KS = CIN / 16;
@@ -93,24 +96,45 @@
   const int mb0 = wv / WPB;
   const int nb0 = (wv % WPB) * NPW;
   const uint4* __restrict__ wp = A.Wp + (size_t)mb0 * 64 + lane;
-
-  constexpr int RING = (KS == 16 && (ROWS == 64 || SRC_F32)) ? ((SRC_F32 && ROWS == 64) ? 4 : 8) : ((KS == 8 && ROWS == 128) ? 4 : KS);
+  unsigned tmask = 0x1FFu;
+  int t0 = 0, t1 = 1;
+  int ord[TAPS ? P : 1];
+  if constexpr (TAPS) {
+#pragma unroll
+    for (int p = 0; p < P; ++p) {
+      const long long g = row0 + p * RPP + tid / CPR;
+      ord[p] = A.order[g < A.n ? g : A.n - 1];
+    }
+    int m = 0;
+    for (int i = lane; i < ROWS; i += 64) m |= row0 + i < A.n ? A.omask[row0 + i] : 0;
+    tmask = 0u;
+#pragma unroll
+    for (int k = 0; k < 9; ++k) tmask |= __ballot((m >> k) & 1) != 0ull ? 1u << k : 0u;
+    tmask = __builtin_amdgcn_readfirstlane(tmask);
+    const unsigned r1 = tmask & (tmask - 1u);
+    t0 = tmask ? __builtin_ctz(tmask) : 0;
+    t1 = r1 ? __builtin_ctz(r1) : t0;
+  }
+
+  constexpr int RING = (KS == 16 && (ROWS == 64 || SRC_F32)) ? (((SRC_F32 || (TAPS && COUT >= 256)) && ROWS == 64) ? 4 : 8) : ((KS == 8 && ROWS == 128) ? 4 : KS);
   SpFrag wr[RING][MPW];
 #pragma unroll
   for (int ks = 0; ks < RING; ++ks)
 #pragma unroll
-    for (int j = 0; j < MPW; ++j) wr[ks][j].q = wp[((size_t)ks * MB + j * kWaves) * 64];
+    for (int j = 0; j < MPW; ++j) wr[ks][j].q = wp[(((size_t)(TAPS ? t0 * KS : 0) + ks) * MB + j * kWaves) * 64];
 
   constexpr int GD = 1;
   constexpr int RQ = SRC_F32 ? 2 : 1;
   const int gc = tid % CPR;
-  long long nrow[P];
+  std::conditional_t<TAPS, int, long long> nrow[P];
   unsigned rvalid = 0u;
 #pragma unroll
   for (int p = 0; p < P; ++p) {
     const long long g = row0 + p * RPP + tid / CPR;
     rvalid |= g < A.n ? 1u << p : 0u;
-    nrow[p] = (g < A.n ? g : A.n - 1) * 9;
+    const long long gcl = g < A.n ? g : A.n - 1;
+    if constexpr (TAPS) nrow[p] = ord[p] * 9;
+    else nrow[p] = gcl * 9;
   }
   int idx[P];
   uint4 rq[1][P][RQ];
@@ -153,9 +177,9 @@
       *reinterpret_cast<uint4*>(b + (p * RPP + tid / CPR) * XP + gc * 16) = q;
     }
   };
-  load_idx(0);
+  load_idx(TAPS ? t0 : 0);
   fetch(0);
-  load_idx(1);
+  load_idx(TAPS ? t1 : 1);
   stage(lds, 0);
   __syncthreads();
 
@@ -167,6 +191,55 @@
 #pragma unroll
       for (int i = 0; i < 16; ++i) acc[j][b][i] = 0.f;
 
+  if constexpr (TAPS) {
+    const unsigned wl = (unsigned)(mb0 * 64 + lane);
+    auto tap_step = [&](auto more_c, int cur, int nxt, int nn, int par) {
+      constexpr bool MORE = decltype(more_c)::value;
+      const uint4* __restrict__ wc = A.Wp + (size_t)cur * (KS * MB * 64);
+      const uint4* __restrict__ wn = A.Wp + (size_t)nxt * (KS * MB * 64);
+      if (MORE) {
+        fetch(0);
+        load_idx(nn);
+      }
+      __builtin_amdgcn_sched_barrier(0);
+      const unsigned char* lb = lds + par * (ROWS * XP) + ((nb0 * 32) + (lane & 31)) * XP + (lane >> 5) * 16;
+      SpFrag sf[2][NPW];
+#pragma unroll
+      for (int b = 0; b < NPW; ++b) sf[0][b].q = *reinterpret_cast<const uint4*>(lb + b * 32 * XP);
+#pragma unroll
+      for (int ks = 0; ks < KS; ++ks) {
+        if (ks + 1 < KS) {
+#pragma unroll
+          for (int b = 0; b < NPW; ++b) sf[(ks + 1) & 1][b].q = *reinterpret_cast<const uint4*>(lb + b * 32 * XP + (ks + 1) * 32);
+        }
+#pragma unroll
+        for (int j = 0; j < MPW; ++j)
+#pragma unroll
+          for (int b = 0; b < NPW; ++b) acc[j][b] = __builtin_amdgcn_mfma_f32_32x32x16_bf16(wr[ks % RING][j].v, sf[ks & 1][b].v, acc[j][b], 0, 0, 0);
+        if (ks + RING < KS) {
+#pragma unroll
+          for (int j = 0; j < MPW; ++j) wr[ks % RING][j].q = wc[((ks + RING) * MB + j * kWaves) * 64 + wl];
+        } else if (MORE) {
+#pragma unroll
+          for (int j = 0; j < MPW; ++j) wr[ks % RING][j].q = wn[((ks + RING - KS) * MB + j * kWaves) * 64 + wl];
+        }
+        __builtin_amdgcn_sched_barrier(0);
+      }
+      if (MORE) stage(lds + (par ^ 1) * (ROWS * XP), 0);
+      __syncthreads();
+    };
+    unsigned rem = tmask;
+    int cur = t0, par = 0;
+    while (rem & (rem - 1u)) {
+      rem &= rem - 1u;
+      const int nxt = __builtin_ctz(rem);
+      const unsigned r2 = rem & (rem - 1u);
+      tap_step(std::true_type{}, cur, nxt, r2 ? __builtin_ctz(r2) : nxt, par);
+      cur = nxt;
+      par ^= 1;
+    }
+    if (rem) tap_step(std::false_type{}, cur, cur, cur, par);
+  } else {
 #pragma unroll
   for (int tap = 0; tap < 9; ++tap) {
     if (tap + GD < 9) {
@@ -196,6 +269,7 @@
     }
     if (tap < 8) stage(lds + ((tap + 1) & 1) * (ROWS * XP), 0);
     __syncthreads();
+  }
   }
 
 #pragma unroll
@@ -233,7 +307,8 @@
       const int rl = p * ORPP + r;
       if (rl < ROWS && row0 + rl < A.n) {
         const uint4 q = *reinterpret_cast<const uint4*>(lds + rl * SP + c * 16);
-        *reinterpret_cast<uint4*>(A.Y + (row0 + rl) * COUT + c * 8) = q;
+        const long long yr = TAPS ? (long long)A.order[row0 + rl] : row0 + rl;
+        *reinterpret_cast<uint4*>(A.Y + yr * COUT + c * 8) = q;
         if (stats) {
           const unsigned w[4] = {q.x, q.y, q.z, q.w};
 #pragma unroll
@@ -265,17 +340,17 @@
   }
 }
 
-template <int CIN, int COUT, bool SRC_F32, bool EPI = false>
+template <int CIN, int COUT, bool SRC_F32, bool EPI = false, bool TAPS = false>
 int sp_launch(const SpArgs& A, hipStream_t st) {
   constexpr int ROWS = SpRows<CIN, COUT, SRC_F32>::value;
   constexpr int tile = ROWS * (CIN * 2 + 16), stg = ROWS * (COUT * 2 + 16);
   constexpr int lds = 2 * tile > stg ? 2 * tile : stg;
   static bool once = false;
   if (!once) {
-    GD_CHECK(hipFuncSetAttribute((const void*)k_spconv<CIN, COUT, SRC_F32, EPI>, hipFuncAttributeMaxDynamicSharedMemorySize, lds));
+    GD_CHECK(hipFuncSetAttribute((const void*)k_spconv<CIN, COUT, SRC_F32, EPI, TAPS>, hipFuncAttributeMaxDynamicSharedMemorySize, lds));
     once = true;
   }
-  hipLaunchKernelGGL((k_spconv<CIN, COUT, SRC_F32, EPI>), dim3((unsigned)gd_div_up(A.n, ROWS) + A.ride_blocks), dim3(512), lds, st, A);
+  hipLaunchKernelGGL((k_spconv<CIN, COUT, SRC_F32, EPI, TAPS>), dim3((unsigned)gd_div_up(A.n, ROWS) + A.ride_blocks), dim3(512), lds, st, A);
   GD_LAUNCH_CHECK();
   return 0;
 }
@@ -296,17 +371,22 @@
   return 0;
 }
 int gd_spconv(hipStream_t st, const void* X, int x_f32, const int* nbr, const void* Wp, long long n, int cin, int cout, void* Y, int slot,
-              float* part, const float* ride_part, int ride_S, int ride_cout, int ride_cin, float* ride_dW) {
+              float* part, const float* ride_part, int ride_S, int ride_cout, int ride_cin, float* ride_dW, const int* order,
+              const int* omask) {
   if (n <= 0) return ride_part ? -2 : 0;
   GD_REQUIRE(gd_spconv_supported(cin, cout), "spconv: channels must be 128 or 256");
-  SpArgs A{X, nbr, (const uint4*)Wp, (unsigned short*)Y, n, part, nullptr, nullptr, 0, 0, 0, 0u, nullptr};
+  GD_REQUIRE((order == nullptr) == (omask == nullptr), "spconv: a tap order is rows and masks");
+  GD_REQUIRE(order == nullptr || n < (1ll << 31) / 9, "spconv: a rulebook with a tap order has 32-bit offsets");
+  SpArgs A{X, nbr, (const uint4*)Wp, (unsigned short*)Y, n, part, nullptr, nullptr, 0, 0, 0, 0u, nullptr, order, omask};
   if (ride_part) {
     A.ride_part = ride_part; A.ride_dW = ride_dW; A.ride_S = ride_S; A.ride_cout = ride_cout; A.ride_cin = ride_cin;
     A.ride_blocks = (unsigned)gd_div_up(9ll * ride_cout * ride_cin / 4, 512);
   }
   GdTimed timed(slot, st, (double)n * (9.0 * cin * (x_f32 ? 4 : 2) + 2.0 * cout + 36.0) + 18.0 * cin * cout, 2.0 * n * 9.0 * cin * cout);
-#define SP_CASE(ci, co)                                                    \
-  if (cin == ci && cout == co) return x_f32 ? sp_launch<ci, co, true>(A, st) : sp_launch<ci, co, false>(A, st);
+#define SP_CASE(ci, co)                                                                                                       \
+  if (cin == ci && cout == co)                                                                                                \
+    return order ? (x_f32 ? sp_launch<ci, co, true, false, true>(A, st) : sp_launch<ci, co, false, false, true>(A, st)) \
+                 : (x_f32 ? sp_launch<ci, co, true>(A, st) : sp_launch<ci, co, false>(A, st));
   SP_CASE(128, 128);
   SP_CASE(128, 256);
   SP_CASE(256, 128);
@@ -333,7 +413,13 @@
 
 extern "C" int gdmae_spconv(const void* X, int x_f32, const int* nbr, const void* packed, long long n, int cin, int cout, void* Y,
                             int timing_slot, void* stream) {
-  return gd_spconv((hipStream_t)stream, X, x_f32, nbr, packed, n, cin, cout, Y, timing_slot > 0 ? timing_slot : GD_T_SPCONV_FWD, nullptr, nullptr, 0, 0, 0, nullptr);
+  return gd_spconv((hipStream_t)stream, X, x_f32, nbr, packed, n, cin, cout, Y, timing_slot > 0 ? timing_slot : GD_T_SPCONV_FWD, nullptr, nullptr, 0, 0, 0, nullptr,
+                   nullptr, nullptr);
+}
+extern "C" int gdmae_spconv_taps(const void* X, int x_f32, const int* nbr, const int* order, const int* omask, const void* packed, long long n,
+                                 int cin, int cout, void* Y, float* part, void* stream) {
+  GD_REQUIRE(order != nullptr && omask != nullptr, "spconv_taps: tap order (gdmae_tap_order)");
+  return gd_spconv((hipStream_t)stream, X, x_f32, nbr, packed, n, cin, cout, Y, GD_T_SPCONV_FWD, part, nullptr, 0, 0, 0, nullptr, order, omask);
 }
 extern "C" int gdmae_spconv_bias_relu(const void* X, int x_f32, const int* nbr, const void* packed, const float* bias, long long n, int cin,
                                       int cout, void* Y, void* stream) {
@@ -356,7 +442,7 @@
 extern "C" int gdmae_spconv_stats(const void* X, int x_f32, const int* nbr, const void* packed, long long n, int cin, int cout, void* Y,
                                   float* part, void* stream) {
   GD_REQUIRE(part != nullptr, "spconv_stats: partial rows");
-  return gd_spconv((hipStream_t)stream, X, x_f32, nbr, packed, n, cin, cout, Y, GD_T_SPCONV_FWD, part, nullptr, 0, 0, 0, nullptr);
+  return gd_spconv((hipStream_t)stream, X, x_f32, nbr, packed, n, cin, cout, Y, GD_T_SPCONV_FWD, part, nullptr, 0, 0, 0, nullptr, nullptr, nullptr);
 }
 
 
diff --git a/gd-mae_amd/gdmae_hip/convblock.py b/gd-mae_amd/gdmae_hip/convblock.py
--- a/gd-mae_amd/gdmae_hip/convblock.py
+++ b/gd-mae_amd/gdmae_hip/convblock.py
@@ -16,7 +16,7 @@
 class ConvBNReLUFn(torch.autograd.Function):
     @staticmethod
     def forward(ctx, x, info):
-        weight, bn, nbr, nbr_t, direct, out_f32 = info
+        weight, bn, nbr, nbr_t, direct, out_f32, taps = info
         cout, _, _, cin = weight.shape
         n_in, n_out = x.shape[0], nbr.shape[0]
         dev = x.device
@@ -30,6 +30,9 @@
         a.eps = float(bn.eps)
         a.x, a.nbr, a.nbr_t, a.W = L.ptr(x), L.ptr(nbr), L.ptr(nbr_t), L.ptr(wc)
         a.gamma, a.beta = L.ptr(bn.weight), L.ptr(bn.bias)
+        if taps is not None:
+            assert taps[0].numel() == n_out and taps[2].numel() == n_in
+            a.order, a.omask, a.order_t, a.omask_t = (L.ptr(t) for t in taps)
         if bn.training and bn.running_mean is not None:
             a.momentum = float(bn.momentum)
             a.running_mean, a.running_var, a.num_batches = L.ptr(bn.running_mean), L.ptr(bn.running_var), L.ptr(bn.num_batches_tracked)
@@ -51,7 +54,7 @@
         L.call("gdmae_conv_block_fwd", C.byref(a), L.stream())
         ctx.save_for_backward(x, cols, y, stats, abmv, wc, nbr, nbr_t, bn.weight.detach())
         ctx.meta = (a, nb, direct, x.dtype)
-        ctx.packed = packed
+        ctx.packed, ctx.taps = packed, taps
         return out
 
     @staticmethod
@@ -71,8 +74,8 @@
         return dx, None
 
 
-def conv_bn_relu(x, conv, bn, nbr, nbr_t, out_f32=False):
+def conv_bn_relu(x, conv, bn, nbr, nbr_t, out_f32=False, taps=None):
     direct = [ops.direct_grad(p) for p in (conv.weight, bn.weight, bn.bias)]
     if any(t is None for t in direct) or not x.is_cuda:
         return None
-    return ConvBNReLUFn.apply(x, (conv.weight, bn, nbr, nbr_t, direct, out_f32))
+    return ConvBNReLUFn.apply(x, (conv.weight, bn, nbr, nbr_t, direct, out_f32, taps))
diff --git a/gd-mae_amd/gdmae_hip/lib.py b/gd-mae_amd/gdmae_hip/lib.py
--- a/gd-mae_amd/gdmae_hip/lib.py
+++ b/gd-mae_amd/gdmae_hip/lib.py
@@ -122,6 +122,9 @@
     "gdmae_spconv_packed_bytes": (_Z, [_I, _I]),
     "gdmae_spconv_pack_jobs": (_I, [_P, _I, _I, _I, _P, _P]),
     "gdmae_spconv": (_I, [_P, _I, _P, _P, _L, _I, _I, _P, _I, _P]),
+    "gdmae_spconv_taps": (_I, [_P, _I, _P, _P, _P, _P, _L, _I, _I, _P, _P, _P]),
+    "gdmae_tap_order_workspace_bytes": (_Z, [_L]),
+    "gdmae_tap_order": (_I, [_P, _P, _L, _P, _P, _P, _P]),
     "gdmae_spconv_bias_relu": (_I, [_P, _I, _P, _P, _P, _L, _I, _I, _P, _P]),
     "gdmae_spconv_stat_rows": (_I, [_I, _I, _I]),
     "gdmae_spconv_stats": (_I, [_P, _I, _P, _P, _L, _I, _I, _P, _P, _P]),
@@ -223,7 +226,7 @@
     _fields_ = [("n_points", _L), ("n_cols", _I), ("batch_size", _I), ("lo", _F * 3), ("vs", _F * 3), ("grid", _I * 3), ("n_stages", _I),
                 ("stride", _I * 4), ("win_x", _I * 4), ("win_y", _I * 4), ("n_levels", _I * 4), ("drop_lo", (_I * 3) * 4),
                 ("drop_hi", (_I * 3) * 4), ("max_tokens", (_I * 3) * 4), ("masked", _I), ("keep_frac", _D), ("n_dec", _I),
-                ("dec_sources", _I * 4), ("want_pm", _I), ("cap_points", _L)]
+                ("dec_sources", _I * 4), ("want_pm", _I), ("cap_points", _L), ("want_taps", _I)]
 
 
 class PlanBuffer(C.Structure):
@@ -235,7 +238,7 @@
                  ("eps", _F), ("momentum", _F)]
                 + [(k, _P) for k in ("x", "nbr", "nbr_t", "W", "gamma", "beta", "running_mean", "running_var", "num_batches", "cols",
                                      "y", "stats", "ab", "mv", "out", "g", "dx", "dW", "dgamma", "dbeta", "scratch", "packed_fwd", "packed_bwd")]
-                + [("out_f32", _I)])
+                + [("out_f32", _I)] + [(k, _P) for k in ("order", "omask", "order_t", "omask_t")])
 
 
 _lib = None
diff --git a/gd-mae_amd/gdmae_hip/plan.py b/gd-mae_amd/gdmae_hip/plan.py
--- a/gd-mae_amd/gdmae_hip/plan.py
+++ b/gd-mae_amd/gdmae_hip/plan.py
@@ -339,6 +339,7 @@
 
 
 import collections
+import os
 import time as _time
 
 EVENT_WAIT_S = 0.0
@@ -399,9 +400,10 @@
     for g in range(P.n_dec):
         P.dec_sources[g] = int(dec_sources[g])
     P.want_pm = 1
-    table = (L.PlanBuffer * 160)()
+    P.want_taps = int(keep_frac is not None and os.environ.get("GDMAE_SPCONV_TAPS", "1") != "0")
+    table = (L.PlanBuffer * 224)()
     n_ent, total = C.c_int(0), C.c_size_t(0)
-    L.call("gdmae_geometry_plan_layout", C.byref(P), table, 160, C.byref(n_ent), C.byref(total))
+    L.call("gdmae_geometry_plan_layout", C.byref(P), table, 224, C.byref(n_ent), C.byref(total))
     names = {table[i].name.decode(): (int(table[i].offset), int(table[i].bytes)) for i in range(n_ent.value)}
     hit = _PLAN_SHAPES[key] = (P, names, int(total.value), geo, m_cap, (lo, vs, (gx, gy, gz)))
     while len(_PLAN_SHAPES) > _PLAN_SHAPES_MAX:
@@ -522,6 +524,8 @@
                            V(pre + "nbr_down_t", i32, n_prev, 9) if g["strided"] else None, wps)
             sp._nbr_subm_t = V(pre + "nbr_subm_t", i32, n, 9)
             sp._up_sites = (g["up_s"], V(pre + "up_sites", i32, n * g["up_s"] * g["up_s"])) if g["up_s"] > 1 else None
+            sp._taps = {r: (V(f"{pre}ord_{r}", i32, n_prev if r == "down_t" else n), V(f"{pre}om_{r}", i32, n_prev if r == "down_t" else n))
+                        for r in ("subm", "subm_t", "down", "down_t") if A.has(f"{pre}ord_{r}")}
             stages.append(sp)
         dt = None
         if A.has("dec.tile_slot"):
diff --git a/gd-mae_amd/pcdet/utils/spconv_utils.py b/gd-mae_amd/pcdet/utils/spconv_utils.py
--- a/gd-mae_amd/pcdet/utils/spconv_utils.py
+++ b/gd-mae_amd/pcdet/utils/spconv_utils.py
@@ -65,6 +65,12 @@
         nxt = x._plan.stages[x._stage + 1]
         return nxt.nbr_down, nxt.nbr_down_t, x._stage + 1
 
+    def tap_orders(self, x: SparseConvTensor):
+        sp = x.stage_plan if self.subm else x._plan.stages[x._stage + 1]
+        taps = getattr(sp, "_taps", None) or {}
+        a, b = taps.get("subm" if self.subm else "down"), taps.get("subm_t" if self.subm else "down_t")
+        return None if a is None or b is None else (a[0], a[1], b[0], b[1])
+
     def forward(self, x: SparseConvTensor) -> SparseConvTensor:
         nbr, nbr_t, stage = self.rulebooks(x)
         f = ops.SparseConv3x3.apply(x.features, self.weight, nbr, nbr_t)
@@ -99,7 +105,7 @@
             conv, bn = mods[0], mods[1]
             if self.native_block and isinstance(conv, SparseConvolution):
                 nbr, nbr_t, stage = conv.rulebooks(x)
-                f = convblock.conv_bn_relu(x.features, conv, bn, nbr, nbr_t, self.out_fp32)
+                f = convblock.conv_bn_relu(x.features, conv, bn, nbr, nbr_t, self.out_fp32, conv.tap_orders(x))
                 if f is not None:
                     return x.replace_feature(f) if stage == x._stage else SparseConvTensor(f, x._plan, stage)
             x = conv(x)
diff --git a/include/gdmae_hip.h b/include/gdmae_hip.h
--- a/include/gdmae_hip.h
+++ b/include/gdmae_hip.h
@@ -73,6 +73,8 @@
                             int* tok_cell_out, int* map_out, int* n_out, int* flag_ws, void* scan_ws, void* stream);
 int gdmae_rulebook(const int* n_tok, const int* tok_cell, long long cap, int B, int Yt, int Xt, int Ym, int Xm,
                    const int* map, int mode, int* nbr, void* stream);
+size_t gdmae_tap_order_workspace_bytes(long long cap);
+int gdmae_tap_order(const int* nbr, const int* n_dev, long long cap, int* order, int* omask, void* workspace, void* stream);
 
 size_t gdmae_window_workspace_bytes(int B, int Y, int X, int wx, int wy);
 int gdmae_window_partition(const int* map, int B, int Y, int X, int wx, int wy, int shifted, int nlev,
@@ -237,12 +239,16 @@
   const void* packed_fwd;
   const void* packed_bwd;
   int out_f32;
+  const int *order, *omask;
+  const int *order_t, *omask_t;
 } gdmae_conv_block_args;
 size_t gdmae_conv_block_scratch_bytes(long long n_in, long long n_out, int cin, int cout, int bf16);
 size_t gdmae_spconv_packed_bytes(int cin, int cout);
 int gdmae_spconv_pack_jobs(const float* W , int cin, int cout, int transposed, void* packed, long long* jobs);
 int gdmae_spconv(const void* X, int x_f32, const int* nbr, const void* packed, long long n, int cin, int cout, void* Y,
                  int timing_slot , void* stream);
+int gdmae_spconv_taps(const void* X, int x_f32, const int* nbr, const int* order, const int* omask, const void* packed, long long n,
+                      int cin, int cout, void* Y, float* part, void* stream);
 int gdmae_spconv_bias_relu(const void* X, int x_f32, const int* nbr, const void* packed, const float* bias, long long n, int cin, int cout,
                            void* Y, void* stream);
 int gdmae_spconv_stat_rows(int cin, int cout, int x_f32);
@@ -400,6 +406,7 @@
   int dec_sources[GDMAE_PLAN_MAX_STAGES];
   int want_pm;
   long long cap_points;
+  int want_taps;
 } gdmae_plan_params;
 typedef struct gdmae_plan_buffer {
   char name[40];
```

After: 1087 (median of 6 runs). About the same (+0.8%).
